# gbordelon/fast_ray_tracer

Measured on AMD Instinct MI355X. Metric: Mrays/s (primary+shadow+secondary) + wall-clock/frame, 1/2/4/8 GPU, higher is better.
Workload: dtype f64

## Files before the change

### fast_ray_tracer_amd/csrc/frt_camera.hpp

```cpp
#pragma once

#include "frt_shadow.hpp"

namespace frt {

struct QueuedRay {
    double o[3];
    double d[3];
    uint64_t key;
    int32_t parent;
    int32_t slot;
};

struct HitRec {
    double t;
    int32_t node;
    int32_t pad;
};

__device__ __forceinline__ double rng_uniform(uint64_t seed, uint64_t key, uint64_t d) {
    const uint64_t h = mix64(seed ^ mix64(key * 0x9e3779b97f4a7c15ULL + d * 0xd1b54a32d192ed03ULL + 0x632be59bd9b4e019ULL));
    return (double)(h >> 11) * 0x1.0p-53;
}

__device__ inline void cmj_point(uint64_t seed, uint64_t pixel, int U, int V, int u, int v, double* out) {
    const uint64_t base = 2ull * (uint64_t)U * (uint64_t)V;
    int p = v;
    for (int j = V - 1; j >= 0; --j) {
        const int k = (int)(j + rng_uniform(seed, pixel, base + j) * (double)(V - j));
        if (p == j) p = k;
        else if (p == k) p = j;
    }
    {
        const int f = p * U + u;
        const int jj = f / V, ii = f % V;
        const double r = rng_uniform(seed, pixel, 2ull * (uint64_t)f);
        out[0] = (ii + (jj + r) / (double)U) / (double)V;
    }
    p = u;
    for (int i = U - 1; i >= 0; --i) {
        const int k = (int)(i + rng_uniform(seed, pixel, base + (uint64_t)V + i) * (double)(U - i));
        if (p == i) p = k;
        else if (p == k) p = i;
    }
    {
        const int f = v * U + p;
        const int jj = f / V, ii = f % V;
        const double r = rng_uniform(seed, pixel, 2ull * (uint64_t)f + 1);
        out[1] = (jj + (ii + r) / (double)V) / (double)U;
    }
}

__device__ inline void aperture_point(const frt_camera& cam, uint64_t seed, uint64_t sample, double* xy,
                                      unsigned& err) {
    const double* a = cam.aperture_args;
    const int type = cam.aperture_type;
    if (type == 6 || type == 4 || type == 5 || type == 8 || type < 0 || type > 8) {
        xy[0] = 0.5;
        xy[1] = 0.5;
        return;
    }
    for (int attempt = 0; attempt < 4096; ++attempt) {
        const double x = rng_uniform(seed ^ 0xa5e7u, sample, 2ull * attempt);
        const double y = rng_uniform(seed ^ 0xa5e7u, sample, 2ull * attempt + 1);
        const double u = 2 * x - 1, v = 2 * y - 1;
        bool ok;
        switch (type) {
        case 0: ok = !(u * u + v * v > a[0]); break;
        case 1: ok = ((u > a[0]) && (u <= a[1])) || ((v > a[2]) && (v <= a[3])); break;
        case 2:
            ok = (u <= 0) ? (-u + a[0] <= v) && (v < u + a[1]) : (0 <= x) ? (u + a[2] <= v) && (v < -u + a[3]) : false;
            break;
        case 3: {
            const double mag = u * u + v * v;
            ok = !(mag > a[0] || mag < a[1]);
            break;
        }
        default: ok = true; break;
        }
        if (ok) {
            xy[0] = x;
            xy[1] = y;
            return;
        }
    }
    err |= kErrAperture;
    xy[0] = 0.5;
    xy[1] = 0.5;
}

__device__ __forceinline__ void ray_for_pixel(const frt_camera& cam, double px, double py, const double* jit,
                                              const double* ap, Ray& r) {
    double xoff = (px + jit[0]) * cam.pixel_size;
    double yoff = (py + jit[1]) * cam.pixel_size;
    double wx = cam.half_width - xoff, wy = cam.half_height - yoff;
    double p[3] = {wx, wy, -cam.canvas_distance}, pixel[3], origin[3];
    xf_point(cam.inv, p, pixel);
    double q[3] = {(ap[0] - 0.5) * cam.aperture_size, (ap[1] - 0.5) * cam.aperture_size, 0.0};
    xf_point(cam.inv, q, origin);
    double v[3] = {pixel[0] - origin[0], pixel[1] - origin[1], pixel[2] - origin[2]};
    r.o[0] = origin[0];
    r.o[1] = origin[1];
    r.o[2] = origin[2];
    normalize3(v, r.d);
}

__device__ __forceinline__ void camera_ray(const DevScene& S, const Batch& B, int64_t s, Ray& r, uint64_t& key,
                                           unsigned& err) {
    const int64_t pix = B.pixel_begin + s / B.spp;
    const int sub = (int)(s % B.spp);
    const int64_t hs = S.cam.hsize;
    const int64_t row = B.row_begin + (pix / hs) * B.row_stride;
    const int64_t col = pix % hs;
    const uint64_t global_pixel = (uint64_t)(row * hs + col);
    const uint64_t global_sample = global_pixel * (uint64_t)B.spp + (uint64_t)sub;
    double jit[2], ap[2] = {0.5, 0.5};
    if (S.cam.jitter) {
        const int U = (int)S.cam.usteps, V = (int)S.cam.vsteps;
        cmj_point(B.seed, global_pixel, U, V, sub % U, sub / U, jit);
    } else {
        jit[0] = S.sample_table[2 * sub];
        jit[1] = S.sample_table[2 * sub + 1];
    }
    if (S.cam.aperture_size != 0.0) aperture_point(S.cam, B.seed, global_sample, ap, err);
    ray_for_pixel(S.cam, (double)col, (double)row, jit, ap, r);
    key = (global_sample << 12) | 1ull;
}

}
```

### fast_ray_tracer_amd/csrc/frt_engine.hip

```cpp
#include <hip/hip_runtime.h>
#include <hipcub/hipcub.hpp>

#include <algorithm>
#include <array>
#include <atomic>
#include <condition_variable>
#include <memory>
#include <mutex>
#include <cmath>
#include <cstdio>
#include <cstdlib>
#include <cstring>
#include <string>
#include <chrono>
#include <functional>
#include <thread>
#include <vector>

#include "frt_device.h"
#include "frt_jit.h"
#include "frt_shade.hpp"
#include "frt_shade32.hpp"
#include "frt_shadow.hpp"
#include "frt_jit_rt.hpp"
#include "frt_camera.hpp"
#include "frt_cols.hpp"

namespace frt {

constexpr int kBlock = 256;
constexpr int kMaxPathLength = 11;

struct NodeRec {
    double over_point[3];
    uint64_t key;
    int32_t material;
    int32_t parent;
    int32_t slot;
    int32_t flags;
    double normalv[3];
    double eyev[3];
    double Ka[3], Kd[3], Ks[3];
    double refl[3];
    double Ns, over_d, rf;
};
static_assert(sizeof(NodeRec) == 216, "NodeRec layout");

struct NodeCore {
    int32_t material, flags, parent, slot;
    double normalv[3], eyev[3];
    double over_d, rf;
};
struct NodeColors {
    double Ka[3], Kd[3], Ks[3], refl[3];
    double Ns;
};
static_assert(sizeof(NodeCore) == 80 && sizeof(NodeColors) == 104, "NodeCols layout");
enum NodeFlags : int32_t { kReflApplies = 1, kRefrApplies = 2, kMix = 4, kDissolve = 8, kReflSpawned = 16, kRefrSpawned = 32 };
enum : int32_t { kOwnColors = 64, kOwnD = 128 };

struct NodeCols {
    Cols<NodeCore> core;
    Cols<NodeColors> col;
    const ShadowHead* head = nullptr;
    int32_t root = 0;
    int32_t eye_cam = 0;
    static size_t bytes(int64_t cap) { return Cols<NodeCore>::bytes(cap) + Cols<NodeColors>::bytes(cap); }
    void set(uint64_t* base, int64_t cap) {
        core.w = base;
        core.cap = cap;
        col.w = base + (size_t)Cols<NodeCore>::kWords * cap;
        col.cap = cap;
    }
    __device__ __forceinline__ void store(int64_t i, const NodeRec& v, bool own_colors, bool own_d) const {
        NodeCore c;
        for (int k = 0; k < 3; ++k) {
            c.normalv[k] = v.normalv[k];
            c.eyev[k] = v.eyev[k];
        }
        c.material = v.material;
        c.parent = v.parent;
        c.slot = v.slot;
        c.flags = v.flags | (own_colors ? kOwnColors : 0) | (own_d ? kOwnD : 0);
        c.over_d = v.over_d;
        c.rf = v.rf;
        uint64_t t[10];
        __builtin_memcpy(t, &c, sizeof(c));
        const int64_t cap = core.cap;
        core.w[i] = t[0];
        if (!root) core.w[cap + i] = t[1];
#pragma unroll
        for (int f = 2; f < 5; ++f) core.w[f * cap + i] = t[f];
        if (!eye_cam) {
#pragma unroll
            for (int f = 5; f < 8; ++f) core.w[f * cap + i] = t[f];
        }
        if (own_d) core.w[8 * cap + i] = t[8];
        if (c.flags & kMix) core.w[9 * cap + i] = t[9];
        if (own_colors) {
            NodeColors o;
            for (int k = 0; k < 3; ++k) {
                o.Ka[k] = v.Ka[k];
                o.Kd[k] = v.Kd[k];
                o.Ks[k] = v.Ks[k];
                o.refl[k] = v.refl[k];
            }
            o.Ns = v.Ns;
            col.store(i, o);
        }
    }
    __device__ __forceinline__ void store_miss(int64_t i, int32_t parent, int32_t slot) const {
        core.w[i] = (uint64_t)(uint32_t)-1;
        if (!root) core.w[core.cap + i] = (uint64_t)(uint32_t)parent | ((uint64_t)(uint32_t)slot << 32);
    }
    __device__ __forceinline__ NodeRec load(int64_t i, const frt_material* __restrict__ mats) const {
        uint64_t t[10];
        const int64_t cap = core.cap;
        t[0] = core.w[i];
        t[1] = root ? (uint64_t)(uint32_t)-1 : core.w[cap + i];
#pragma unroll
        for (int f = 2; f < 5; ++f) t[f] = core.w[f * cap + i];
#pragma unroll
        for (int f = 5; f < 8; ++f) t[f] = eye_cam ? 0ull : core.w[f * cap + i];
        const int32_t mat = (int32_t)(uint32_t)t[0], fl = (int32_t)(t[0] >> 32);
        const double od = (fl & kOwnD) ? __longlong_as_double((long long)core.w[8 * cap + i])
                          : mat >= 0 ? 1.0 - mats[mat].Tr : 0.0;
        const double rf = (fl & kMix) ? __longlong_as_double((long long)core.w[9 * cap + i]) : 0.0;
        t[8] = (uint64_t)__double_as_longlong(od);
        t[9] = (uint64_t)__double_as_longlong(rf);
        NodeCore c;
        __builtin_memcpy(&c, t, sizeof(c));
        NodeRec v;
        const ShadowHead& hd = head[i];
        for (int k = 0; k < 3; ++k) {
            v.over_point[k] = hd.over_point[k];
            v.normalv[k] = c.normalv[k];
            v.eyev[k] = c.eyev[k];
        }
        v.key = hd.key;
        v.material = c.material;
        v.parent = c.parent;
        v.slot = c.slot;
        v.flags = c.flags;
        v.over_d = c.over_d;
        v.rf = c.rf;
        if (c.material < 0) {
            for (int k = 0; k < 3; ++k) v.Ka[k] = v.Kd[k] = v.Ks[k] = v.refl[k] = 0.0;
            v.Ns = 0.0;
        } else if (c.flags & kOwnColors) {
            const NodeColors o = col.load(i);
            for (int k = 0; k < 3; ++k) {
                v.Ka[k] = o.Ka[k];
                v.Kd[k] = o.Kd[k];
                v.Ks[k] = o.Ks[k];
                v.refl[k] = o.refl[k];
            }
            v.Ns = o.Ns;
        } else {
            const frt_material& M = mats[c.material];
            for (int k = 0; k < 3; ++k) {
                v.Ka[k] = M.Ka[k];
                v.Kd[k] = M.Kd[k];
                v.Ks[k] = M.Ks[k];
                v.refl[k] = M.refl[k];
            }
            v.Ns = M.Ns;
        }
        return v;
    }
};










extern __shared__ __align__(16) char frt_walk_smem[];

#ifndef FRT_TRACE_WAVES
#define FRT_TRACE_WAVES 4
#endif
template <int kFeat>
__global__ void __launch_bounds__(kTraceBlock)
__attribute__((amdgpu_waves_per_eu((kFeat & kFeatTorus) ? 1 : FRT_TRACE_WAVES, 8))) k_trace(DevScene S, Batch B, const QueuedRay* __restrict__ q, int64_t n,
                                                       HitRec* __restrict__ hits, double* __restrict__ hn12, unsigned* err,
                                                       int filter_casts) {
    const int64_t i = (int64_t)blockIdx.x * blockDim.x + threadIdx.x;
    const bool live = i < n && (q == nullptr || q[queue_slot(B, i)].parent >= -1);
    Ray r{{0, 0, 0}, {0, 0, 1}};
    unsigned e = 0;
    if (live) {
        if (q == nullptr) {
            uint64_t key;
            camera_ray(S, B, i, r, key, e);
        } else {
            const QueuedRay& qr = q[queue_slot(B, i)];
            for (int k = 0; k < 3; ++k) {
                r.o[k] = qr.o[k];
                r.d[k] = qr.d[k];
            }
        }
    }
    double t;
    double n12[2];
    const int node = walk<false, kFeat>(S, r, 0.0, live, t, frt_walk_smem, e, n12, filter_casts != 0);
    if (i < n) {
        hits[i] = live ? HitRec{t, node, 0} : HitRec{0.0, -1, 0};
        if (hn12 != nullptr) {
            hn12[2 * i] = live ? n12[0] : 1.0;
            hn12[2 * i + 1] = live ? n12[1] : 1.0;
        }
    }
    if (e) atomicOr(err, e);
}

template <int kFeat>
__global__ void __launch_bounds__(kTraceBlock) k_trace_redo(DevScene S, Batch B, const QueuedRay* __restrict__ q, int64_t n,
                                                            HitRec* __restrict__ hits, unsigned* err,
                                                            const int32_t* __restrict__ redo,
                                                            const unsigned* __restrict__ redo_count, unsigned redo_cap) {
    const unsigned cnt = min(*redo_count, redo_cap);
    const int64_t wave = ((int64_t)blockIdx.x * blockDim.x + threadIdx.x) >> 6;
    const int64_t nwaves = ((int64_t)gridDim.x * blockDim.x) >> 6;
    unsigned e = 0;
    for (int64_t base = wave * 64; base < (int64_t)cnt; base += nwaves * 64) {
        const int64_t k = base + (threadIdx.x & 63);
        const int64_t i = k < (int64_t)cnt ? (int64_t)redo[k] : -1;
        const bool live = i >= 0 && i < n;
        Ray r{{0, 0, 0}, {0, 0, 1}};
        if (live) {
            if (q == nullptr) {
                uint64_t key;
                camera_ray(S, B, i, r, key, e);
            } else {
                const QueuedRay& qr = q[queue_slot(B, i)];
                for (int a = 0; a < 3; ++a) {
                    r.o[a] = qr.o[a];
                    r.d[a] = qr.d[a];
                }
            }
        }
        double t;
        double n12[2];
        const int node = walk<false, kFeat>(S, r, 0.0, live, t, frt_walk_smem, e, n12, false);
        if (live) hits[i] = HitRec{t, node, 0};
    }
    if (e) atomicOr(err, e);
}

#ifndef FRT_PREPARE_WAVES
#define FRT_PREPARE_WAVES 1
#endif
template <bool kPat>
__device__ __forceinline__ bool prepare_node(const DevScene& S, const Batch& B, const QueuedRay* __restrict__ q,
                                             int64_t n, const HitRec* __restrict__ hits, const double* __restrict__ hn12,
                                             NodeCols& rec,
                                             ShadowHead* __restrict__ heads, QueuedRay* __restrict__ next_q,
                                             unsigned long long* counters, unsigned* err, int64_t node, double* op,
                                             int* spawned, int uniform_ok) {
    unsigned long long* line = counters + kCounterLine * (blockIdx.x % kQueueSegs);
    const int64_t seg_base = (int64_t)(blockIdx.x % kQueueSegs) * B.next_segcap;
#ifdef FRT_WALK_PROF
    unsigned long long pt0 = prof_stamp();
    auto pstamp = [&](int k) {
        const unsigned long long t1 = prof_stamp();
        if ((threadIdx.x & 63) == 0) atomicAdd(S.dbg + kDbgProf + 8 + k, t1 - pt0);
        pt0 = t1;
    };
#define PSTAMP(k) pstamp(k)
#else
#define PSTAMP(k)
#endif
    Ray r;
    uint64_t key;
    int32_t parent = -1, slot = 0;
    if (q == nullptr) {
        unsigned ce = 0;
        camera_ray(S, B, node, r, key, ce);
    } else {
        const QueuedRay& qr = q[queue_slot(B, node)];
        for (int k = 0; k < 3; ++k) {
            r.o[k] = qr.o[k];
            r.d[k] = qr.d[k];
        }
        key = qr.key;
        parent = qr.parent;
        slot = qr.slot;
    }
    PSTAMP(0);
    const HitRec hr = hits[node];
    PSTAMP(1);
    if (hr.node < 0) {
        rec.store_miss(node, parent, slot);
        heads[node].material = -1;
        return false;
    }
    auto prepare_hit = [&](const DevScene& S, const int leaf) __attribute__((always_inline)) {
    Hit h{hr.t, -1, -1, leaf};
    Comps c;
    prepare<kPat>(S, r, h, c);
    c.n1 = hn12 != nullptr ? hn12[2 * node] : 1.0;
    c.n2 = hn12 != nullptr ? hn12[2 * node + 1] : 1.0;
    PSTAMP(2);
    if (B.stats) wave_count(line + 17, true);
    const frt_material& M = S.materials[c.material];
    NodeRec nr;
    for (int k = 0; k < 3; ++k) {
        nr.over_point[k] = c.over_point[k];
        nr.normalv[k] = c.normalv[k];
        nr.eyev[k] = c.eyev[k];
        nr.Ka[k] = c.Ka[k];
        nr.Kd[k] = c.Kd[k];
        nr.Ks[k] = c.Ks[k];
        nr.refl[k] = c.refl[k];
    }
    nr.Ns = c.Ns;
    nr.over_d = c.over_d;
    nr.rf = 0.0;
    nr.key = key;
    nr.material = c.material;
    nr.parent = parent;
    nr.slot = slot;
    int32_t flags = 0;
    if (S.cfg.include_specular) {
        const bool reflect_applies = B.remaining > 0 && M.reflective;
        bool refract_applies = false;
        double refr_dir[3] = {0, 0, 0};
        if (B.remaining > 0 && c.over_d > 0.0) {
            double n_ratio = c.n1 / c.n2;
            double cos_i = dot3(c.eyev, c.normalv);
            double sin2_t = n_ratio * n_ratio * (1.0 - cos_i * cos_i);
            if (!(sin2_t > 1.0)) {
                refract_applies = true;
                double cos_t = sqrt(1.0 - sin2_t);
                double s1 = n_ratio * cos_i - cos_t;
                for (int k = 0; k < 3; ++k) {
                    double t1 = c.normalv[k] * s1;
                    double t2 = c.eyev[k] * n_ratio;
                    refr_dir[k] = t1 - t2;
                }
            }
        }
        if (reflect_applies) flags |= kReflApplies;
        if (refract_applies) flags |= kRefrApplies;
        if (M.reflective && c.over_d < 1.0) {
            flags |= kMix;
            nr.rf = schlick(c.eyev, c.normalv, c.n1, c.n2);
        }
        if (M.Tr > 0.0 && c.over_d > 0.0) flags |= kDissolve;

        const uint64_t code = key & 0xFFFull;
        const uint64_t base = key & ~0xFFFull;
        const bool want_refl = reflect_applies && (c.refl[0] != 0.0 || c.refl[1] != 0.0 || c.refl[2] != 0.0);
        const bool tf_zero = M.Tf[0] == 0.0 && M.Tf[1] == 0.0 && M.Tf[2] == 0.0;
        const bool want_refr = refract_applies && !tf_zero;
        if (want_refl) flags |= kReflSpawned;
        if (want_refr) flags |= kRefrSpawned;
        const bool dense = spawned != nullptr;
        const unsigned long long at_refl = dense ? 0ull : wave_append(line + B.level + 1, want_refl);
        const unsigned long long at_refr = dense ? 0ull : wave_append(line + B.level + 1, want_refr);
        if (dense) *spawned = (want_refl ? 1 : 0) | (want_refr ? 2 : 0);
        if (B.stats) {
            wave_count(line + 16, reflect_applies && !want_refl);
            wave_count(line + 16, refract_applies && !want_refr);
        }
        if (want_refl) {
            if (dense || (int64_t)at_refl < B.next_segcap) {
                QueuedRay qo;
                for (int k = 0; k < 3; ++k) {
                    qo.o[k] = c.over_point[k];
                    qo.d[k] = c.reflectv[k];
                }
                qo.key = base | ((code * 2) & 0xFFFull);
                qo.parent = (int32_t)node;
                qo.slot = 0;
                next_q[dense ? node : seg_base + (int64_t)at_refl] = qo;
            } else {
                atomicOr(err, kErrQueueOverflow);
            }
        }
        if (want_refr) {
            if (dense || (int64_t)at_refr < B.next_segcap) {
                QueuedRay qo;
                for (int k = 0; k < 3; ++k) {
                    qo.o[k] = c.under_point[k];
                    qo.d[k] = refr_dir[k];
                }
                qo.key = base | ((code * 2 + 1) & 0xFFFull);
                qo.parent = (int32_t)node;
                qo.slot = 1;
                next_q[dense ? n + node : seg_base + (int64_t)at_refr] = qo;
            } else {
                atomicOr(err, kErrQueueOverflow);
            }
        }
    }
    nr.flags = flags;
    PSTAMP(3);
    const bool own = kPat && (M.map_Ka >= 0 || M.map_Kd >= 0 || M.map_Ks >= 0 || M.map_refl >= 0 || M.map_Ns >= 0);
    rec.store(node, nr, own, kPat && M.map_d >= 0);
    ShadowHead hd;
    for (int k = 0; k < 3; ++k) hd.over_point[k] = c.over_point[k];
    hd.key = key;
    hd.material = c.material;
    hd.pad = 0;
#ifdef FRT_EXPERIMENT_HEAD_COLS
    {
        uint64_t t[5];
        __builtin_memcpy(t, &hd, sizeof(hd));
        uint64_t* w = (uint64_t*)heads;
#pragma unroll
        for (int f = 0; f < 5; ++f) w[(int64_t)f * n + node] = t[f];
    }
#else
    heads[node] = hd;
#endif
    PSTAMP(4);
    for (int k = 0; k < 3; ++k) op[k] = c.over_point[k];
    };
    if (uniform_ok) {
        const int leaf_u = uniform(hr.node);
        if (__ballot(hr.node != leaf_u) == 0ull) {
            if (B.stats) wave_count(line + 18, (int)(threadIdx.x & 63) == __builtin_ctzll(__ballot(true)));
            prepare_hit(uniform_view(S), leaf_u);
            return true;
        }
    }
    prepare_hit(S, hr.node);
    return true;
}

__device__ __forceinline__ void tile_box(int64_t node, int64_t n, bool hit, const double* op, float* __restrict__ tbox,
                                         int tile_log2, float* __restrict__ stbox, int sub_log2) {
    float lo[3], hi[3];
#pragma unroll
    for (int a = 0; a < 3; ++a) {
        lo[a] = hit ? __double2float_rd(op[a]) : __builtin_huge_valf();
        hi[a] = hit ? __double2float_ru(op[a]) : -__builtin_huge_valf();
    }
    for (int off = 1; off < (1 << tile_log2); off <<= 1) {
        if (stbox != nullptr && off == (1 << sub_log2) && node < n && (node & (off - 1)) == 0) {
            float* b = stbox + 6 * (node >> sub_log2);
#pragma unroll
            for (int a = 0; a < 3; ++a) {
                b[a] = lo[a];
                b[a + 3] = hi[a];
            }
        }
#pragma unroll
        for (int a = 0; a < 3; ++a) {
            lo[a] = fminf(lo[a], __shfl_xor(lo[a], off, 64));
            hi[a] = fmaxf(hi[a], __shfl_xor(hi[a], off, 64));
        }
    }
    if (node < n && (node & ((1 << tile_log2) - 1)) == 0) {
        float* b = tbox + 6 * (node >> tile_log2);
#pragma unroll
        for (int a = 0; a < 3; ++a) {
            b[a] = lo[a];
            b[a + 3] = hi[a];
        }
    }
}

template <bool kPat>
__global__ void __launch_bounds__(kBlock) __attribute__((amdgpu_waves_per_eu(kPat ? 1 : FRT_PREPARE_WAVES, 8)))
k_prepare(DevScene S, Batch B, const QueuedRay* __restrict__ q, int64_t n, const HitRec* __restrict__ hits,
          const double* __restrict__ hn12,
          NodeCols rec, ShadowHead* __restrict__ heads, QueuedRay* __restrict__ next_q, unsigned long long* counters,
          unsigned* err, float* __restrict__ tbox, int tile_log2, float* __restrict__ stbox, int sub_log2,
          int32_t* __restrict__ counts, unsigned long long* __restrict__ spawn_masks, int uniform_ok) {
    const int64_t node = (int64_t)blockIdx.x * blockDim.x + threadIdx.x;
    double op[3] = {0.0, 0.0, 0.0};
    bool hit = false;
    if (node < n && counts != nullptr)
        for (int l = 0; l < S.num_lights; ++l) counts[node * S.num_lights + l] = 0;
    int spawned = 0;
    if (node < n)
        hit = prepare_node<kPat>(S, B, q, n, hits, hn12, rec, heads, next_q, counters, err, node, op,
                                 spawn_masks != nullptr ? &spawned : nullptr, uniform_ok);
    if (spawn_masks != nullptr) {
        const unsigned long long mr = __ballot(spawned & 1), mt = __ballot((spawned >> 1) & 1);
        const int64_t g = node >> 6, G = (n + 63) >> 6;
        if ((threadIdx.x & 63) == 0 && g < G) {
            spawn_masks[g] = mr;
            spawn_masks[G + g] = mt;
        }
    }
    if (tbox != nullptr) tile_box(node, n, hit, op, tbox, tile_log2, stbox, sub_log2);
}

#ifdef FRT_SHADOW_WAVES
#define FRT_SHADOW_ATTR __attribute__((amdgpu_waves_per_eu(FRT_SHADOW_WAVES, 8)))
#else
#define FRT_SHADOW_ATTR
#endif
template <int kFeat>
__global__ void __launch_bounds__(kTraceBlock) FRT_SHADOW_ATTR k_shadow(DevScene S, Batch B, const ShadowHead* __restrict__ shead, int64_t n,
                                                        const int32_t* __restrict__ j_light,
                                                        const int32_t* __restrict__ j_point, int32_t samples_per_node,
                                                        int32_t* __restrict__ counts, unsigned* err) {
    ShadowLane L;
    shadow_lane(S, B, shead, n, j_light, j_point, samples_per_node, (int64_t)blockIdx.x * blockDim.x + threadIdx.x, L);
    unsigned e = 0;
    double unused;
#ifdef FRT_EXPERIMENT_NOWALK
    const bool lit = L.live && L.distance > 0.5;
#else
    const bool lit = walk<true, kFeat>(S, L.r, L.distance, L.live, unused, frt_walk_smem, e) == 0 && L.live;
#endif
    if (e) atomicOr(err, e);
    shadow_count(S, L, lit, counts);
}

template <int kFeat>
__global__ void __launch_bounds__(kTraceBlock) k_shadow_redo(DevScene S, Batch B, const ShadowHead* __restrict__ shead, int64_t n,
                                                             const int32_t* __restrict__ j_light,
                                                             const int32_t* __restrict__ j_point, int32_t samples_per_node,
                                                             int32_t* __restrict__ counts, unsigned* err,
                                                             const int64_t* __restrict__ redo,
                                                             const unsigned* __restrict__ redo_count, unsigned redo_cap) {
    const unsigned cnt = min(*redo_count, redo_cap);
    const int64_t wave = ((int64_t)blockIdx.x * blockDim.x + threadIdx.x) >> 6;
    const int64_t nwaves = ((int64_t)gridDim.x * blockDim.x) >> 6;
    unsigned e = 0;
    for (int64_t base = wave * 64; base < (int64_t)cnt; base += nwaves * 64) {
        const int64_t k = base + (threadIdx.x & 63);
        ShadowLane L;
        shadow_lane(S, B, shead, n, j_light, j_point, samples_per_node, k < (int64_t)cnt ? redo[k] : -1, L);
        double unused;
        const bool lit = walk<true, kFeat>(S, L.r, L.distance, L.live, unused, frt_walk_smem, e) == 0 && L.live;
        if (lit) atomicAdd(counts + L.node * S.num_lights + L.light, 1);
    }
    if (e) atomicOr(err, e);
}

#ifndef FRT_SHADE_FACTOR
#define FRT_SHADE_FACTOR 1
#endif
#ifndef FRT_SHADE_ALG
#define FRT_SHADE_ALG 1
#endif
#ifndef FRT_SHADE_SKIP
#define FRT_SHADE_SKIP 1
#endif
#ifndef FRT_SHADE_FMA
#define FRT_SHADE_FMA 1
#endif
__device__ __forceinline__ double dot3_shade(const double* a, const double* b) {
    if (FRT_SHADE_FMA) return __builtin_fma(a[0], b[0], __builtin_fma(a[1], b[1], a[2] * b[2]));
    return dot3(a, b);
}
__device__ __forceinline__ void camera_eyev(const DevScene& S, const Batch& B, int64_t i, double* eyev) {
    Ray r;
    uint64_t key;
    unsigned ce = 0;
    camera_ray(S, B, i, r, key, ce);
    for (int k = 0; k < 3; ++k) eyev[k] = r.d[k] * -1.0;
}

__global__ void __launch_bounds__(kBlock) k_view_rays(DevScene S, Batch B, const frt_camera* __restrict__ cams,
                                                      int32_t nviews, int64_t view_pixels, int64_t n,
                                                      QueuedRay* __restrict__ q, unsigned* err) {
    const int64_t i = (int64_t)blockIdx.x * blockDim.x + threadIdx.x;
    if (i >= n) return;
    const int64_t pix = B.pixel_begin + i / B.spp;
    const int view = (int)min((int64_t)(nviews - 1), pix / view_pixels);
    Batch Bv = B;
    Bv.pixel_begin = pix - (int64_t)view * view_pixels - i / B.spp;
    unsigned e = 0;
    auto emit = [&](const frt_camera& cam) {
        DevScene Sv = S;
        Sv.cam = cam;
        QueuedRay qr;
        Ray r;
        camera_ray(Sv, Bv, i, r, qr.key, e);
        for (int k = 0; k < 3; ++k) {
            qr.o[k] = r.o[k];
            qr.d[k] = r.d[k];
        }
        qr.parent = -1;
        qr.slot = 0;
        q[i] = qr;
    };
    const int view_u = uniform(view);
    if (__ballot(view != view_u) == 0ull) emit(const_table(cams)[view_u]);
    else emit(cams[view]);
    if (e) atomicOr(err, e);
}

constexpr int kLdsPoints = 128;
__device__ __forceinline__ void shade_node(const DevScene& S, const Batch& B, const NodeRec& nr, int64_t i,
                                           const int32_t* __restrict__ counts, double* out, double* lds_row = nullptr,
                                           int32_t c0 = -1) {
    double sA[3] = {0, 0, 0}, sD[3] = {0, 0, 0}, sS[3] = {0, 0, 0};
    if (S.cfg.include_direct) {
        for (int li = 0; li < S.num_lights; ++li) {
            const frt_light& L = S.lights[li];
            const int32_t cnt = c0 >= 0 ? c0 : counts[i * S.num_lights + li];
// ... 308 lines not shown
                const int row = L.rows <= 1 ? 0 : light_row(L, B.seed, nr.key, li, 1);
                const int ra = __builtin_amdgcn_readfirstlane(row);
                if (L.rows <= 1) {
                    uniform_points(row0);
                } else if (__ballot(row != ra) == 0ull) {
                    uniform_points(row0 + 3 * (int64_t)ra * ns);
                } else {
                    const float* pts = row0 + 3 * (int64_t)row * ns;
                    float a[3] = {pts[0], pts[1], pts[2]};
                    const float* q1 = pts + 3 * min(1, ns - 1);
                    float b[3] = {q1[0], q1[1], q1[2]};
                    for (int p = 0; p < ns; ++p) {
                        const float lp[3] = {a[0], a[1], a[2]};
                        a[0] = b[0];
                        a[1] = b[1];
                        a[2] = b[2];
                        const float* q = pts + 3 * min(p + 2, ns - 1);
                        b[0] = q[0];
                        b[1] = q[1];
                        b[2] = q[2];
                        point_term32(P, Q, lp, sums);
                    }
                }
                const double scaling = inten / (double)L.num_samples;
                for (int k = 0; k < 3; ++k) {
                    const double dacc = nr.Kd[k] * L.intensity[k] * sums.ldn;
                    const double sacc =
                        nr.Ks[k] * L.intensity[k] * sums.b + (1.0 - nr.Ks[k]) * L.intensity[k] * sums.fb;
                    cD[k] = (0.0 + dacc) * scaling;
                    cS[k] = (0.0 + sacc) * scaling;
                }
            }
            if (S.cfg.include_ambient)
                for (int k = 0; k < 3; ++k) cA[k] = 0.0 + amb[k];
            for (int k = 0; k < 3; ++k) {
                sA[k] += cA[k];
                sD[k] += cD[k];
                sS[k] += cS[k];
            }
        }
    }
    for (int k = 0; k < 3; ++k) {
        out[k] = sA[k];
        out[4 + k] = sD[k];
        out[8 + k] = sS[k];
    }
    out[3] = out[7] = out[11] = 0.0;
}

__device__ __forceinline__ bool shade_heavy(const DevScene& S, const int32_t* __restrict__ counts, int64_t i) {
    if (!S.cfg.include_direct || !(S.cfg.include_diffuse || S.cfg.include_spec_highlight)) return false;
    for (int li = 0; li < S.num_lights; ++li)
        if (counts[i * S.num_lights + li] != 0) return true;
    return false;
}

__device__ __forceinline__ void ambient_node(const DevScene& S, const NodeRec& nr, double* out) {
    double sA[3] = {0, 0, 0};
    if (S.cfg.include_direct && S.cfg.include_ambient)
        for (int li = 0; li < S.num_lights; ++li) {
            const frt_light& L = S.lights[li];
            for (int k = 0; k < 3; ++k) sA[k] += 0.0 + nr.Ka[k] * L.intensity[k];
        }
    for (int k = 0; k < 3; ++k) {
        out[k] = sA[k];
        out[4 + k] = 0.0;
        out[8 + k] = 0.0;
    }
    out[3] = out[7] = out[11] = 0.0;
}

constexpr int kShadeSegs = 64;
static_assert(kShadeSegs == jit::kMixSegs, "k_shade_lit reads its slots with jit::mix_slot");
template <bool kLazy>
__global__ void __launch_bounds__(kBlock) k_shade(DevScene S, Batch B, NodeCols rec, int64_t n,
                                                  const int32_t* __restrict__ counts, Cols<Tri9> surface,
                                                  uint32_t* __restrict__ lit, unsigned* __restrict__ lcount,
                                                  uint32_t segcap) {
    const int64_t i = (int64_t)blockIdx.x * blockDim.x + threadIdx.x;
    bool heavy = false, mine = false;
    NodeRec nr{};
    if (i < n) {
        nr = rec.load(i, S.materials);
        mine = nr.material >= 0;
        heavy = mine && lit != nullptr && shade_heavy(S, counts, i);
    }
    if (!kLazy && mine && !heavy) {
        double out[12];
        if (rec.eye_cam) camera_eyev(S, B, i, nr.eyev);
        shade_node(S, B, nr, i, counts, out);
        tri_store(surface, i, out);
    }
    if (lit != nullptr) {
        const unsigned long long m = __ballot(heavy);
        if (m) {
            const int lane = threadIdx.x & 63;
            const int seg = (int)(blockIdx.x % kShadeSegs);
            unsigned base = 0;
            if (lane == 0) base = atomicAdd(lcount + seg * jit::kMixLine, (unsigned)__popcll(m));
            base = __shfl(base, 0, 64);
            const unsigned at = base + (unsigned)__popcll(m & ((1ull << lane) - 1));
            if (heavy) lit[(size_t)seg * segcap + at] = (uint32_t)i;
        }
    }
}

struct MaskPopc {
    const unsigned long long* m;
    int64_t count;
    __host__ __device__ uint32_t operator()(int64_t i) const { return i < count ? (uint32_t)__popcll(m[i]) : 0u; }
};
__global__ void __launch_bounds__(kBlock) k_spawn_expand(const unsigned long long* __restrict__ masks,
                                                         const uint32_t* __restrict__ offs, int64_t n, int64_t G,
                                                         uint32_t* __restrict__ qperm,
                                                         unsigned long long* __restrict__ counters) {
    const int64_t g = (int64_t)blockIdx.x * blockDim.x + threadIdx.x;
    if (g == 0) counters[20] = offs[2 * G];
    if (g >= 2 * G) return;
    unsigned long long m = masks[g];
    uint32_t at = offs[g];
    const uint32_t slot0 = (uint32_t)((g < G ? 0 : n) + ((g < G ? g : g - G) << 6));
    while (m != 0ull) {
        qperm[at++] = slot0 + (uint32_t)__builtin_ctzll(m);
        m &= m - 1ull;
    }
}

__global__ void __launch_bounds__(kBlock) k_queue_keys(Batch B, const QueuedRay* __restrict__ q, int64_t n, int pbits,
                                                       int shift, uint32_t* __restrict__ keys,
                                                       uint32_t* __restrict__ slots) {
    const int64_t i = (int64_t)blockIdx.x * blockDim.x + threadIdx.x;
    if (i >= n) return;
    const int64_t s = queue_slot(B, i);
    const QueuedRay& qr = q[s];
    keys[i] = ((uint32_t)(qr.slot & 1) << (pbits - shift)) | ((uint32_t)qr.parent >> shift);
    slots[i] = (uint32_t)s;
}

__device__ __forceinline__ unsigned lit_total(const unsigned* __restrict__ lcount) {
    const int lane = threadIdx.x & 63;
    unsigned incl = lcount[lane * jit::kMixLine];
#pragma unroll
    for (int o = 1; o < 64; o <<= 1) {
        const unsigned t = __shfl_up(incl, o, 64);
        if (lane >= o) incl += t;
    }
    return __shfl(incl, 63, 64);
}

__global__ void __launch_bounds__(kBlock) k_lit_rows(DevScene S, Batch B, const ShadowHead* __restrict__ head,
                                                     const uint32_t* __restrict__ lit, const unsigned* __restrict__ lcount,
                                                     uint32_t segcap, int sort_light, uint32_t* __restrict__ rows,
                                                     uint32_t* __restrict__ nodes) {
    const uint32_t m = blockIdx.x * blockDim.x + threadIdx.x;
    const unsigned total = lit_total(lcount);
    if (blockIdx.x * blockDim.x + (threadIdx.x & ~63u) >= total) return;
    const size_t slot = jit::mix_slot(m < total ? m : 0u, lcount, segcap);
    if (m >= total) return;
    const uint32_t i = lit[slot];
    rows[m] = (uint32_t)light_row(S.lights[sort_light], B.seed, head[i].key, sort_light, 1);
    nodes[m] = i;
}

struct LitStage {
    double over_point[3], normalv[3], eyev[3];
    uint64_t key;
    int32_t material, flags;
    uint32_t node;
    int32_t c0;
};
static_assert(sizeof(LitStage) == 96, "LitStage layout");

__global__ void __launch_bounds__(kBlock) k_lit_stage(DevScene S, Batch B, NodeCols rec, const int32_t* __restrict__ counts,
                                                      const uint32_t* __restrict__ lit, const unsigned* __restrict__ lcount,
                                                      uint32_t segcap, int sort_light, uint32_t* __restrict__ rows,
                                                      uint32_t* __restrict__ vals, LitStage* __restrict__ stage) {
    const uint32_t m = blockIdx.x * blockDim.x + threadIdx.x;
    const unsigned total = lit_total(lcount);
    if (blockIdx.x * blockDim.x + (threadIdx.x & ~63u) >= total) return;
    const size_t slot = jit::mix_slot(m < total ? m : 0u, lcount, segcap);
    if (m >= total) return;
    const uint32_t i = lit[slot];
    NodeRec nr = rec.load(i, S.materials);
    if (rec.eye_cam) camera_eyev(S, B, i, nr.eyev);
    LitStage r;
    for (int k = 0; k < 3; ++k) {
        r.over_point[k] = nr.over_point[k];
        r.normalv[k] = nr.normalv[k];
        r.eyev[k] = nr.eyev[k];
    }
    r.key = nr.key;
    r.material = nr.material;
    r.flags = nr.flags;
    r.node = i;
    r.c0 = S.num_lights == 1 ? counts[i] : -1;
    uint64_t w[12];
    __builtin_memcpy(w, &r, sizeof(r));
    uint64_t* dst = (uint64_t*)(stage + m);
#pragma unroll
    for (int k = 0; k < 12; ++k) dst[k] = w[k];
    rows[m] = (uint32_t)light_row(S.lights[sort_light], B.seed, nr.key, sort_light, 1);
    vals[m] = m;
}

#ifndef FRT_SHADE_WAVES
#define FRT_SHADE_WAVES 4
#endif
template <bool kRows, bool kFast32>
__device__ __forceinline__ void shade_lit_body(const DevScene& S, const Batch& B, const NodeCols& rec,
                                               const int32_t* __restrict__ counts, Cols<Tri9> surface,
                                               const uint32_t* __restrict__ lit,
                                               const unsigned* __restrict__ lcount, uint32_t segcap,
                                               const uint32_t* __restrict__ flat,
                                               const LitStage* __restrict__ stage, uint32_t* __restrict__ spos,
                                               const Light32& F) {
    const uint32_t m = blockIdx.x * blockDim.x + threadIdx.x;
    const int lane = threadIdx.x & 63;
    const unsigned c = lcount[lane * jit::kMixLine];
    unsigned incl = c;
#pragma unroll
    for (int o = 1; o < 64; o <<= 1) {
        const unsigned t = __shfl_up(incl, o, 64);
        if (lane >= o) incl += t;
    }
    const unsigned total = __shfl(incl, 63, 64);
    if (blockIdx.x * blockDim.x + (threadIdx.x & ~63u) >= total) return;
    int64_t i = 0;
    NodeRec nr{};
    int32_t c0 = -1;
    const bool staged = kRows && stage != nullptr;
    const bool sorted_out = kRows && spos != nullptr;
    if (staged) {
        if (m >= total) return;
        const uint64_t* src = (const uint64_t*)(stage + flat[m]);
        uint64_t w[12];
#pragma unroll
        for (int k = 0; k < 12; ++k) w[k] = src[k];
        LitStage r;
        __builtin_memcpy(&r, w, sizeof(r));
        for (int k = 0; k < 3; ++k) {
            nr.over_point[k] = r.over_point[k];
            nr.normalv[k] = r.normalv[k];
            nr.eyev[k] = r.eyev[k];
        }
        nr.key = r.key;
        nr.material = r.material;
        nr.flags = r.flags;
        c0 = r.c0;
        i = (int64_t)r.node;
    } else {
        if (flat != nullptr) {
            if (m >= total) return;
            i = (int64_t)flat[m];
        } else {
            const size_t slot = jit::mix_slot(m < total ? m : 0u, lcount, segcap);
            if (m >= total) return;
            i = (int64_t)lit[slot];
        }
        nr = rec.load(i, S.materials);
        if (rec.eye_cam) camera_eyev(S, B, i, nr.eyev);
    }
    if (staged) {
        if (nr.flags & kOwnColors) {
            const NodeColors o = rec.col.load(i);
            for (int k = 0; k < 3; ++k) {
                nr.Ka[k] = o.Ka[k];
                nr.Kd[k] = o.Kd[k];
                nr.Ks[k] = o.Ks[k];
            }
            nr.Ns = o.Ns;
        } else {
            const frt_material& M = S.materials[nr.material];
            for (int k = 0; k < 3; ++k) {
                nr.Ka[k] = M.Ka[k];
                nr.Kd[k] = M.Kd[k];
                nr.Ks[k] = M.Ks[k];
            }
            nr.Ns = M.Ns;
        }
    }
    double out[12];
#ifndef FRT_SHADE_LDS_ROWS
#define FRT_SHADE_LDS_ROWS 0
#endif
    if constexpr (kFast32) {
        shade_node32(S, B, F, nr, i, counts, out, c0);
    } else if (kRows && FRT_SHADE_LDS_ROWS) {
        __shared__ double lds_rows[kBlock / 64][3 * kLdsPoints];
        shade_node(S, B, nr, i, counts, out, lds_rows[threadIdx.x >> 6], c0);
    } else {
        shade_node(S, B, nr, i, counts, out, nullptr, c0);
    }
    if (sorted_out) {
        uint64_t* dst = surface.w + (size_t)9 * m;
#pragma unroll
        for (int k = 0; k < 3; ++k) {
            dst[k] = (uint64_t)__double_as_longlong(out[k]);
            dst[3 + k] = (uint64_t)__double_as_longlong(out[4 + k]);
            dst[6 + k] = (uint64_t)__double_as_longlong(out[8 + k]);
        }
        spos[i] = m;
        return;
    }
    tri_store(surface, i, out);
}

template <bool kRows>
__global__ void __launch_bounds__(kBlock) __attribute__((amdgpu_waves_per_eu(FRT_SHADE_WAVES, 8))) k_shade_lit(DevScene S, Batch B, NodeCols rec,
                                                      const int32_t* __restrict__ counts, Cols<Tri9> surface,
                                                      const uint32_t* __restrict__ lit,
                                                      const unsigned* __restrict__ lcount, uint32_t segcap,
                                                      const uint32_t* __restrict__ flat,
                                                      const LitStage* __restrict__ stage, uint32_t* __restrict__ spos) {
    shade_lit_body<kRows, false>(S, B, rec, counts, surface, lit, lcount, segcap, flat, stage, spos, Light32{});
}

template <bool kRows>
__global__ void __launch_bounds__(kBlock) k_shade_lit32(DevScene S, Batch B, NodeCols rec,
                                                        const int32_t* __restrict__ counts, Cols<Tri9> surface,
                                                        const uint32_t* __restrict__ lit,
                                                        const unsigned* __restrict__ lcount, uint32_t segcap,
                                                        const uint32_t* __restrict__ flat,
                                                        const LitStage* __restrict__ stage, uint32_t* __restrict__ spos,
                                                        Light32 F) {
    shade_lit_body<kRows, true>(S, B, rec, counts, surface, lit, lcount, segcap, flat, stage, spos, F);
}

__device__ __forceinline__ void combine_node(const DevScene& S, const int32_t* __restrict__ counts,
                                             const NodeRec& nr, int64_t i, Cols<Tri9> surface, Cols<Tri9> child,
                                             const frt_material* __restrict__ mats, int32_t include_specular,
                                             double* col, const uint32_t* __restrict__ spos = nullptr) {
    if (nr.material < 0) {
        for (int k = 0; k < 12; ++k) col[k] = 0.0;
        return;
    }
    if (counts != nullptr && !shade_heavy(S, counts, i)) {
        ambient_node(S, nr, col);
    } else if (spos != nullptr) {
        const uint64_t* src = surface.w + (size_t)9 * spos[i];
#pragma unroll
        for (int k = 0; k < 3; ++k) {
            col[k] = __longlong_as_double((long long)src[k]);
// ... 720 lines not shown
    std::vector<void*> owned;
    std::vector<double> host_table;
    hipStream_t stream = nullptr;
    int32_t* j_light = nullptr;
    int32_t* j_point = nullptr;
    int32_t samples_per_node = 0;
    size_t lds_bytes = 0;
    void* jit_shadow = nullptr;
    void* jit_beam = nullptr;
    void* jit_tile = nullptr;
    void* jit_list = nullptr;
    int tile = 0;
    uint64_t scene_key = 0;
    void* jit_sub = nullptr;
    int sub = 0;
    int sub_ps = 0;
    const int32_t* light_psamp2 = nullptr;
    const float* light_sbox = nullptr;
    uint32_t* slist = nullptr;
    int64_t slist_cap = 0;
    uint64_t sub_pairs = 0, sub_mixed = 0;
    void* jit_subtile = nullptr;
    void* jit_trace = nullptr;
    int32_t* tredo = nullptr;
    int64_t tredo_cap = 0;
    int subtile = 0;
    bool node_beam = false;
    float* stbox = nullptr;
    int64_t stbox_cap = 0;
    uint32_t* s2list = nullptr;
    int64_t s2list_cap = 0;
    uint64_t subtile_pairs = 0, subtile_mixed = 0;
    float* tbox = nullptr;
    int64_t tbox_cap = 0;
    uint32_t* tlist = nullptr;
    int64_t tlist_cap = 0;
    uint64_t tile_pairs = 0, tile_mixed = 0, node_pairs = 0, node_mixed = 0;
    bool jit_beam_on = true;
    const int32_t* light_psamp = nullptr;
    const float* light_aabb = nullptr;
    uint32_t* mixed = nullptr;
    int64_t mixed_cap = 0;
    unsigned* mcount = nullptr;
    uint64_t sync_epoch = 0;
    PinnedBuf<unsigned> host_mcount;
    PinnedBuf<unsigned long long> host_counters;
    PinnedBuf<unsigned> host_lcount;
    int64_t* redo = nullptr;
    unsigned* redo_count = nullptr;
    unsigned redo_cap = 0;
    frt_frame_stats* cur_st = nullptr;
    uint64_t rays_walked = 0;
    uint64_t pairs_walked = 0;
    uint64_t heads_walked = 0;
    unsigned long long uniform_stats[3] = {0, 0, 0};
    uint32_t* shade_lit = nullptr;
    int64_t shade_lit_cap = 0;
    int sort_light = -1;
    int shade_stage = 0;
    uint32_t* lit_row = nullptr;
    int64_t lit_row_cap = 0;
    uint32_t* lit_flat = nullptr;
    int64_t lit_flat_cap = 0;
    frt::LitStage* lit_stage = nullptr;
    int64_t lit_stage_cap = 0;
    bool fast32 = false;
    frt::Light32 light32{nullptr, nullptr};
    int queue_sort = 2;
    int queue_sort_shift = 0;
    int prepare_uniform = 1;
    uint32_t* qsort = nullptr;
    int64_t qsort_cap = 0;
    unsigned long long* spawn_masks = nullptr;
    int64_t spawn_masks_cap = 0;
    uint32_t* spawn_offs = nullptr;
    int64_t spawn_offs_cap = 0;
    unsigned char* scan_tmp = nullptr;
    int64_t scan_tmp_cap = 0;
    unsigned* shade_lcount = nullptr;
    int64_t shade_lcount_cap = 0;
    unsigned long long* jit_stats = nullptr;
    struct Level {
        frt::NodeCols rec;
        frt::ShadowHead* head = nullptr;
        frt::QueuedRay* q = nullptr;
        frt::Cols<frt::Tri9> surface;
        frt::Cols<frt::Tri9> child;
        int64_t* qprefix = nullptr;
        std::vector<int64_t> hprefix = std::vector<int64_t>(frt::kQueueSegs + 1, 0);
        int32_t* counts = nullptr;
        uint32_t* spos = nullptr;
        bool staged = false;
        uint32_t* qperm = nullptr;
        int64_t qperm_cap = 0;
        bool sorted = false;
        int64_t cap = 0;
    };
    std::vector<Level> levels;
    frt::HitRec* hits = nullptr;
    int64_t hits_cap = 0;
    double* hn12 = nullptr;
    int64_t hn12_cap = 0;
    frt::Cols<frt::Tri9> sample_col;
    int64_t sample_cap = 0;
    double* out_dev = nullptr;
    int64_t out_cap = 0;
    frt_camera* view_cams = nullptr;
    int64_t view_cams_cap = 0;
    int32_t strip_views = 0;
    frt::QueuedRay* view_q = nullptr;
    int64_t view_q_cap = 0;
    unsigned long long* counters = nullptr;
    unsigned* err = nullptr;
    hipEvent_t ev[2] = {nullptr, nullptr};
    struct Mark {
        int slot;
        size_t a, b;
    };
    std::vector<hipEvent_t> ev_pool;
    std::vector<Mark> ev_marks;
    size_t ev_used = 0;
    std::vector<frt_light> host_lights;
    struct Gi {
        bool built = false;
        uint64_t seed = 0;
        void* map_mem[2] = {nullptr, nullptr};
        uint64_t photons[2] = {0, 0};
        frt::QueuedRay* pq[2] = {nullptr, nullptr};
        double* ppow[2] = {nullptr, nullptr};
        int64_t pq_cap[2] = {0, 0}, ppow_cap[2] = {0, 0};
        frt::HitRec* phits = nullptr;
        int64_t phits_cap = 0;
        double* pn12 = nullptr;
        int64_t pn12_cap = 0;
        frt::StoredPhoton* store = nullptr;
        int64_t store_cap = 0;
        frt::QueuedRay* gq = nullptr;
        frt::HitRec* ghits = nullptr;
        double* gcol = nullptr;
        frt::GatherReq* greq = nullptr;
        int64_t gq_cap = 0, ghits_cap = 0, gcol_cap = 0, greq_cap = 0;
        unsigned* gwork = nullptr;
        uint32_t* gkeys = nullptr;
        int64_t gkeys_cap = 0;
        double* extra = nullptr;
        double* fgather = nullptr;
        int64_t extra_cap = 0, fgather_cap = 0;
    } gi;
};

static thread_local std::string g_last_error;

static inline void hip_ignore(hipError_t) {}

static int fail(const std::string& msg) {
    g_last_error = msg;
    return -1;
}

#define FRT_HIP(call)                                                                                   \
    do {                                                                                                \
        hipError_t e_ = (call);                                                                         \
        if (e_ != hipSuccess) return fail(std::string(#call) + ": " + hipGetErrorString(e_));          \
    } while (0)

template <typename T>
static const T* upload(frt_scene_handle* h, const T* src, size_t count, int& rc) {
// ... 1137 lines not shown
        hipMemset(h->S.dbg, 0, frt::kDbgSlots * sizeof(unsigned long long)) != hipSuccess) {
        frt_scene_release(h);
        return fail("frt_scene_upload: debug counters");
    }
#endif
    static const bool wtrace = std::getenv("FRT_WARMUP_TRACE") != nullptr;
    const auto ts0 = std::chrono::steady_clock::now();
    {
        std::lock_guard<std::mutex> lk(g_warm_mu);
        if (device >= 0 && device < 64 && g_warm_stream[device] != nullptr) {
            h->stream = g_warm_stream[device];
            g_warm_stream[device] = nullptr;
        }
    }
    const bool stream_ok = h->stream != nullptr || hipStreamCreate(&h->stream) == hipSuccess;
    if (wtrace)
        std::fprintf(stderr, "frt upload: hipStreamCreate %.2f ms\n",
                     std::chrono::duration<double, std::milli>(std::chrono::steady_clock::now() - ts0).count());
    if (!stream_ok || hipMalloc((void**)&h->counters, frt::kQueueSegs * frt::kCounterLine * sizeof(unsigned long long)) != hipSuccess ||
        hipMalloc((void**)&h->err, sizeof(unsigned)) != hipSuccess || hipEventCreate(&h->ev[0]) != hipSuccess ||
        hipEventCreate(&h->ev[1]) != hipSuccess) {
        frt_scene_release(h);
        return fail("frt_scene_upload: stream / counter allocation failed");
    }
    h->levels.resize((size_t)std::max(1, sc->config.path_length + 2));
    *out = h;
    phase(6);
    t_upload_phases[7] = std::chrono::duration<double, std::milli>(std::chrono::steady_clock::now() - up0).count();
    return 0;
}

void frt_scene_release(frt_scene_handle* h) {
    if (!h) return;
    hip_ignore(hipSetDevice(h->device));
    if (h->jit_stats) {
        std::vector<unsigned long long> c(kJitStatWords);
        if (hipMemcpy(c.data(), h->jit_stats, c.size() * sizeof(unsigned long long), hipMemcpyDeviceToHost) == hipSuccess) {
            unsigned long long live = 0, amb = 0, pairs = 0, mixed = 0, tpairs = 0, tmixed = 0, spairs = 0, smixed = 0,
                               upairs = 0, umixed = 0;
            for (int j = 0; j < 64; ++j) {
                live += c[32 * j];
                amb += c[32 * j + 1];
                pairs += c[32 * j + 2];
                mixed += c[32 * j + 3];
                tpairs += c[32 * j + 4];
                tmixed += c[32 * j + 5];
                spairs += c[32 * j + 6];
                smixed += c[32 * j + 7];
                upairs += c[32 * j + 8];
                umixed += c[32 * j + 9];
            }
            if (tpairs)
                std::fprintf(stderr, "frt jit stats: tile pair kernel (%d nodes per tile): live tile pairs %llu, mixed %llu (%.2f%%)\n",
                             h->tile, tpairs, tmixed, 100.0 * (double)tmixed / (double)tpairs);
            std::fprintf(stderr, "frt jit stats: pair kernel: live pairs %llu, mixed %llu (%.2f%%)\n", pairs, mixed,
                         pairs ? 100.0 * (double)mixed / (double)pairs : 0.0);
            if (spairs)
                std::fprintf(stderr, "frt jit stats: sub-part pair kernel (%d sub-parts): live sub-pairs %llu, mixed %llu (%.2f%%)\n",
                             h->sub, spairs, smixed, 100.0 * (double)smixed / (double)spairs);
            if (upairs)
                std::fprintf(stderr, "frt jit stats: sub-tile pair kernel (%d nodes per sub-tile): live sub-tile pairs %llu, mixed %llu (%.2f%%)\n",
                             h->subtile, upairs, umixed, 100.0 * (double)umixed / (double)upairs);
            std::fprintf(stderr, "frt jit stats: live shadow lanes %llu, re-walked in binary64 %llu (%.4f%%)\n", live, amb,
                         live ? 100.0 * (double)amb / (double)live : 0.0);
            std::fprintf(stderr, "frt jit stats: (node, light) pairs: all lit %llu, all shadowed %llu, mixed %llu\n",
                         h->uniform_stats[0], h->uniform_stats[1], h->uniform_stats[2]);
            for (int k = 0; k < std::min(h->S.num_nodes, 512); ++k)
                if (c[2048 + 2 * k])
                    std::fprintf(stderr, "frt jit stats: node %d: %llu waves, %llu lanes tested; composites: %llu waves, %llu lanes entered\n",
                                 k, c[2048 + 2 * k], c[2048 + 2 * k + 1], c[3072 + 2 * k], c[3072 + 2 * k + 1]);
            for (int k = std::max(h->S.num_nodes, 100); k < 2048; ++k)
                if (c[3072 + 2 * k + 1])
                    std::fprintf(stderr, "frt jit stats: beam site %d: %llu waves, %llu lanes\n", k, c[3072 + 2 * k],
                                 c[3072 + 2 * k + 1]);
            for (int k = 0; k < 2048; ++k)
                if (c[9216 + 2 * k + 1])
                    std::fprintf(stderr, "frt jit stats: tile beam site %d: %llu waves, %llu lanes\n", k, c[9216 + 2 * k],
                                 c[9216 + 2 * k + 1]);
        }
    }
    for (void* p : h->owned) hip_ignore(hipFree(p));
    for (auto& L : h->levels) {
        hip_ignore(hipFree(L.rec.core.w));
        hip_ignore(hipFree(L.head));
        hip_ignore(hipFree(L.q));
        hip_ignore(hipFree(L.surface.w));
        hip_ignore(hipFree(L.child.w));
        hip_ignore(hipFree(L.counts));
        hip_ignore(hipFree(L.spos));
        hip_ignore(hipFree(L.qprefix));
        hip_ignore(hipFree(L.qperm));
    }
    hip_ignore(hipFree(h->hits));
    hip_ignore(hipFree(h->hn12));
    {
        auto& G = h->gi;
        for (int m = 0; m < 2; ++m) {
            hip_ignore(hipFree(G.map_mem[m]));
            hip_ignore(hipFree(G.pq[m]));
            hip_ignore(hipFree(G.ppow[m]));
        }
        hip_ignore(hipFree(G.phits));
        hip_ignore(hipFree(G.pn12));
        hip_ignore(hipFree(G.store));
        hip_ignore(hipFree(G.gq));
        hip_ignore(hipFree(G.ghits));
        hip_ignore(hipFree(G.gcol));
        hip_ignore(hipFree(G.greq));
        hip_ignore(hipFree(G.gwork));
        hip_ignore(hipFree(G.gkeys));
        hip_ignore(hipFree(G.extra));
        hip_ignore(hipFree(G.fgather));
    }
    hip_ignore(hipFree(h->sample_col.w));
    hip_ignore(hipFree(h->out_dev));
    hip_ignore(hipFree(h->view_cams));
    hip_ignore(hipFree(h->view_q));
    hip_ignore(hipFree(h->counters));
    hip_ignore(hipFree(h->shade_lit));
    hip_ignore(hipFree(h->shade_lcount));
    hip_ignore(hipFree(h->lit_row));
    hip_ignore(hipFree(h->lit_flat));
    hip_ignore(hipFree(h->qsort));
    hip_ignore(hipFree(h->spawn_masks));
    hip_ignore(hipFree(h->spawn_offs));
    hip_ignore(hipFree(h->lit_stage));
    hip_ignore(hipFree(h->scan_tmp));
    hip_ignore(hipFree(h->mixed));
    hip_ignore(hipFree(h->tlist));
    hip_ignore(hipFree(h->slist));
    hip_ignore(hipFree(h->stbox));
    hip_ignore(hipFree(h->s2list));
    hip_ignore(hipFree(h->tredo));
    hip_ignore(hipFree(h->tbox));
    hip_ignore(hipFree(h->err));
    for (hipEvent_t e : h->ev_pool) hip_ignore(hipEventDestroy(e));
    if (h->ev[0]) hip_ignore(hipEventDestroy(h->ev[0]));
    if (h->ev[1]) hip_ignore(hipEventDestroy(h->ev[1]));
    if (h->stream) hip_ignore(hipStreamDestroy(h->stream));
    delete h;
}

static int32_t level_eye_cam(const frt_scene_handle* h, size_t d) {
    static const bool eye_cam_env = !(std::getenv("FRT_EYE_CAM") && std::atoi(std::getenv("FRT_EYE_CAM")) == 0);
    return d == 0 && !h->S.cfg.use_gi && eye_cam_env && h->strip_views == 0 ? 1 : 0;
}

static int ensure_level(frt_scene_handle* h, size_t d, int64_t need) {
    auto& L = h->levels[d];
    if (need <= L.cap) return 0;
    int64_t nc = std::max<int64_t>(need, L.cap * 2);
    hip_ignore(hipFree(L.rec.core.w));
    hip_ignore(hipFree(L.head));
    L.head = nullptr;
    hip_ignore(hipFree(L.q));
    hip_ignore(hipFree(L.surface.w));
    hip_ignore(hipFree(L.child.w));
    hip_ignore(hipFree(L.counts));
    hip_ignore(hipFree(L.spos));
    L.spos = nullptr;
    L.rec = {};
    L.q = nullptr;
    L.surface = {};
    L.child = {};
    L.counts = nullptr;
    {
        void* p = nullptr;
        FRT_HIP(hipMalloc(&p, frt::NodeCols::bytes(nc)));
        L.rec.set((uint64_t*)p, nc);
        L.rec.root = d == 0 ? 1 : 0;
        L.rec.eye_cam = level_eye_cam(h, d);
    }
    FRT_HIP(hipMalloc((void**)&L.head, nc * sizeof(frt::ShadowHead)));
    L.rec.head = L.head;
    FRT_HIP(hipMalloc((void**)&L.q, nc * sizeof(frt::QueuedRay)));
    FRT_HIP(hipMalloc((void**)&L.surface.w, frt::Cols<frt::Tri9>::bytes(nc)));
    L.surface.cap = nc;
    FRT_HIP(hipMalloc((void**)&L.child.w, frt::Cols<frt::Tri9>::bytes(2 * nc)));
    L.child.cap = 2 * nc;
    if (!L.qprefix) FRT_HIP(hipMalloc((void**)&L.qprefix, (frt::kQueueSegs + 1) * sizeof(int64_t)));
    FRT_HIP(hipMalloc((void**)&L.counts, nc * std::max(1, h->S.num_lights) * sizeof(int32_t)));
    if (h->shade_stage) FRT_HIP(hipMalloc((void**)&L.spos, nc * sizeof(uint32_t)));
    L.cap = nc;
    return 0;
}

static inline unsigned grid_for(int64_t n, int block = frt::kBlock) { return (unsigned)((n + block - 1) / block); }

static hipError_t stream_sync(frt_scene_handle* h) {
    const hipError_t e = hipStreamSynchronize(h->stream);
    if (e == hipSuccess) h->sync_epoch++;
    return e;
}

static bool shade_split() {
    const char* e = std::getenv("FRT_SHADE_SPLIT");
    return !(e && std::strcmp(e, "0") == 0);
}
static bool shade_lazy(const frt_scene_handle* h) {
    const char* e = std::getenv("FRT_SHADE_LAZY");
    return shade_split() && !h->S.cfg.use_gi && !(e && std::strcmp(e, "0") == 0);
}

struct KTimer {
    frt_scene_handle* h;
    frt_frame_stats* st;
    int slot;
    size_t a = 0;
    static hipEvent_t event(frt_scene_handle* h, size_t i) {
        while (h->ev_pool.size() <= i) {
            hipEvent_t e;
            hip_ignore(hipEventCreate(&e));
            h->ev_pool.push_back(e);
        }
        return h->ev_pool[i];
    }
    KTimer(frt_scene_handle* h_, frt_frame_stats* st_, int slot_) : h(h_), st(st_), slot(slot_) {
        if (st) {
            a = h->ev_used++;
            hip_ignore(hipEventRecord(event(h, a), h->stream));
        }
    }
    ~KTimer() {
        if (st) {
            size_t b = h->ev_used++;
            hip_ignore(hipEventRecord(event(h, b), h->stream));
            h->ev_marks.push_back({slot, a, b});
        }
    }
};

static void collect_timings(frt_scene_handle* h, frt_frame_stats* st) {
    for (const auto& m : h->ev_marks) {
        float ms = 0.f;
        hip_ignore(hipEventElapsedTime(&ms, h->ev_pool[m.a], h->ev_pool[m.b]));
        if (m.slot < 8) {
            st->kernel_ms[m.slot] += ms;
            st->kernel_launches[m.slot] += 1;
        } else if (m.slot < 24) {
            st->sub_ms[m.slot - 8] += ms;
            st->sub_launches[m.slot - 8] += 1;
        }
    }
    h->ev_marks.clear();
    h->ev_used = 0;
}

}

template <int F>
static void launch_trace_f(frt_scene_handle* h, const frt::Batch& B, const frt::QueuedRay* q, int64_t n,
                           frt::HitRec* hits, int filter_casts, double* hn12) {
    hipLaunchKernelGGL(frt::k_trace<F>, dim3(grid_for(n, frt::kTraceBlock)), dim3(frt::kTraceBlock), h->lds_bytes,
                       h->stream, h->S, B, q, n, hits, hn12, h->err, filter_casts);
}

template <int F>
static void launch_trace_redo_f(frt_scene_handle* h, const frt::Batch& B, const frt::QueuedRay* q, int64_t n,
                                frt::HitRec* hits) {
    const unsigned cap = (unsigned)(h->tredo_cap - 2);
    hipLaunchKernelGGL(frt::k_trace_redo<F>, dim3(1024), dim3(frt::kTraceBlock), h->lds_bytes, h->stream, h->S, B, q, n,
                       hits, h->err, h->tredo, (const unsigned*)(h->tredo + cap), cap);
}

static void launch_trace(frt_scene_handle* h, const frt::Batch& B, const frt::QueuedRay* q, int64_t n,
                         frt::HitRec* hits = nullptr, int filter_casts = 0, double* hn12 = nullptr, bool jit = false) {
    if (hits == nullptr) hits = h->hits;
    static const bool jit_trace_env = !(std::getenv("FRT_JIT_TRACE") && std::atoi(std::getenv("FRT_JIT_TRACE")) == 0);
    if (jit && h->jit_trace && jit_trace_env && !filter_casts && hn12 == nullptr && n > 0 && n < ((int64_t)1 << 31)) {
        if (!grow(&h->tredo, h->tredo_cap, n + 2)) {
            unsigned cap = (unsigned)(h->tredo_cap - 2);
            unsigned* cnt = (unsigned*)(h->tredo + cap);
            hip_ignore(hipMemsetAsync(cnt, 0, sizeof(unsigned), h->stream));
            void* args[] = {&h->S, (void*)&B, (void*)&q, &n, &hits, &h->err, &h->tredo, &cnt, &cap};
            if (hipModuleLaunchKernel((hipFunction_t)h->jit_trace, (unsigned)grid_for(n, frt::kTraceBlock), 1, 1,
                                      frt::kTraceBlock, 1, 1, 0, h->stream, args, nullptr) == hipSuccess) {
                switch (h->S.features & 3) {
                case 0: launch_trace_redo_f<0>(h, B, q, n, hits); break;
                case 1: launch_trace_redo_f<1>(h, B, q, n, hits); break;
                case 2: launch_trace_redo_f<2>(h, B, q, n, hits); break;
                default: launch_trace_redo_f<3>(h, B, q, n, hits); break;
                }
                static const bool trace_stats = std::getenv("FRT_JIT_TRACE_STATS") != nullptr;
                if (trace_stats) {
                    unsigned c = 0;
                    hip_ignore(hipMemcpyAsync(&c, cnt, sizeof(c), hipMemcpyDeviceToHost, h->stream));
                    hip_ignore(hipStreamSynchronize(h->stream));
                    std::fprintf(stderr, "frt: frt_jit_trace level %d: %lld rays, %u to the generic walk\n", B.level,
                                 (long long)n, c);
                    const char* dump = std::getenv("FRT_JIT_TRACE_DUMP");
                    if (dump && B.level == 0 && c > 0) {
                        std::vector<int32_t> v(std::min<size_t>(c, cap));
                        hip_ignore(hipMemcpy(v.data(), h->tredo, v.size() * sizeof(int32_t), hipMemcpyDeviceToHost));
                        if (FILE* f = std::fopen(dump, "wb")) {
                            std::fwrite(v.data(), sizeof(int32_t), v.size(), f);
                            std::fclose(f);
                        }
                    }
                }
                return;
            }
            std::fprintf(stderr, "frt: scene-specialised closest-hit kernel launch failed; k_trace\n");
            (void)hipGetLastError();
            h->jit_trace = nullptr;
        } else {
            (void)hipGetLastError();
        }
    }
    switch (h->S.features & 3) {
    case 0: launch_trace_f<0>(h, B, q, n, hits, filter_casts, hn12); break;
    case 1: launch_trace_f<1>(h, B, q, n, hits, filter_casts, hn12); break;
    case 2: launch_trace_f<2>(h, B, q, n, hits, filter_casts, hn12); break;
    default: launch_trace_f<3>(h, B, q, n, hits, filter_casts, hn12); break;
    }
}

template <int F>
static void launch_shadow_f(frt_scene_handle* h, const frt::Batch& B, const frt::ShadowHead* rec, int64_t n, int32_t* counts) {
    const int64_t work = n * h->samples_per_node;
    hipLaunchKernelGGL(frt::k_shadow<F>, dim3(grid_for(work, frt::kTraceBlock)), dim3(frt::kTraceBlock), h->lds_bytes,
                       h->stream, h->S, B, rec, n, h->j_light, h->j_point, h->samples_per_node, counts, h->err);
}

template <int F>
static void launch_shadow_redo_f(frt_scene_handle* h, const frt::Batch& B, const frt::ShadowHead* rec, int64_t n,
                                 int32_t* counts) {
    hipLaunchKernelGGL(frt::k_shadow_redo<F>, dim3(64), dim3(frt::kTraceBlock), h->lds_bytes, h->stream, h->S, B, rec, n,
                       h->j_light, h->j_point, h->samples_per_node, counts, h->err, h->redo, h->redo_count, h->redo_cap);
}

static uint64_t seg_table(const PinnedBuf<unsigned>& host_mcount, uint32_t segcap, uint64_t lpe,
                          frt::jit::SegTable& seg, uint64_t& total) {
    uint64_t nblk = 0;
    total = 0;
    for (int j = 0; j < frt::jit::kMixSegs; ++j) {
        const uint64_t c = std::min<uint64_t>(host_mcount[(size_t)j * frt::jit::kMixLine], segcap);
        seg.bstart[j] = (uint32_t)nblk;
        seg.count[j] = (uint32_t)c;
        total += c;
        nblk += (c * lpe + frt::kTraceBlock - 1) / frt::kTraceBlock;
    }
    seg.bstart[frt::jit::kMixSegs] = (uint32_t)nblk;
    return nblk;
}

static void launch_shadow(frt_scene_handle* h, const frt::Batch& B, const frt::ShadowHead* rec, int64_t n, int32_t* counts,
                          int64_t node0 = 0) {
    if (h->jit_shadow) {
        using frt::jit::kMixLine;
        using frt::jit::kMixSegs;
        int64_t NP = 0;
        for (const auto& L : h->host_lights) NP += std::max(1, (L.num_samples + frt_jit_part_size() - 1) / frt_jit_part_size());
        const char* mp_env = std::getenv("FRT_JIT_MAX_PAIRS");
        const long long mp = mp_env ? std::atoll(mp_env) : 0;
        int64_t kMaxPairs = mp >= 1 && mp < (1ll << 31) ? (int64_t)mp : (int64_t)((1ll << 31) - 1);
        static const int64_t min_pairs = [] {
            const char* e = std::getenv("FRT_JIT_MIN_PAIRS");
            return e ? (int64_t)std::atoll(e) : (int64_t)1 << 18;
        }();
        const bool beam_on = h->jit_beam_on && n * NP >= min_pairs;
        const bool tiled = beam_on && h->tile > 0 && h->jit_tile && h->jit_list && h->tbox;
        const bool subbed = tiled && h->jit_sub && h->sub > 0 && h->light_psamp2 && h->light_sbox;
        if (subbed && h->node_beam) {
            kMaxPairs = std::min<int64_t>(kMaxPairs, (int64_t)(0xFFFFFFFFull / (uint64_t)h->sub));
        } else if (subbed) {
            int stl = 0;
            while (h->subtile > 0 && (1 << stl) < h->tile / h->subtile) ++stl;
            const uint64_t per_tile = ((uint64_t)NP * (uint64_t)h->sub) << stl;
            const int64_t tiled_max = (int64_t)(0xFFFFFFFFull / per_tile) * h->tile * NP;
            kMaxPairs = std::min<int64_t>(std::min<int64_t>(tiled_max, (int64_t)0xFFFFFFFFll),
                                          mp >= 1 && mp < (1ll << 31) ? (int64_t)mp : INT64_MAX);
        }
        if (n * NP > kMaxPairs) {
            int64_t per = std::max<int64_t>(1, kMaxPairs / NP);
            if (h->tile > 0) per = std::max<int64_t>(h->tile, per / h->tile * h->tile);
            for (int64_t off = 0; off < n; off += per)
                launch_shadow(h, B, rec + off, std::min(per, n - off), counts + off * h->S.num_lights, node0 + off);
            return;
        }
        const int64_t npairs = n * NP;
        uint32_t nn = (uint32_t)n;
        uint32_t segcap = 0;
        unsigned* mc_tile = h->mcount;
        unsigned* mc_sub = h->mcount + kMixSegs * kMixLine;
        unsigned* mc_subtile = h->mcount + 2 * kMixSegs * kMixLine;
        unsigned* mc_node = h->mcount + 3 * kMixSegs * kMixLine;
        if (beam_on) hip_ignore(hipMemsetAsync(h->mcount, 0, 4 * kMixSegs * kMixLine * sizeof(unsigned), h->stream));
        uint64_t total_mixed = 0;
        const uint32_t* direct_in = nullptr;
        uint32_t direct_subq = 0, direct_nodes = 0;
        if (beam_on) {
            frt::jit::SegTable tseg{};
            uint32_t tsegcap = 0;
            uint64_t list_blocks = 0, listed = 0;
            const uint32_t* list_in = h->tlist;
            uint32_t list_segcap = 0;
            const float* list_boxes = h->light_aabb;
            int tl = 0;
            while ((1 << tl) < h->tile) ++tl;
            if (tiled) {
                const int64_t ntiles = (n + h->tile - 1) >> tl;
                uint32_t ntp = (uint32_t)(ntiles * NP);
                const int64_t tblocks = (ntiles * NP + frt::kTraceBlock - 1) / frt::kTraceBlock;
                tsegcap = (uint32_t)std::max<int64_t>(frt::kTraceBlock, ((tblocks + kMixSegs - 1) / kMixSegs) * frt::kTraceBlock);
                if (grow(&h->tlist, h->tlist_cap, 2 * (int64_t)tsegcap * kMixSegs)) {
                    (void)hipGetLastError();
                    h->jit_shadow = nullptr;
                    launch_shadow(h, B, rec, n, counts, node0);
                    return;
                }
                const float* tb = h->tbox + 6 * (node0 >> tl);
                const uint32_t* no_list = nullptr;
                uint32_t zero = 0;
                void* targs[] = {&h->S, (void*)&B, (void*)&rec, &ntp, &nn, (void*)&tb, (void*)&no_list, &tseg, &zero, &zero,
                                 &h->light_aabb, &counts, &h->tlist, &mc_tile, &tsegcap, &h->err, &h->jit_stats,
                                 &h->light_psamp2};
                hipError_t le;
                {
                    KTimer tt(h, h->cur_st, 12);
                    le = hipModuleLaunchKernel((hipFunction_t)h->jit_tile, grid_for(ntiles * NP, frt::kTraceBlock), 1, 1,
                                               frt::kTraceBlock, 1, 1, 0, h->stream, targs, nullptr);
                }
                if (le != hipSuccess) {
                    std::fprintf(stderr, "frt: scene-specialised tile kernel launch failed (%s); pairs per node\n",
                                 hipGetErrorString(le));
                    (void)hipGetLastError();
                    h->tile = 0;
                    launch_shadow(h, B, rec, n, counts, node0);
                    return;
                }
                if (hipMemcpyAsync(h->host_mcount.data(), mc_tile, h->host_mcount.size() * sizeof(unsigned),
                                   hipMemcpyDeviceToHost, h->stream) != hipSuccess ||
                    stream_sync(h) != hipSuccess)
                    return;
                list_blocks = seg_table(h->host_mcount, tsegcap, subbed ? (uint64_t)h->sub : (uint64_t)h->tile, tseg, listed);
                h->tile_pairs += ntp;
                h->tile_mixed += listed;
                list_in = h->tlist;
                list_segcap = tsegcap;
                if (subbed && listed > 0) {
                    const uint64_t sblocks = list_blocks;
                    const frt::jit::SegTable sseg = tseg;
                    const uint32_t ssegcap = (uint32_t)std::max<uint64_t>(frt::kTraceBlock,
                                                                          ((sblocks + kMixSegs - 1) / kMixSegs) * frt::kTraceBlock);
                    if (grow(&h->slist, h->slist_cap, 2 * (int64_t)ssegcap * kMixSegs)) {
                        (void)hipGetLastError();
                        h->jit_shadow = nullptr;
                        hip_ignore(hipMemsetAsync(counts, 0, (size_t)n * h->S.num_lights * sizeof(int32_t), h->stream));
                        launch_shadow(h, B, rec, n, counts, node0);
                        return;
                    }
                    hipError_t se = hipSuccess;
                    {
                        KTimer ts(h, h->cur_st, 13);
                        const uint64_t max_blocks = ((1ull << 31) - 1) / frt::kTraceBlock;
                        uint32_t zero = 0;
                        for (uint64_t b0 = 0; b0 < sblocks && se == hipSuccess; b0 += max_blocks) {
                            uint32_t b0u = (uint32_t)b0;
                            void* sargs[] = {&h->S, (void*)&B, (void*)&rec, &zero, &nn, (void*)&tb, &h->tlist, (void*)&sseg, &b0u,
                                             &tsegcap, &h->light_sbox, &counts, &h->slist, &mc_sub, (void*)&ssegcap, &h->err,
// ... 852 lines not shown
        else if (std::strcmp(e, "fast32") == 0)
            p = FRT_PRECISION_FAST32;
        else
            return fail(std::string("FRT_PRECISION=") + e + " is not supported (parity or fast32)");
    }
    if (p != FRT_PRECISION_PARITY && p != FRT_PRECISION_FAST32)
        return fail("precision " + std::to_string(P->precision) + " is not supported");
    if (p == FRT_PRECISION_FAST32 && !shade_split())
        return fail("precision fast32 is not supported with FRT_SHADE_SPLIT=0 (the unsplit k_shade is binary64 only)");
    h->fast32 = p == FRT_PRECISION_FAST32;
    return 0;
}

static int ensure_light32(frt_scene_handle* h) {
    if (h->light32.off != nullptr || h->S.num_lights == 0) return 0;
    int64_t len = 0;
    for (const frt_light& L : h->host_lights)
        len = std::max<int64_t>(len, L.points + 3 * (int64_t)L.num_samples * std::max(1, L.rows));
    if (len == 0 || h->S.light_points == nullptr) return 0;
    std::vector<double> pts((size_t)len);
    FRT_HIP(hipMemcpy(pts.data(), h->S.light_points, (size_t)len * sizeof(double), hipMemcpyDeviceToHost));
    std::vector<float> off((size_t)len + 4, 0.0f);
    std::vector<double> cent((size_t)h->S.num_lights * 3, 0.0);
    for (size_t l = 0; l < h->host_lights.size(); ++l) {
        const frt_light& L = h->host_lights[l];
        const int64_t np = (int64_t)L.num_samples * std::max(1, L.rows);
        if (np <= 0) continue;
        const double* p = pts.data() + L.points;
        double c[3] = {0.0, 0.0, 0.0};
        for (int64_t q = 0; q < np; ++q)
            for (int k = 0; k < 3; ++k) c[k] += p[3 * q + k];
        for (int k = 0; k < 3; ++k) cent[3 * l + (size_t)k] = c[k] /= (double)np;
        for (int64_t q = 0; q < np; ++q)
            for (int k = 0; k < 3; ++k) off[(size_t)(L.points + 3 * q + k)] = (float)(p[3 * q + k] - c[k]);
    }
    int rc = 0;
    const float* doff = upload(h, off.data(), off.size(), rc);
    const double* dcent = upload(h, cent.data(), cent.size(), rc);
    if (rc) return rc;
    h->light32.cent = dcent;
    h->light32.off = doff;
    return 0;
}

static int render_impl(frt_scene_handle* h, const frt_frame_params* P, double* dev_out, frt_frame_stats* st) {
    h->cur_st = st;
    h->rays_walked = 0;
    h->pairs_walked = 0;
    h->heads_walked = 0;
    h->tile_pairs = h->tile_mixed = h->node_pairs = h->node_mixed = h->sub_pairs = h->sub_mixed = 0;
    h->subtile_pairs = h->subtile_mixed = 0;
    const int rc = render_frame(h, P, dev_out, st);
    if (rc) h->gi.built = false;
    return rc;
}

static int render_strip(frt_scene_handle* h, const frt_camera* cams, int32_t nviews, const frt_frame_params* P,
                        double* dev_out, frt_frame_stats* st) {
    FRT_HIP(hipSetDevice(h->device));
    if (grow(&h->view_cams, h->view_cams_cap, nviews)) return -1;
    FRT_HIP(hipMemcpy(h->view_cams, cams, (size_t)nviews * sizeof(frt_camera), hipMemcpyHostToDevice));
    const frt_camera own = h->S.cam;
    h->S.cam = cams[0];
    h->strip_views = nviews;
    const int rc = render_impl(h, P, dev_out, st);
    h->strip_views = 0;
    h->S.cam = own;
    if (!h->levels.empty()) h->levels[0].rec.eye_cam = level_eye_cam(h, 0);
    return rc;
}

static int render_frame(frt_scene_handle* h, const frt_frame_params* P, double* dev_out, frt_frame_stats* st) {
    using namespace frt;
    FRT_HIP(hipSetDevice(h->device));
    if (frame_precision(h, P)) return -1;
    if (h->fast32 && ensure_light32(h)) return -1;
    const int64_t hs = h->S.cam.hsize;
    const int64_t stride = P->row_stride > 0 ? P->row_stride : 1;
    int64_t nrows = 0;
    for (int64_t r = P->row_begin; r < P->row_end; r += stride) nrows++;
    const int32_t nviews = h->strip_views;
    const int64_t npix = nrows * hs * std::max(1, nviews);
    if (!h->levels.empty()) h->levels[0].rec.eye_cam = level_eye_cam(h, 0);
    const int32_t spp = (int32_t)(h->S.cam.usteps * h->S.cam.vsteps);
    if (spp <= 0) return fail("render: usteps*vsteps must be positive");
    const char* benv = std::getenv("FRT_BATCH_SAMPLES");
    const int64_t bdef = benv && std::atoll(benv) > 0 ? (int64_t)std::atoll(benv) : (int64_t)1 << 23;
    int64_t batch = P->batch_samples > 0 ? P->batch_samples : bdef;
    int64_t pix_per_batch = std::max<int64_t>(1, batch / spp);
    const int path = h->S.cfg.path_length;
    if (st) {
        std::memset(st, 0, sizeof(*st));
        (void)hipEventRecord(h->ev[0], h->stream);
    }
    FRT_HIP(hipMemsetAsync(h->err, 0, sizeof(unsigned), h->stream));
    FRT_HIP(hipMemsetAsync(h->counters, 0, frt::kQueueSegs * frt::kCounterLine * sizeof(unsigned long long), h->stream));
    if (h->S.cfg.use_gi && (!h->gi.built || h->gi.seed != P->seed)) {
        hipEvent_t p0 = nullptr, p1 = nullptr;
        if (st) {
            hip_ignore(hipEventCreate(&p0));
            hip_ignore(hipEventCreate(&p1));
            hip_ignore(hipEventRecord(p0, h->stream));
        }
        const int rc = build_photon_maps(h, P->seed);
        if (st) {
            hip_ignore(hipEventRecord(p1, h->stream));
            hip_ignore(hipEventSynchronize(p1));
            float ms = 0.f;
            hip_ignore(hipEventElapsedTime(&ms, p0, p1));
            st->photon_ms = ms;
            st->photon_pass = 1;
            hip_ignore(hipEventDestroy(p0));
            hip_ignore(hipEventDestroy(p1));
        }
        if (rc) return rc;
    }
    if (st) {
        st->photons[0] = h->gi.photons[0];
        st->photons[1] = h->gi.photons[1];
    }
    if (!h->host_counters.resize((size_t)kQueueSegs * kCounterLine) ||
        !h->host_lcount.resize((size_t)kShadeSegs * jit::kMixLine))
        return fail("render: pinned host buffer allocation failed");
    auto& host_counters = h->host_counters;
    for (int64_t p0 = 0; p0 < npix; p0 += pix_per_batch) {
        const int64_t bp = std::min<int64_t>(pix_per_batch, npix - p0);
        const int64_t ns = bp * spp;
        if (ns > h->sample_cap) {
            hip_ignore(hipFree(h->sample_col.w));
            h->sample_col = {};
            h->sample_cap = 0;
            FRT_HIP(hipMalloc((void**)&h->sample_col.w, frt::Cols<frt::Tri9>::bytes(ns)));
            h->sample_col.cap = h->sample_cap = ns;
        }
        if (ensure_level(h, 0, ns)) return -1;
        if (nviews > 0 && grow(&h->view_q, h->view_q_cap, ns)) return -1;
        Batch B{};
        B.sample_begin = 0;
        const int64_t first_row = P->row_begin + ((p0 / hs) % std::max<int64_t>(1, nrows)) * stride;
        B.sample_begin = (first_row * hs + p0 % hs) * spp;
        B.pixel_begin = p0;
        B.num_samples = ns;
        B.row_begin = P->row_begin;
        B.row_stride = stride;
        B.seed = P->seed;
        B.spp = spp;
        B.stats = st != nullptr ? 1 : 0;
        std::vector<int64_t> count(path + 2, 0);
        count[0] = ns;
        FRT_HIP(hipMemset2DAsync(h->counters, kCounterLine * sizeof(unsigned long long), 0, 16 * sizeof(unsigned long long),
                                 kQueueSegs, h->stream));
        for (int d = 0; d <= path; ++d) {
            const int64_t n = count[d];
            if (n == 0) break;
            B.level = d;
            B.remaining = path - d;
            auto& L = h->levels[d];
            if (ensure_level(h, d + 1, 2 * n + (int64_t)kQueueSegs * 2 * kBlock)) return -1;
            auto& N = h->levels[d + 1];
            B.qprefix = d > 0 ? L.qprefix : nullptr;
            B.qperm = d > 0 && L.sorted ? L.qperm : nullptr;
            B.qsegcap = L.cap / kQueueSegs;
            B.next_segcap = N.cap / kQueueSegs;
            if (h->S.num_lights < 1)
                FRT_HIP(hipMemsetAsync(L.counts, 0, (size_t)n * sizeof(int32_t), h->stream));
            if (grow(&h->hits, h->hits_cap, n)) return -1;
            if (!h->S.cfg.all_ni_one && grow(&h->hn12, h->hn12_cap, 2 * n)) return -1;
            double* hn12 = h->S.cfg.all_ni_one ? nullptr : h->hn12;
            const QueuedRay* q = d == 0 ? (nviews > 0 ? h->view_q : nullptr) : L.q;
            bool dense = false;
            {
                KTimer t(h, st, d == 0 ? 5 : 0);
                if (d == 0 && nviews > 0) {
                    hipLaunchKernelGGL(k_view_rays, dim3(grid_for(n)), dim3(kBlock), 0, h->stream, h->S, B,
                                       (const frt_camera*)h->view_cams, nviews, nrows * hs, n, h->view_q, h->err);
                    FRT_HIP(hipGetLastError());
                }
                launch_trace(h, B, q, n, h->hits, 0, hn12, true);
                FRT_HIP(hipGetLastError());
            }
            {
                KTimer t(h, st, 6);
                const bool tiles = h->tile > 0 && h->jit_shadow && h->jit_beam_on && h->S.cfg.include_direct &&
                                   h->samples_per_node > 0;
                int tl = 0;
                while (tiles && (1 << tl) < h->tile) ++tl;
                if (tiles && grow(&h->tbox, h->tbox_cap, 6 * ((n >> tl) + 1))) return -1;
                const bool subtiles = tiles && h->subtile > 0 && h->subtile < h->tile;
                int stl = 0;
                while (subtiles && (1 << stl) < h->subtile) ++stl;
                if (subtiles && grow(&h->stbox, h->stbox_cap, 6 * ((n >> stl) + 1))) return -1;
                dense = h->queue_sort == 2 && d < path && 2 * n <= (int64_t)UINT32_MAX && N.cap >= 2 * n;
                const int64_t G = (n + 63) >> 6;
                if (dense && (grow(&h->spawn_masks, h->spawn_masks_cap, 2 * G) ||
                              grow(&h->spawn_offs, h->spawn_offs_cap, 2 * G + 1) || grow(&N.qperm, N.qperm_cap, 2 * n)))
                    return -1;
                hipLaunchKernelGGL(h->S.num_patterns > 0 ? k_prepare<true> : k_prepare<false>, dim3(grid_for(n)),
                                   dim3(kBlock), 0, h->stream, h->S, B, q, n, h->hits, hn12,
                                   L.rec, L.head, N.q, h->counters, h->err, tiles ? h->tbox : nullptr, tl,
                                   subtiles ? h->stbox : nullptr, stl, L.counts, dense ? h->spawn_masks : nullptr,
                                   h->prepare_uniform);
                FRT_HIP(hipGetLastError());
                if (dense) {
                    hipcub::CountingInputIterator<int64_t> idx(0);
                    hipcub::TransformInputIterator<uint32_t, MaskPopc, hipcub::CountingInputIterator<int64_t>> popc(
                        idx, MaskPopc{h->spawn_masks, 2 * G});
                    size_t tmp_bytes = 0;
                    FRT_HIP(hipcub::DeviceScan::ExclusiveSum(nullptr, tmp_bytes, popc, h->spawn_offs, (int)(2 * G + 1),
                                                             h->stream));
                    if (grow(&h->scan_tmp, h->scan_tmp_cap, (int64_t)tmp_bytes + 16)) return -1;
                    FRT_HIP(hipcub::DeviceScan::ExclusiveSum((void*)h->scan_tmp, tmp_bytes, popc, h->spawn_offs,
                                                             (int)(2 * G + 1), h->stream));
                    hipLaunchKernelGGL(k_spawn_expand, dim3(grid_for(2 * G)), dim3(kBlock), 0, h->stream, h->spawn_masks,
                                       h->spawn_offs, n, G, N.qperm, h->counters);
                    FRT_HIP(hipGetLastError());
                }
            }
            FRT_HIP(hipMemcpyAsync(host_counters.data(), h->counters, host_counters.size() * sizeof(unsigned long long),
                                   hipMemcpyDeviceToHost, h->stream));
            const uint64_t counters_epoch = h->sync_epoch;
            if (h->S.cfg.include_direct && h->samples_per_node > 0) {
                KTimer t(h, st, 1);
                launch_shadow(h, B, L.head, n, L.counts);
                FRT_HIP(hipGetLastError());
            }
            if (h->jit_stats && h->S.num_lights > 0) {
                std::vector<int32_t> hc((size_t)n * h->S.num_lights);
                std::vector<frt::ShadowHead> hh((size_t)n);
                FRT_HIP(hipMemcpyAsync(hc.data(), L.counts, hc.size() * sizeof(int32_t), hipMemcpyDeviceToHost, h->stream));
                FRT_HIP(hipMemcpyAsync(hh.data(), L.head, hh.size() * sizeof(frt::ShadowHead), hipMemcpyDeviceToHost, h->stream));
                FRT_HIP(hipStreamSynchronize(h->stream));
                for (int64_t i = 0; i < n; ++i) {
                    if (hh[(size_t)i].material < 0) continue;
                    for (int l = 0; l < h->S.num_lights; ++l) {
                        const int32_t c = hc[(size_t)(i * h->S.num_lights + l)];
                        h->uniform_stats[c == 0 ? 1 : (c == h->host_lights[(size_t)l].num_samples ? 0 : 2)]++;
                    }
                }
            }
            {
                KTimer t(h, st, 2);
                const bool split = shade_split();
                const int64_t nblocks = grid_for(n);
                const uint32_t segcap = (uint32_t)(((nblocks + kShadeSegs - 1) / kShadeSegs) * kBlock);
                if (split && (grow(&h->shade_lit, h->shade_lit_cap, (int64_t)segcap * kShadeSegs) ||
                              grow(&h->shade_lcount, h->shade_lcount_cap, (int64_t)kShadeSegs * jit::kMixLine)))
                    return -1;
                if (split)
                    FRT_HIP(hipMemsetAsync(h->shade_lcount, 0, (size_t)kShadeSegs * jit::kMixLine * sizeof(unsigned),
                                           h->stream));
                const bool sorted = split && h->sort_light >= 0;
                const int nrows = sorted ? std::max(1, h->host_lights[(size_t)h->sort_light].rows) : 0;
                int row_bits = 1;
                while (row_bits < 32 && (1ll << row_bits) < nrows) ++row_bits;
                const bool sorted_out = sorted && shade_lazy(h) && L.spos != nullptr && h->shade_stage > 0;
                const bool staged = sorted_out && h->shade_stage == 1;
                L.staged = sorted_out;
                if (sorted) {
                    const int64_t lcap = (int64_t)segcap * kShadeSegs;
                    if (grow(&h->lit_row, h->lit_row_cap, 2 * lcap) || grow(&h->lit_flat, h->lit_flat_cap, 2 * lcap))
                        return -1;
                    if (staged && grow(&h->lit_stage, h->lit_stage_cap, lcap)) return -1;
                }
                if (shade_lazy(h))
                    hipLaunchKernelGGL(k_shade<true>, dim3(grid_for(n)), dim3(kBlock), 0, h->stream, h->S, B, L.rec, n,
                                       L.counts, L.surface, h->shade_lit, h->shade_lcount, segcap);
                else
                    hipLaunchKernelGGL(k_shade<false>, dim3(grid_for(n)), dim3(kBlock), 0, h->stream, h->S, B, L.rec, n,
                                       L.counts, L.surface, split ? h->shade_lit : nullptr, h->shade_lcount, segcap);
                if (sorted) {
                    KTimer ts(h, st, 16);
                    const int64_t lcap = (int64_t)segcap * kShadeSegs;
                    uint32_t *keys = h->lit_row, *keys2 = h->lit_row + lcap, *vals = h->lit_flat + lcap;
                    if (staged)
                        hipLaunchKernelGGL(k_lit_stage, dim3(grid_for(n)), dim3(kBlock), 0, h->stream, h->S, B, L.rec,
                                           L.counts, h->shade_lit, h->shade_lcount, segcap, h->sort_light, keys, vals,
                                           h->lit_stage);
                    else
                        hipLaunchKernelGGL(k_lit_rows, dim3(grid_for(n)), dim3(kBlock), 0, h->stream, h->S, B, L.head,
                                           h->shade_lit, h->shade_lcount, segcap, h->sort_light, keys, vals);
                    auto& lc = h->host_lcount;
                    FRT_HIP(hipMemcpyAsync(lc.data(), h->shade_lcount, lc.size() * sizeof(unsigned), hipMemcpyDeviceToHost,
                                           h->stream));
                    FRT_HIP(stream_sync(h));
                    int64_t listed = 0;
                    for (int sgi = 0; sgi < kShadeSegs; ++sgi) listed += lc[(size_t)sgi * jit::kMixLine];
                    if (st != nullptr) st->lit_nodes += (uint64_t)listed;
                    if (listed > 0) {
                        size_t tmp_bytes = 0;
                        FRT_HIP(hipcub::DeviceRadixSort::SortPairs(nullptr, tmp_bytes, keys, keys2, vals, h->lit_flat,
                                                                   (int)listed, 0, row_bits, h->stream));
                        if (grow(&h->scan_tmp, h->scan_tmp_cap, (int64_t)tmp_bytes + 16)) return -1;
                        FRT_HIP(hipcub::DeviceRadixSort::SortPairs((void*)h->scan_tmp, tmp_bytes, keys, keys2, vals,
                                                                   h->lit_flat, (int)listed, 0, row_bits, h->stream));
                    }
                }
                if (split && st != nullptr && !sorted) {
                    auto& lc = h->host_lcount;
                    FRT_HIP(hipMemcpyAsync(lc.data(), h->shade_lcount, lc.size() * sizeof(unsigned), hipMemcpyDeviceToHost,
                                           h->stream));
                    FRT_HIP(hipStreamSynchronize(h->stream));
                    for (int sgi = 0; sgi < kShadeSegs; ++sgi) st->lit_nodes += lc[(size_t)sgi * jit::kMixLine];
                }
#ifndef FRT_SHADE_LIT_BLOCK
#define FRT_SHADE_LIT_BLOCK 64
#endif
                if (split && h->fast32) {
                    KTimer tl(h, st, 17);
                    hipLaunchKernelGGL(sorted ? k_shade_lit32<true> : k_shade_lit32<false>,
                                       dim3(grid_for(n, FRT_SHADE_LIT_BLOCK)), dim3(FRT_SHADE_LIT_BLOCK), 0, h->stream,
                                       h->S, B, L.rec, L.counts, L.surface, h->shade_lit, h->shade_lcount, segcap,
                                       sorted ? (const uint32_t*)h->lit_flat : nullptr,
                                       staged ? (const frt::LitStage*)h->lit_stage : nullptr,
                                       sorted_out ? L.spos : nullptr, h->light32);
                } else if (split) {
                    KTimer tl(h, st, 15);
                    hipLaunchKernelGGL(sorted ? k_shade_lit<true> : k_shade_lit<false>, dim3(grid_for(n, FRT_SHADE_LIT_BLOCK)),
                                       dim3(FRT_SHADE_LIT_BLOCK), 0,
                                       h->stream, h->S, B, L.rec, L.counts, L.surface, h->shade_lit, h->shade_lcount, segcap,
                                       sorted ? (const uint32_t*)h->lit_flat : nullptr,
                                       staged ? (const frt::LitStage*)h->lit_stage : nullptr,
                                       sorted_out ? L.spos : nullptr);
                }
                FRT_HIP(hipGetLastError());
            }
            if (h->S.cfg.use_gi) {
                KTimer t(h, st, 7);
                if (shade_gi(h, B, L, n, st)) return -1;
            }
            if (h->sync_epoch == counters_epoch) FRT_HIP(stream_sync(h));
            int64_t next = 0;
            bool overflow = false;
            for (int j = 0; j < kQueueSegs && !dense; ++j) {
                N.hprefix[j] = next;
                int64_t c = (int64_t)host_counters[(size_t)j * kCounterLine + d + 1];
                if (c > B.next_segcap) {
                    overflow = true;
                    c = B.next_segcap;
                }
                next += c;
            }
            if (dense) next = (int64_t)host_counters[20];
            N.hprefix[kQueueSegs] = next;
            if (overflow) {
                unsigned e = kErrQueueOverflow;
                FRT_HIP(hipMemcpyAsync(h->err, &e, sizeof(unsigned), hipMemcpyHostToDevice, h->stream));
            }
            if (next > 0 && d < path && !dense)
                FRT_HIP(hipMemcpyAsync(N.qprefix, N.hprefix.data(), (kQueueSegs + 1) * sizeof(int64_t), hipMemcpyHostToDevice,
                                       h->stream));
            count[d + 1] = d < path ? next : 0;
            int pbits = 1;
            while (pbits < 32 && (1ll << pbits) < n) ++pbits;
            N.sorted = dense || (h->queue_sort == 1 && d < path && next >= 4096 && !overflow && pbits < 32 &&
                                 N.cap <= (int64_t)UINT32_MAX);
            if (N.sorted && !dense) {
                KTimer t(h, st, 6);
                if (grow(&h->qsort, h->qsort_cap, 3 * next) || grow(&N.qperm, N.qperm_cap, next)) return -1;
                uint32_t *keys = h->qsort, *keys2 = h->qsort + next, *slots = h->qsort + 2 * next;
                Batch Bn = B;
                Bn.qprefix = N.qprefix;
                Bn.qsegcap = N.cap / kQueueSegs;
                Bn.qperm = nullptr;
                const int shift = std::min(h->queue_sort_shift, pbits - 1);
                hipLaunchKernelGGL(k_queue_keys, dim3(grid_for(next)), dim3(kBlock), 0, h->stream, Bn, N.q, next, pbits,
                                   shift, keys, slots);
                FRT_HIP(hipGetLastError());
                size_t tmp_bytes = 0;
                FRT_HIP(hipcub::DeviceRadixSort::SortPairs(nullptr, tmp_bytes, keys, keys2, slots, N.qperm, (int)next, 0,
                                                           pbits - shift + 1, h->stream));
                if (grow(&h->scan_tmp, h->scan_tmp_cap, (int64_t)tmp_bytes + 16)) return -1;
                FRT_HIP(hipcub::DeviceRadixSort::SortPairs((void*)h->scan_tmp, tmp_bytes, keys, keys2, slots, N.qperm,
                                                           (int)next, 0, pbits - shift + 1, h->stream));
            }
            if (st) {
                if (d > 0) st->secondary_rays += (uint64_t)n;
                else st->primary_rays += (uint64_t)n;
            }
        }
        const char* fuse_env = std::getenv("FRT_FUSE_RESOLVE");
        const bool fuse = spp <= kFuseBlock && !(fuse_env && std::strcmp(fuse_env, "0") == 0);
        const bool lazy = shade_lazy(h);
        for (int d = path; d >= 0; --d) {
            const int64_t n = count[d];
            if (n == 0) continue;
            if (d == 0 && fuse) {
                KTimer t(h, st, 4);
                const int32_t ppb = kFuseBlock / spp;
                hipLaunchKernelGGL(k_combine_resolve, dim3((unsigned)((bp + ppb - 1) / ppb)), dim3(kFuseBlock), 0, h->stream,
                                   h->S, lazy ? h->levels[0].counts : nullptr, h->levels[0].rec, n, h->levels[0].surface, h->levels[0].child, spp, ppb, bp,
                                   h->S.materials, h->S.cfg.include_specular, dev_out + 4 * p0,
                                   h->levels[0].staged ? (const uint32_t*)h->levels[0].spos : nullptr);
                FRT_HIP(hipGetLastError());
                continue;
            }
            KTimer t(h, st, 3);
            const Cols<Tri9> parent_child = d > 0 ? h->levels[d - 1].child : Cols<Tri9>{};
            hipLaunchKernelGGL(k_combine, dim3(grid_for(n)), dim3(kBlock), 0, h->stream, h->S,
                               lazy ? h->levels[d].counts : nullptr, h->levels[d].rec, n,
                               h->levels[d].surface, h->levels[d].child, parent_child, h->sample_col, spp,
                               h->S.materials, h->S.cfg.include_specular,
                               h->levels[d].staged ? (const uint32_t*)h->levels[d].spos : nullptr);
            FRT_HIP(hipGetLastError());
        }
        if (!fuse) {
            KTimer t(h, st, 4);
            hipLaunchKernelGGL(k_resolve, dim3((unsigned)((bp + 63) / 64)), dim3(kResolveBlock), 0, h->stream, h->sample_col, bp, spp,
                               dev_out + 4 * p0);
            FRT_HIP(hipGetLastError());
        }
    }
    FRT_HIP(hipMemcpyAsync(host_counters.data(), h->counters, host_counters.size() * sizeof(unsigned long long),
                           hipMemcpyDeviceToHost, h->stream));
    unsigned err = 0;
    FRT_HIP(hipMemcpyAsync(&err, h->err, sizeof(unsigned), hipMemcpyDeviceToHost, h->stream));
    if (st) (void)hipEventRecord(h->ev[1], h->stream);
    FRT_HIP(hipStreamSynchronize(h->stream));
    if (st) {
        float ms = 0.f;
        (void)hipEventElapsedTime(&ms, h->ev[0], h->ev[1]);
        st->render_ms = ms;
        uint64_t pruned = 0, hits = 0, uniform_waves = 0;
        for (int j = 0; j < kQueueSegs; ++j) {
            pruned += host_counters[(size_t)j * kCounterLine + 16];
            hits += host_counters[(size_t)j * kCounterLine + 17];
            uniform_waves += host_counters[(size_t)j * kCounterLine + 18];
        }
        st->prepare_uniform_waves = uniform_waves;
        st->pruned_secondary = pruned;
        st->hits = hits;
        st->shadow_rays = h->S.cfg.include_direct ? hits * (uint64_t)h->samples_per_node : 0;
        constexpr double kHead = (double)sizeof(frt::ShadowHead);
        bool multi = false;
        for (const auto& L : h->host_lights) multi = multi || L.rows > 1;
        st->shadow_kernel_bytes = !(h->S.cfg.include_direct && h->samples_per_node > 0) ? 0.0
                                  : h->jit_shadow != nullptr ? (double)h->pairs_walked * 8.0 + (double)h->heads_walked * (kHead + 4.0) +
                                                                   (multi ? 24.0 * (double)h->rays_walked : 0.0)
                                                             : (double)hits * (kHead + 4.0 * h->S.num_lights);
        st->errors = err;
        st->shadow_jit = h->jit_shadow != nullptr ? 1 : 0;
        st->shadow_rays_walked = h->jit_shadow != nullptr ? h->rays_walked : st->shadow_rays;
        st->shadow_tile_pairs = h->tile_pairs;
        st->shadow_tile_mixed = h->tile_mixed;
        st->shadow_pairs = h->node_pairs;
        st->shadow_pairs_mixed = h->node_mixed;
        st->shadow_sub_pairs = h->sub_pairs;
        st->shadow_sub_mixed = h->sub_mixed;
        st->shadow_subtile_pairs = h->subtile_pairs;
        st->shadow_subtile_mixed = h->subtile_mixed;
        collect_timings(h, st);
    }
#if defined(FRT_WALK_STATS) || defined(FRT_WALK_PROF)
    dump_walk_stats(h);
#endif
    if (err) {
        char buf[128];
        std::snprintf(buf, sizeof(buf), "render: device error bits 0x%x", err);
        return fail(buf);
    }
    return 0;
}

static int check_camera(const char* who, const frt_camera* cam) {
    const std::string w(who);
    if (cam->hsize <= 0 || cam->vsize <= 0)
        return fail(w + ": hsize and vsize must be positive (got " + std::to_string(cam->hsize) + " x " +
                    std::to_string(cam->vsize) + ")");
    if (cam->usteps <= 0 || cam->vsteps <= 0)
        return fail(w + ": usteps and vsteps must be positive (got " + std::to_string(cam->usteps) + " x " +
                    std::to_string(cam->vsteps) + ")");
    const int64_t kMaxSamples = (int64_t)1 << 52;
    if (cam->usteps > INT32_MAX / cam->vsteps)
        return fail(w + ": usteps * vsteps = " + std::to_string(cam->usteps) + " * " + std::to_string(cam->vsteps) +
                    " samples per pixel are more than the engine indexes (2^31 - 1)");
    const int64_t spp = cam->usteps * cam->vsteps;
    if (cam->hsize > kMaxSamples / spp || cam->vsize > kMaxSamples / spp / cam->hsize)
        return fail(w + ": " + std::to_string(cam->hsize) + " x " + std::to_string(cam->vsize) + " pixels of " +
                    std::to_string(spp) + " samples are more samples per frame than the engine indexes (2^52)");
    return 0;
}

int frt_scene_set_camera(frt_scene_handle* h, const frt_camera* cam, const double* sample_table) {
    if (!h || !cam) return fail("frt_scene_set_camera: null argument");
    if (check_camera("frt_scene_set_camera", cam)) return -1;
    if (!sample_table) return fail("frt_scene_set_camera: null sample table");
    const size_t nt = (size_t)(2 * cam->usteps * cam->vsteps);
    if (h->host_table.size() != nt || std::memcmp(h->host_table.data(), sample_table, nt * sizeof(double)) != 0) {
        FRT_HIP(hipSetDevice(h->device));
        void* p = nullptr;
        FRT_HIP(hipMalloc(&p, nt * sizeof(double)));
        const hipError_t e = hipMemcpy(p, sample_table, nt * sizeof(double), hipMemcpyHostToDevice);
        if (e != hipSuccess) {
            hip_ignore(hipFree(p));
            return fail(std::string("frt_scene_set_camera: hipMemcpy: ") + hipGetErrorString(e));
        }
        void* old = (void*)h->S.sample_table;
        auto at = old != nullptr ? std::find(h->owned.begin(), h->owned.end(), old) : h->owned.end();
        if (at != h->owned.end()) {
            *at = p;
            hip_ignore(hipFree(old));
        } else {
            h->owned.push_back(p);
        }
        h->S.sample_table = (const double*)p;
        h->host_table.assign(sample_table, sample_table + nt);
    }
    h->S.cam = *cam;
    return 0;
}

static int check_views(const char* who, const frt_scene_handle* h, const frt_camera* cams, int32_t nviews) {
    const std::string w(who);
    if (nviews <= 0) return fail(w + ": the number of views must be positive (got " + std::to_string(nviews) + ")");
    for (int32_t k = 0; k < nviews; ++k) {
        if (check_camera(who, cams + k)) return -1;
        const frt_camera &a = cams[0], &b = cams[k];
        if (a.hsize != b.hsize || a.vsize != b.vsize)
// ... 105 lines not shown
```

### fast_ray_tracer_amd/csrc/frt_jit.hip

```cpp
#include <hip/hip_runtime.h>
#include <hip/hiprtc.h>

#include <unistd.h>
#include <sys/stat.h>

#include <atomic>
#include <chrono>
#include <cmath>
#include <condition_variable>
#include <cstdio>
#include <cstdlib>
#include <cstring>
#include <functional>
#include <map>
#include <memory>
#include <mutex>
#include <set>
#include <thread>
#include <sstream>
#include <string>
#include <vector>

#include "frt_device.h"
#include "frt_jit.h"
// ... 1149 lines not shown
            o << "            if (ms && result != 1) {\n                amb = true;\n                alive = false;\n            }\n";
        o << "            if (alive && any_entry) alive = false;  // the first world shape with entries ends the walk\n";
        o << "        }\n";
    }
}

std::string frt_jit_shadow_source(const frt::WalkNode* wn, int num_nodes, const int32_t* roots, int num_roots,
                                  const frt_light* lights, int num_lights, std::string& why) {
    if (num_nodes > kMaxNodes) {
        why = "scene has more than " + std::to_string(kMaxNodes) + " nodes";
        return "";
    }
    if (num_lights < 1 || num_lights > kMaxLights) {
        why = "scene has " + std::to_string(num_lights) + " lights (the scene-specialised kernel takes 1.." +
              std::to_string(kMaxLights) + ")";
        return "";
    }
    Gen g;
    g.wn = wn;
    g.nn = num_nodes;
    g.stats = std::getenv("FRT_JIT_STATS") != nullptr;
    for (int ri = 0; ri < num_roots; ++ri)
        if (!g.check(roots[ri])) {
            why = g.why;
            return "";
        }
    LightTabs T;
    T.lights = lights;
    T.n = num_lights;
    T.start.assign((size_t)num_lights + 1, 0);
    T.rowbase.assign((size_t)num_lights + 1, 0);
    for (int l = 0; l < num_lights; ++l) {
        T.start[(size_t)l + 1] = T.start[(size_t)l] + lights[l].num_samples;
        T.rowbase[(size_t)l + 1] = T.rowbase[(size_t)l] + std::max(1, lights[l].rows);
        T.multi_row = T.multi_row || lights[l].rows > 1;
    }
    T.parts.assign((size_t)num_lights, 0);
    T.partbase.assign((size_t)num_lights + 1, 0);
    T.boxbase.assign((size_t)num_lights + 1, 0);
    for (int l = 0; l < num_lights; ++l) {
        T.parts[(size_t)l] = std::max<int64_t>(1, (lights[l].num_samples + frt_jit_part_size() - 1) / frt_jit_part_size());
        T.partbase[(size_t)l + 1] = T.partbase[(size_t)l] + T.parts[(size_t)l];
        T.boxbase[(size_t)l + 1] = T.boxbase[(size_t)l] + T.parts[(size_t)l] * std::max(1, lights[l].rows);
    }
    T.np = T.partbase[(size_t)num_lights];
    const std::string NP = std::to_string(T.np) + "u";
    const std::string NL = std::to_string(num_lights) + "u";
    std::ostringstream& o = g.o;
    header(o);

    const int TS = frt_jit_tile_size();
    int TSL = 0;
    while ((1 << TSL) < TS) ++TSL;
    const bool resume = std::getenv("FRT_JIT_RESUME") == nullptr || std::atoi(std::getenv("FRT_JIT_RESUME")) != 0;
    if (resume && !(std::getenv("FRT_JIT_FLAGS") && std::atoi(std::getenv("FRT_JIT_FLAGS")) == 0)) g.assign_flags();
    const bool stats_on = g.stats;
    const int u32_mode = std::getenv("FRT_JIT_U32") ? std::atoi(std::getenv("FRT_JIT_U32")) : 1;
    const int order_mode = std::getenv("FRT_JIT_ORDER") ? std::atoi(std::getenv("FRT_JIT_ORDER")) : 1;
    const int SQ = TS > 0 ? frt_jit_sub_count() : 0;
    int SQL = 0;
    while ((1 << SQL) < SQ) ++SQL;
    const bool st_on = !T.multi_row || std::getenv("FRT_JIT_SUBTILE") != nullptr;
    const int ST = SQ > 0 && st_on && frt_jit_subtile_size() < TS ? frt_jit_subtile_size() : 0;
    const int NST = ST ? TS / ST : 0;
    int STL = 0, NSTL = 0;
    while (ST && (1 << STL) < ST) ++STL;
    while (NST && (1 << NSTL) < NST) ++NSTL;
    const int PS = frt_jit_part_size();
    const int PS2 = SQ ? frt_jit_sub_ps(PS, SQ) : 0;
    int NM = T.multi_row ? 4 : 1;
    if (const char* e = std::getenv("FRT_JIT_NODE_MAJOR")) NM = std::atoi(e);
    if (NM < 1 || NM > 64 || (NM & (NM - 1)) != 0) NM = 1;
    std::string subn;
    for (int l = 0; SQ && l < num_lights; ++l)
        for (int64_t p = 0; p < T.parts[(size_t)l]; ++p) {
            const int c = p + 1 < T.parts[(size_t)l] ? PS : lights[l].num_samples - (int)p * PS;
            for (int x : frt_jit_sub_sizes(std::max(c, 0), SQ)) subn += (subn.empty() ? "" : ", ") + std::to_string(x);
        }
    auto pair_kernel = [&](int mode) {
        const char* name = mode == 0 ? "frt_jit_beam" : mode == 1 ? "frt_jit_tile" : mode == 2 ? "frt_jit_beam_list"
                         : mode == 3 ? "frt_jit_sub" : "frt_jit_subtile";
        const bool boxed = mode == 1 || mode == 3 || mode == 4;
        o << "extern \"C\" __global__ void __launch_bounds__(kTraceBlock)" << waves_attr("FRT_JIT_BEAM_WAVES") << "\n"
          << name << "(DevScene S, Batch B, const ShadowHead* __restrict__ shead, uint32_t nlanes, uint32_t nnodes,\n"
             "             const float* __restrict__ tbox, const uint32_t* __restrict__ tlist, jit::SegTable seg,\n"
             "             uint32_t b0, uint32_t tsegcap,\n"
             "             const float* __restrict__ laabb, int32_t* __restrict__ counts, uint32_t* __restrict__ mixed,\n"
             "             unsigned* __restrict__ mcount, uint32_t segcap, unsigned* __restrict__ err,\n"
             "             unsigned long long* __restrict__ jstats, const int32_t* __restrict__ psamp2) {\n"
             "    const uint32_t tid = blockIdx.x * blockDim.x + threadIdx.x;\n";
        for (int k = 0; k < num_nodes; ++k) g.node32(k, "    ");
        o << "    uint32_t node = 0, gp = 0, pp = 0, tile = 0;\n"
             "    bool live = false;\n"
             "    uint32_t START = 0, FLAGS = 0;  // (frt_jit_beam_list: the tile's resume point and flags)\n"
             "    bool START_ANY = false;\n"
          << (boxed ? "    jit::BeamBox32 W;\n" : "    jit::Beam32 W;\n");
        if (mode == 0) {
            o << "    bool in = tid < nlanes;\n"
                 "    if (in) {\n"
                 "        node = tid / " << NP << ";\n"
                 "        gp = tid - node * " << NP << ";\n"
                 "    }\n";
        } else if (mode == 1) {
            o << "    bool in = tid < nlanes;\n"
                 "    if (in) {\n"
                 "        tile = tid / " << NP << ";\n"
                 "        gp = tid - tile * " << NP << ";\n"
                 "    }\n";
        } else if (mode == 3) {
            o << "    constexpr int32_t SUBN[] = {" << subn << "};\n"
                 "    bool in = false;\n"
                 "    uint32_t q = 0;\n"
                 "    {\n"
                 "        const uint32_t gb = b0 + blockIdx.x;\n"
                 "        const int sg = jit::seg_of_block(seg, gb);\n"
                 "        const uint32_t u = (gb - seg.bstart[sg]) * blockDim.x + threadIdx.x;\n"
                 "        const uint32_t mi = u >> " << SQL << ";\n"
                 "        q = u & " << (SQ - 1) << "u;\n"
                 "        if (mi < seg.count[sg]) {\n"
                 "            const size_t slot = (size_t)sg * tsegcap + mi;\n"
                 "            const uint32_t entry = tlist[slot];\n"
                 "            const uint32_t rsv = tlist[(size_t)jit::kMixSegs * tsegcap + slot];\n"
                 "            START = rsv & " << ((1u << kStartBits) - 1) << "u;\n"
                 "            FLAGS = rsv & " << (0x7fffffffu & ~((1u << kStartBits) - 1)) << "u;\n"
                 "            START_ANY = (rsv >> 31) != 0;\n"
                 "            tile = entry / " << NP << ";\n"
                 "            gp = entry - tile * " << NP << ";\n"
                 "            in = (tile << " << TSL << ") < nnodes && SUBN[gp * " << SQ << "u + q] > 0;\n"
                 "        }\n"
                 "    }\n";
        } else {
            const int LL = mode == 4 ? NSTL : ST ? STL : TSL;
            if (SQ) o << "    constexpr int32_t SUBN[] = {" << subn << "};\n";
            o << "    bool in = false;\n"
                 "    uint32_t q = 0, st = 0;\n"
                 "    {\n"
                 "        const uint32_t gb = b0 + blockIdx.x;\n"
                 "        const int sg = jit::seg_of_block(seg, gb);\n"
                 "        const uint32_t u = (gb - seg.bstart[sg]) * blockDim.x + threadIdx.x;\n"
                 "        const uint32_t mi = u >> " << LL << ";\n"
                 "        if (mi < seg.count[sg]) {\n"
                 "            const size_t slot = (size_t)sg * tsegcap + mi;\n"
                 "            const uint32_t entry = tlist[slot];\n"
                 "            const uint32_t rsv = tlist[(size_t)jit::kMixSegs * tsegcap + slot];\n"
                 "            START = rsv & " << ((1u << kStartBits) - 1) << "u;\n"
                 "            FLAGS = rsv & " << (0x7fffffffu & ~((1u << kStartBits) - 1)) << "u;\n"
                 "            START_ANY = (rsv >> 31) != 0;\n"
                 "            // (SQ: tile sub-pairs (tile pair) * SQ + q; mode 2 after the sub-tile kernel: times NST plus\n"
                 "            // the sub-tile; mode 4: its lanes' sub-tiles)\n"
                 "            const uint32_t e2 = entry >> " << (mode == 2 ? NSTL : 0) << ";\n"
                 "            st = " << (mode == 4 ? "u & " + std::to_string(std::max(NST - 1, 0)) + "u"
                                       : "entry & " + std::to_string(mode == 2 ? std::max(NST - 1, 0) : 0) + "u") << ";\n"
                 "            const uint32_t tp = e2 >> " << SQL << ";\n"
                 "            q = e2 & " << std::max(SQ - 1, 0) << "u;\n"
                 "            tile = tp / " << NP << ";\n"
                 "            gp = tp - tile * " << NP << ";\n";
            if (mode == 4)
                o << "            node = (tile << " << TSL << ") + (st << " << STL << ");  // (the sub-tile's first)\n";
            else if (ST)
                o << "            node = (tile << " << TSL << ") + (st << " << STL << ") + (u & " << (ST - 1) << "u);\n";
            else
                o << "            node = (tile << " << TSL << ") + (u & " << (TS - 1) << "u);\n";
            o << "            in = node < nnodes;\n"
                 "        }\n"
                 "    }\n";
        }
        T.light_of_part(o, "gp", "    ");
        o << "    pp = gp - " << T.partbase_of() << ";\n"
             "    if (in) {\n";
        if (boxed) {
            if (mode != 1)
                o << "        const float* bx = laabb + 6 * ((size_t)gp * " << SQ << "u + q);\n";
            else
                o << "        const float* bx = laabb + 6 * (" << (T.multi_row ? T.boxbase[(size_t)num_lights] : 0)
                  << "LL + (int64_t)gp);\n";
            if (mode == 4)
                o << "        live = jit::beam_box32(tbox + 6 * ((size_t)tile * " << NST << "u + st), bx, bx + 3, W);  // (false: no live node)\n";
            else
                o << "        live = jit::beam_box32(tbox + 6 * (size_t)tile, bx, bx + 3, W);  // (false: no live node in the tile)\n";
        } else {
            o << "        const ShadowHead* nr = shead + node;\n"
                 "        live = nr->material >= 0;\n"
                 "        if (live) {\n";
            if (T.multi_row)
                o << "            const int row = light_row_n(" << T.rows() << ", B.seed, nr->key, lt, 0);\n";
            else
                o << "            const int row = 0;\n";
            if (mode == 2 && SQ && T.multi_row) {
                o << "            float bl[3] = {__builtin_huge_valf(), __builtin_huge_valf(), __builtin_huge_valf()};\n"
                     "            float bh[3] = {-__builtin_huge_valf(), -__builtin_huge_valf(), -__builtin_huge_valf()};\n"
                     "            const double* rp = S.light_points + " << T.points() << " + 3 * ((int64_t)row * " << T.ns()
                  << ");\n"
                     "            for (uint32_t k = 0; k < " << PS2 << "u; ++k) {\n"
                     "                const int32_t js = psamp2[((size_t)gp * " << SQ << "u + q) * " << PS2 << "u + k];\n"
                     "                if (js < 0) break;\n"
                     "                for (int a = 0; a < 3; ++a) {\n"
                     "                    bl[a] = fminf(bl[a], __double2float_rd(rp[3 * js + a]));\n"
                     "                    bh[a] = fmaxf(bh[a], __double2float_ru(rp[3 * js + a]));\n"
                     "                }\n"
                     "            }\n"
                     "            jit::beam32(nr->over_point, bl, bh, W);\n";
            } else {
                if (mode == 2 && SQ)
                    o << "            const float* bx = laabb + 6 * ((size_t)gp * " << SQ << "u + q);\n";
                else
                    o << "            const float* bx = laabb + 6 * (" << T.boxbase_of() << " + (int64_t)row * " << T.nparts()
                      << " + pp);\n";
                o << "            jit::beam32(nr->over_point, bx, bx + 3, W);\n";
            }
            o << "        }\n";
        }
        o << "    }\n"
             "    bool alive = live;\n"
             "    bool amb = false;  // a pair the beam cannot decide: mixed\n"
             "    bool ms = false;  // a sphere that may block some of the rays was passed (sphere_beam32 == 2)\n"
             "    int result = 0;\n"
             "    uint32_t RS = START;  // the next kernel's resume point for this pair (Gen::track_start)\n"
             "    bool RS_ANY = START_ANY;\n"
             "    {  // the interval walk on the beam (s = t / |D|: DIST = 1)\n"
             "        const jit::Iv DIST{1.0f - 1e-7f, 1.0f + 1e-7f};\n";
        g.beam = true;
        g.order_opt = order_mode == 2 || (order_mode == 1 && boxed);
        g.u32 = u32_mode >= 1;
        g.beam_stats = stats_on;
        g.stats = false;
        g.track_start = resume;
        g.gate_start = (mode == 2 || mode == 3 || mode == 4) && resume;
        g.JS = boxed ? "jstats + 1024 + 6144" : "jstats + 1024";
        walk32(g, roots, num_roots);
        g.JS = "jstats + 1024";
        g.beam = false;
        g.order_opt = false;
        g.track_start = false;
        g.gate_start = false;
        g.stats = stats_on;
        o << "    }\n";
        const std::string cnt = "(int32_t)min(" + std::to_string(frt_jit_part_size()) + "u, " + T.ns() + " - pp * " +
                                std::to_string(frt_jit_part_size()) + "u)";
        const std::string rsv = "RS | FLAGS | (RS_ANY ? 0x80000000u : 0u)";
        const bool run_counts = !(std::getenv("FRT_JIT_RUN_COUNTS") && std::atoi(std::getenv("FRT_JIT_RUN_COUNTS")) == 0);
        if (mode == 1 && run_counts) {
            o << "    // the part's samples are unshadowed from every node of the tile (summed over the wave's lanes of the tile)\n"
                 "    jit::add_run_counts(shead, counts, " << NL << ", live && !amb && result == 0, tile << " << TSL << ", "
              << TS << "u, (uint32_t)lt, " << cnt << ", nnodes);\n"
                 "    jit::mix_append(live && amb, tile * " << NP << " + gp, " << rsv << ", mixed, mcount, segcap, err);\n"
                 "    if (jstats != nullptr) {  // diagnostics (FRT_JIT_STATS): tile pairs / mixed tile pairs\n"
                 "        unsigned long long* line = jstats + 32 * (blockIdx.x % 64);\n"
                 "        wave_count(line + 4, live);\n"
                 "        wave_count(line + 5, live && amb);\n"
                 "    }\n"
                 "}\n\n";
        } else if (mode == 3 && run_counts) {
            o << "    // the sub-part's samples are unshadowed from every node of the tile (summed over the tile's lanes)\n"
                 "    jit::add_run_counts(shead, counts, " << NL << ", live && !amb && result == 0, tile << " << TSL << ", "
              << TS << "u, (uint32_t)lt, in ? SUBN[gp * " << SQ << "u + q] : 0, nnodes);\n"
                 "    jit::mix_append(live && amb, (tile * " << NP << " + gp) * " << SQ << "u + q, " << rsv
              << ", mixed, mcount, segcap, err);\n"
                 "    if (jstats != nullptr) {  // diagnostics (FRT_JIT_STATS): sub-part pairs / mixed ones\n"
                 "        unsigned long long* line = jstats + 32 * (blockIdx.x % 64);\n"
                 "        wave_count(line + 6, live);\n"
                 "        wave_count(line + 7, live && amb);\n"
                 "    }\n"
                 "}\n\n";
        } else if (mode == 4 && run_counts) {
            o << "    // the sub-part's samples are unshadowed from every node of the sub-tile (summed over its lanes)\n"
                 "    jit::add_run_counts(shead, counts, " << NL << ", live && !amb && result == 0, node, " << ST
              << "u, (uint32_t)lt, in ? SUBN[gp * " << SQ << "u + q] : 0, nnodes);\n"
                 "    jit::mix_append(live && amb, (((tile * " << NP << " + gp) * " << SQ << "u + q) << " << NSTL << ") + st, "
              << rsv << ", mixed, mcount, segcap, err);\n"
                 "    if (jstats != nullptr) {  // diagnostics (FRT_JIT_STATS): sub-tile pairs / mixed ones\n"
                 "        unsigned long long* line = jstats + 32 * (blockIdx.x % 64);\n"
                 "        wave_count(line + 8, live);\n"
                 "        wave_count(line + 9, live && amb);\n"
                 "    }\n"
                 "}\n\n";
        } else if (mode == 1) {
            o << "    if (live && !amb && result == 0) {  // the part's samples are unshadowed from every node of the tile\n"
                 "        for (uint32_t n = 0; n < " << TS << "u; ++n) {\n"
                 "            const uint32_t nd = (tile << " << TSL << ") + n;\n"
                 "            if (nd < nnodes && shead[nd].material >= 0) atomicAdd(counts + nd * " << NL << " + (uint32_t)lt, " << cnt << ");\n"
                 "        }\n"
                 "    }\n"
                 "    jit::mix_append(live && amb, tile * " << NP << " + gp, " << rsv << ", mixed, mcount, segcap, err);\n"
                 "    if (jstats != nullptr) {  // diagnostics (FRT_JIT_STATS): tile pairs / mixed tile pairs\n"
                 "        unsigned long long* line = jstats + 32 * (blockIdx.x % 64);\n"
                 "        wave_count(line + 4, live);\n"
                 "        wave_count(line + 5, live && amb);\n"
                 "    }\n"
                 "}\n\n";
        } else if (mode == 3) {
            o << "    if (live && !amb && result == 0) {  // the sub-part's samples are unshadowed from every node of the tile\n"
                 "        for (uint32_t n = 0; n < " << TS << "u; ++n) {\n"
                 "            const uint32_t nd = (tile << " << TSL << ") + n;\n"
                 "            if (nd < nnodes && shead[nd].material >= 0) atomicAdd(counts + nd * " << NL
              << " + (uint32_t)lt, SUBN[gp * " << SQ << "u + q]);\n"
                 "        }\n"
                 "    }\n"
                 "    jit::mix_append(live && amb, (tile * " << NP << " + gp) * " << SQ << "u + q, " << rsv
              << ", mixed, mcount, segcap, err);\n"
                 "    if (jstats != nullptr) {  // diagnostics (FRT_JIT_STATS): sub-part pairs / mixed ones\n"
                 "        unsigned long long* line = jstats + 32 * (blockIdx.x % 64);\n"
                 "        wave_count(line + 6, live);\n"
                 "        wave_count(line + 7, live && amb);\n"
                 "    }\n"
                 "}\n\n";
        } else if (mode == 4) {
            o << "    if (live && !amb && result == 0) {  // the sub-part's samples are unshadowed from every node of the sub-tile\n"
                 "        for (uint32_t n = 0; n < " << ST << "u; ++n) {\n"
                 "            const uint32_t nd = node + n;\n"
                 "            if (nd < nnodes && shead[nd].material >= 0) atomicAdd(counts + nd * " << NL
              << " + (uint32_t)lt, SUBN[gp * " << SQ << "u + q]);\n"
                 "        }\n"
                 "    }\n"
                 "    jit::mix_append(live && amb, (((tile * " << NP << " + gp) * " << SQ << "u + q) << " << NSTL << ") + st, "
              << rsv << ", mixed, mcount, segcap, err);\n"
                 "    if (jstats != nullptr) {  // diagnostics (FRT_JIT_STATS): sub-tile pairs / mixed ones\n"
                 "        unsigned long long* line = jstats + 32 * (blockIdx.x % 64);\n"
                 "        wave_count(line + 8, live);\n"
                 "        wave_count(line + 9, live && amb);\n"
                 "    }\n"
                 "}\n\n";
        } else if (mode == 2 && SQ) {
            o << "    if (live && !amb && result == 0)  // the sub-part's samples are all unshadowed\n"
                 "        atomicAdd(counts + node * " << NL << " + (uint32_t)lt, SUBN[gp * " << SQ << "u + q]);\n"
                 "    jit::mix_append(live && amb, (node * " << NP << " + gp) * " << SQ << "u + q, " << rsv
              << ", mixed, mcount, segcap, err);\n"
                 "    if (jstats != nullptr) {  // diagnostics (FRT_JIT_STATS): pairs / mixed pairs\n"
                 "        unsigned long long* line = jstats + 32 * (blockIdx.x % 64);\n"
                 "        wave_count(line + 2, live);\n"
                 "        wave_count(line + 3, live && amb);\n"
                 "    }\n"
                 "}\n\n";
        } else {
            o << "    if (live && !amb && result == 0)  // the part's samples are all unshadowed\n"
                 "        atomicAdd(counts + node * " << NL << " + (uint32_t)lt, " << cnt << ");\n"
                 "    jit::mix_append(live && amb, node * " << NP << " + gp, " << rsv << ", mixed, mcount, segcap, err);\n"
                 "    if (jstats != nullptr) {  // diagnostics (FRT_JIT_STATS): pairs / mixed pairs\n"
                 "        unsigned long long* line = jstats + 32 * (blockIdx.x % 64);\n"
                 "        wave_count(line + 2, live);\n"
                 "        wave_count(line + 3, live && amb);\n"
                 "    }\n"
                 "}\n\n";
        }
    };
    pair_kernel(0);
    if (TS > 0) {
        pair_kernel(1);
        pair_kernel(2);
    }
    if (SQ > 0) pair_kernel(3);
    if (ST > 0) pair_kernel(4);
    g.u32 = u32_mode >= 2;

    o << "extern \"C\" __global__ void __launch_bounds__(kTraceBlock)" << waves_attr("FRT_JIT_WAVES") << "\n"
         "frt_jit_shadow(DevScene S, Batch B, const ShadowHead* __restrict__ shead, uint32_t total, uint32_t m0,\n"
         "               const uint32_t* __restrict__ mixed, jit::SegTable seg, uint32_t b0, uint32_t segcap,\n"
         "               uint32_t all_pairs, const int32_t* __restrict__ psamp, uint32_t subq,\n"
         "               const int32_t* __restrict__ psamp2,\n"
         "               uint32_t lpp, uint64_t magic, uint32_t shift, uint32_t spn,\n"
         "               int32_t* __restrict__ counts, int64_t* __restrict__ redo, unsigned* __restrict__ redo_count,\n"
         "               unsigned redo_cap, unsigned* __restrict__ err, unsigned long long* __restrict__ jstats,\n"
         "               uint32_t nnodes) {\n"
         "    const uint32_t tid = blockIdx.x * blockDim.x + threadIdx.x;\n";
    for (int k = 0; k < num_nodes; ++k) g.node32(k, "    ");
    o << "    jit::Lane32 L;\n"
         "    uint32_t START = 0;  // first node whose subtree this lane walks (the pair kernel's resume point)\n"
         "    bool START_ANY = false;\n"
         "    uint32_t FLAGS = 0;  // boxes every ray of the lane's pair enters (Gen::fbit)\n"
         "    L.valid = L.live = false;\n"
         "    L.node = 0;\n"
         "    L.light = 0;\n"
         "    L.lp = L.op = nullptr;\n"
         "    double LP[3] = {0.0, 0.0, 0.0}, OP[3] = {0.0, 0.0, 0.0};\n"
         "    uint32_t jall = 0;  // the sample's index among the node's spn samples (k_shadow_redo's lane)\n"
         "    uint32_t j = 0;  // the lane's sample within its part\n"
         "    {\n"
         "        // every pair in order (all_pairs: no pair kernel ran; lanes tid of pairs m0 + tid / lpp) or the\n"
         "        // mixed ones (the block's segment of the list, jit::SegTable)\n"
         "        uint32_t u = tid;\n"
         "        int sg = 0;\n"
         "        if (!all_pairs) {\n"
         "            const uint32_t gb = b0 + blockIdx.x;\n"
         "            sg = jit::seg_of_block(seg, gb);\n"
         "            u = (gb - seg.bstart[sg]) * blockDim.x + threadIdx.x;\n"
         "        }\n"
         "        uint32_t mi = (uint32_t)(((uint64_t)u * magic) >> shift);  // u / lpp\n"
         "        j = u - mi * lpp;\n";
    if (NM > 1)
        o << "        if (subq >= 2 && !all_pairs) {\n"
             "            // node-major lanes (a multi-row light): groups of " << NM << " consecutive list entries, lane w of a\n"
             "            // group = (entry w % kg, node lane w / kg), so a node's samples of the group's entries sit side by\n"
             "            // side and read its own light row together (kg: the group's entries, fewer in the last group)\n"
             "            const uint32_t cnt = seg.count[sg], grp = " << NM << "u * lpp, gi = u / grp, w = u - gi * grp;\n"
             "            const uint32_t base = gi * " << NM << "u;\n"
             "            const uint32_t kg = cnt > base ? min(" << NM << "u, cnt - base) : " << NM << "u;\n"
             "            const uint32_t jn = w / kg;\n"
             "            mi = u < cnt * lpp ? base + (w - jn * kg) : cnt;\n"
             "            j = jn;\n"
             "        }\n";
    o << "        const size_t slot = (size_t)sg * segcap + mi;\n"
         "        if (all_pairs ? tid < total : mi < seg.count[sg]) {\n"
         "            const uint32_t pair = all_pairs ? m0 + mi : mixed[slot];\n"
         "            const uint32_t rsv = all_pairs ? 0u : mixed[(size_t)jit::kMixSegs * segcap + slot];  // resume point\n"
         "            START = rsv & " << ((1u << kStartBits) - 1) << "u;\n"
         "            FLAGS = rsv & " << (0x7fffffffu & ~((1u << kStartBits) - 1)) << "u;\n"
         "            START_ANY = (rsv >> 31) != 0;\n"
         "            // subq 0: (node, part) pairs; 1: sub-part pairs (node pair) * SQ + q (frt_jit_beam_list after\n"
         "            // frt_jit_sub); 2 / 3: the entries frt_jit_sub / frt_jit_subtile leave, walked here without the node\n"
         "            // pair kernel: a tile's (sub-tile's) nodes times the sub-part's samples, the node's samples consecutive\n"
         "            uint32_t gp = 0, q = 0;\n"
         "            if (subq >= 2) {\n"
         "                const uint32_t nn = j / " << std::max(PS2, 1) << "u;\n"
         "                j -= nn * " << std::max(PS2, 1) << "u;\n"
         "                const uint32_t e2 = subq == 3 ? pair >> " << NSTL << " : pair;\n"
         "                const uint32_t tp = e2 >> " << SQL << ";\n"
         "                q = e2 & " << std::max(SQ - 1, 0) << "u;\n"
         "                const uint32_t tile = tp / " << NP << ";\n"
         "                gp = tp - tile * " << NP << ";\n"
         "                L.node = (tile << " << TSL << ") + (subq == 3 ? (pair & " << std::max(NST - 1, 0) << "u) << " << STL
      << " : 0u) + nn;\n"
         "            } else {\n"
         "                const uint32_t npair = subq ? pair >> " << SQL << " : pair;\n"
         "                L.node = npair / " << NP << ";\n"
         "                gp = npair - L.node * " << NP << ";\n"
         "                q = pair & " << std::max(SQ - 1, 0) << "u;\n"
         "            }\n";
    T.light_of_part(o, "gp", "            ");
    o << "            const int32_t jp = subq ? psamp2[(gp * " << std::max(SQ, 1) << "u + q) * " << std::max(PS2, 1)
      << "u + j] : psamp[gp * " << frt_jit_part_size() << "u + j];  // the light's sample (-1: none)\n"
         "            const uint32_t js = (uint32_t)max(jp, 0);\n"
         "            const bool in_range = L.node < nnodes;  // (a tile's nodes past the batch's last)\n"
         "            L.light = lt;\n"
         "            L.valid = jp >= 0 && in_range;\n"
         "            jall = " << T.first() << " + js;\n"
         "            const ShadowHead* nr = shead + (in_range ? L.node : 0u);\n"
         "            if (L.valid && nr->material >= 0) {\n"
         "                L.live = true;\n";
    if (T.multi_row)
        o << "                const int row = light_row_n(" << T.rows() << ", B.seed, nr->key, lt, 0);\n";
    else
        o << "                const int row = 0;\n";
    o << "                L.lp = S.light_points + " << T.points() << " + 3 * ((int64_t)row * " << T.ns() << " + js);\n"
         "                L.op = nr->over_point;\n"
         "                for (int a = 0; a < 3; ++a) {\n"
         "                    LP[a] = L.lp[a];\n"
         "                    OP[a] = L.op[a];\n"
         "                }\n"
         "            }\n"
         "        }\n"
         "    }\n"
         "    bool alive = L.live;\n"
         "    bool handed = false;\n"
         "    int shadowed = 0;\n"
         "    bool amb = false;  // a lane whose binary32 walk met an undecidable comparison\n"
         "    {  // binary32 interval walk\n"
         "        int result = 0;\n"
         "        jit::World32 W;\n"
         "        jit::Iv DIST{0.0f, 0.0f};\n"
         "        Ray R64 = Ray{{0, 0, 0}, {0, 0, 1}};  // the binary64 ray, once a leaf needs it\n"
         "        double D64 = 0.0;\n"
         "        bool have64 = false;\n";
    const int nowalk = std::getenv("FRT_JIT_DBG_NOWALK") ? std::atoi(std::getenv("FRT_JIT_DBG_NOWALK")) : 0;
    if (nowalk == 1) o << "        alive = false;\n";
    o << "        if (alive && !jit::ray32v(LP, OP, W, DIST)) {  // no binary32 bounds for this ray: binary64 walk\n"
         "            amb = true;\n"
         "            alive = false;\n"
         "        }\n";
    if (nowalk == 2) o << "        if (__builtin_amdgcn_readfirstlane(__float_as_int(W.P[0] + W.Q[2] + DIST.hi)) == 1) atomicOr(err, 0u);\n"
                          "        alive = false;\n";
    g.gate_start = resume;
    walk32(g, roots, num_roots);
    g.gate_start = false;
    o << "        shadowed = result;\n    }\n";
    o << "    if (__ballot(amb)) {  // the reference's binary64 arithmetic for those lanes\n"
         "        Ray R0 = Ray{{0, 0, 0}, {0, 0, 1}};\n"
         "        double dist = 0.0;\n"
         "        if (amb) jit::ray64(L, R0, dist);\n"
         "        if (amb && !jit::finite_ray(R0, dist)) {  // to the generic walk (k_shadow_redo)\n"
         "            amb = false;\n"
         "            handed = true;\n"
         "            const unsigned at = atomicAdd(redo_count, 1u);\n"
         "            if (at < redo_cap) redo[at] = (int64_t)L.node * spn + jall;\n"
         "            else atomicOr(err, kErrQueueOverflow);\n"
         "        }\n"
         "        bool alive = amb;\n"
         "        int result = 0;\n";
    for (int ri = 0; ri < num_roots; ++ri) {
        o << "        // ---- world shape " << ri << " (node " << roots[ri] << ")\n";
        o << "        if (__ballot(alive)) {\n";
        o << "            bool any_entry = false;\n";
        g.top(roots[ri], "true", "R0", ri == num_roots - 1, "            ");
        o << "            if (alive && any_entry) alive = false;\n";
        o << "        }\n";
    }
    o << "        if (amb) shadowed = result;\n    }\n";
    o << "    if (jstats != nullptr) {  // diagnostics (FRT_JIT_STATS): live lanes / lanes re-walked in binary64\n"
         "        unsigned long long* line = jstats + 32 * (blockIdx.x % 64);\n"
         "        wave_count(line, L.live);\n"
         "        wave_count(line + 1, amb);\n"
         "    }\n";
    if (NM > 1)
        o << "    if (subq >= 2 && !all_pairs) jit::count_runs(S, L, L.live && !handed && shadowed == 0, counts);\n    else\n";
    o << "    jit::count_part(S, L, L.live && !handed && shadowed == 0, j, subq >= 2 ? " << std::max(PS2, 1)
      << "u : lpp, counts);\n}\n";

    bool closest = std::getenv("FRT_JIT_TRACE") == nullptr || std::atoi(std::getenv("FRT_JIT_TRACE")) != 0;
    for (int ri = 0; closest && ri < num_roots; ++ri) closest = g.closest_ok(roots[ri]);
    if (closest) {
        g.u32 = false;
        g.stats = false;
        g.beam = false;
        g.track_start = g.gate_start = false;
        o << "extern \"C\" __global__ void __launch_bounds__(kTraceBlock)" << waves_attr("FRT_JIT_TRACE_WAVES") << "\n"
             "frt_jit_trace(DevScene S, Batch B, const QueuedRay* __restrict__ q, int64_t n, HitRec* __restrict__ hits,\n"
             "              unsigned* __restrict__ err, int32_t* __restrict__ redo, unsigned* __restrict__ redo_count,\n"
             "              unsigned redo_cap) {\n"
             "    const int64_t i = (int64_t)blockIdx.x * blockDim.x + threadIdx.x;\n";
        for (int k = 0; k < num_nodes; ++k) g.node32(k, "    ");
        o << "    const bool live = i < n && (q == nullptr || q[queue_slot(B, i)].parent >= -1);\n"
             "    Ray ray{{0, 0, 0}, {0, 0, 1}};\n"
             "    unsigned e = 0;\n"
             "    if (live) {\n"
             "        if (q == nullptr) {\n"
             "            uint64_t key;\n"
             "            camera_ray(S, B, i, ray, key, e);\n"
             "        } else {\n"
             "            const QueuedRay& qr = q[queue_slot(B, i)];\n"
             "            for (int a = 0; a < 3; ++a) {\n"
             "                ray.o[a] = qr.o[a];\n"
             "                ray.d[a] = qr.d[a];\n"
             "            }\n"
             "        }\n"
             "    }\n"
             "    bool alive = live, amb = false;\n"
             "    jit::World32 W;\n"
             "    if (alive && !jit::ray32d(ray, W)) {  // no binary32 bounds for this ray: the generic walk\n"
             "        amb = true;\n"
             "        alive = false;\n"
             "    }\n";
        g.trace_dbg = std::getenv("FRT_JIT_TRACE_DBG") != nullptr;
        if (g.trace_dbg)
            o << "    const bool dbgl = live && (i == 0 || i == " << std::atoll(std::getenv("FRT_JIT_TRACE_DBG")) << "ll);\n"
                 "    if (dbgl) printf(\"frt_jit_trace i %lld o %a %a %a d %a %a %a amb %d\\n\", (long long)i, ray.o[0], ray.o[1],"
                 " ray.o[2], ray.d[0], ray.d[1], ray.d[2], (int)amb);\n";
        o <<
             "    // (the binary64 ray for the leaves evaluated exactly; the shadow walk's lane state, unused)\n"
             "    const Ray R0 = ray;\n"
             "    jit::Lane32 L;\n"
             "    L.live = L.valid = false;\n"
             "    L.lp = L.op = nullptr;\n"
             "    bool have64 = true;\n"
             "    Ray R64 = ray;\n"
             "    double D64 = 0.0;\n"
             "    jit::Iv BT{0.0f, 0.0f};  // the best entry so far (bk < 0: none)\n"
             "    int bk = -1, bj = 0;\n";
        for (int ri = 0; ri < num_roots; ++ri) {
            o << "    // ---- world shape " << ri << " (node " << roots[ri] << ")\n";
            o << "    if (__ballot(alive)) {\n";
            g.slots.clear();
            g.topc(roots[ri], "true", "", "        ");
            o << "    }\n";
        }
        o << "    // the winner's binary64 t: its own leaf's entries (the same arithmetic as the generic walk's)\n"
             "    double t = 0.0;\n"
             "    if (!amb && bk >= 0) {\n"
             "        switch (bk) {\n";
        for (int k = 0; k < num_nodes; ++k) {
            if (composite(wn[k].type)) continue;
            o << "        case " << k << ": {\n";
            g.chain(k, false, "rl", "            ");
            o << "            t = jit::leaf_entry<" << type_name(wn[k].type) << ", " << (wn[k].has_xf ? "true" : "false")
              << ">(S, S.wn[" << k << "], rl, bj);\n            break;\n        }\n";
        }
        o << "        default: break;\n"
             "        }\n"
             "    }\n"
             "    // the undecided rays to the list, one atomic per wave\n"
             "    const bool rd = i < n && amb;\n"
             "    const unsigned long long m = __ballot(rd);\n"
             "    if (m) {\n"
             "        const int lane = (int)(threadIdx.x & 63), leader = __builtin_ctzll(m);\n"
             "        unsigned base = 0;\n"
             "        if (lane == leader) base = atomicAdd(redo_count, (unsigned)__popcll(m));\n"
             "        const unsigned at = __builtin_amdgcn_readlane(base, leader) + (unsigned)__popcll(m & ((1ull << lane) - 1));\n"
             "        if (rd) {\n"
             "            if (at < redo_cap) redo[at] = (int32_t)i;\n"
             "            else atomicOr(err, kErrQueueOverflow);\n"
             "        }\n"
             "    }\n"
             "    if (i < n && !amb) hits[i] = live && bk >= 0 ? HitRec{t, bk, 0} : HitRec{0.0, -1, 0};\n"
             "    if (e) atomicOr(err, e);\n"
             "}\n";
    }
    return o.str();
}

static int compile_code(const std::string& src, const std::string& arch, std::vector<char>& code, std::string& log) {
    hiprtcProgram prog;
    const int nh = (int)(sizeof(kJitHeaderNames) / sizeof(kJitHeaderNames[0]));
    if (hiprtcCreateProgram(&prog, src.c_str(), "frt_jit_shadow.hip", nh, kJitHeaderSrc, kJitHeaderNames) !=
        HIPRTC_SUCCESS) {
        log = "hiprtcCreateProgram failed";
        return -1;
    }
    const std::string off = "--offload-arch=" + arch;
    const char* opts[] = {off.c_str(), kJitOpts[0], kJitOpts[1], kJitOpts[2]};
    g_stat[0]++;
    const hiprtcResult rc = hiprtcCompileProgram(prog, 4, opts);
    size_t ls = 0;
    hiprtcGetProgramLogSize(prog, &ls);
    if (ls > 1) {
        log.assign(ls, '\0');
        hiprtcGetProgramLog(prog, &log[0]);
    }
    if (rc != HIPRTC_SUCCESS) {
        hiprtcDestroyProgram(&prog);
        return -1;
    }
    size_t cs = 0;
    hiprtcGetCodeSize(prog, &cs);
    code.resize(cs);
    hiprtcGetCode(prog, code.data());
    hiprtcDestroyProgram(&prog);
    if (const char* co = std::getenv("FRT_JIT_CO")) {
        if (FILE* f = std::fopen(co, "wb")) {
            std::fwrite(code.data(), 1, code.size(), f);
            std::fclose(f);
        }
    }
    return 0;
}

int frt_jit_compile_only(const std::string& src, const std::string& arch, std::string& log) {
// ... 150 lines not shown
```

### fast_ray_tracer_amd/csrc/frt_jit_rt.hpp

```cpp
#pragma once

#include "frt_shadow.hpp"

namespace frt {
namespace jit {

__device__ __forceinline__ bool box_enter(const WalkNode& nd, const Ray& lr, bool skip_behind) {
    Frame32 lf;
    frame32(lr, lf);
    float tmin32 = -1.0f, tmax32 = 1.0f, err32 = 0.0f;
    const int dec = lf.exact ? -1 : box32(nd.bb32, nd.bmag, lf, tmin32, tmax32, err32);
    double tmin = -1.0, tmax = 1.0;
    bool enter;
    if (dec >= 0) {
        enter = dec != 0;
        tmax = (double)tmax32 + (double)err32;
    } else if (origin_inside(nd.bbox, lr)) {
        enter = true;
    } else {
        double lrc[3];
#pragma unroll
        for (int a = 0; a < 3; ++a) lrc[a] = recip<1>(lr.d[a]);
        enter = box_decide(nd.bbox, lr, lrc, tmin, tmax);
    }
    if (skip_behind && behind(tmax)) enter = false;
    return enter;
}

template <int kType, bool kXf>
__device__ __forceinline__ void leaf_top(const DevScene& S, const WalkNode& nd, const Ray& R, double dist, bool act,
                                         bool& alive, int& result, bool& any_entry) {
    const Ray lr = kXf ? xf_ray_walk(nd.m, R) : R;
    LeafHits H;
    if (kType == FRT_CUBE) cube_hits_for_decisions(lr, dist, H);
    else leaf_hits<true>(kType, S.prim + nd.prim, lr, H);
    if (act && H.t.n > 0) {
        any_entry = true;
        bool stop_here = false, blocked = false;
#pragma unroll
        for (int j = 0; j < 4; ++j) {
            const double t = H.t.at(j);
            if (j < H.t.n) {
                stop_here = stop_here || !(t <= 0);
                blocked = blocked || (t > 0 && t < dist);
            }
        }
        if (stop_here) {
            result = blocked && nd.casts ? 1 : 0;
            alive = false;
        }
    }
}

template <int kType, bool kXf>
__device__ __forceinline__ void leaf_slots(const DevScene& S, const WalkNode& nd, const Ray& R, bool act, double& t0,
                                           double& t1, bool& v0, bool& v1) {
    const Ray lr = kXf ? xf_ray_walk(nd.m, R) : R;
    LeafHits H;
    leaf_hits<true>(kType, S.prim + nd.prim, lr, H);
    t0 = H.t.v0;
    t1 = H.t.v1;
    v0 = act && H.t.n > 0;
    v1 = act && H.t.n > 1;
}

template <int kOp>
__device__ __forceinline__ bool allowed(bool lhit, bool inl, bool inr) {
    if (kOp == 0) return lhit ? !inr : !inl;
    if (kOp == 1) return lhit ? inr : inl;
    return lhit ? !inr : inl;
}

__device__ __forceinline__ bool finite_ray(const Ray& r, double dist) {
    bool f = __builtin_isfinite(dist);
#pragma unroll
    for (int a = 0; a < 3; ++a) f = f && __builtin_isfinite(r.o[a]) && __builtin_isfinite(r.d[a]);
    return f;
}

constexpr float kU = 0x1p-24f;
constexpr float kXfErr = 6.0f * kU;
constexpr float kXfErrD = 12.0f * kU;
constexpr float kSlabRel = 7.0f * kU;
constexpr float kSlack = 1.01f;
constexpr float kAaK1 = 2.5f * kU;
constexpr float kAaK0 = 12.0f * kU;

struct Iv {
    float lo, hi;
};

__device__ __forceinline__ int iv_le(const Iv& a, const Iv& b) { return a.hi <= b.lo ? 1 : (a.lo > b.hi ? 0 : -1); }
__device__ __forceinline__ int iv_le0(const Iv& a) { return a.hi <= 0.0f ? 1 : (a.lo > 0.0f ? 0 : -1); }
__device__ __forceinline__ int iv_lt(const Iv& a, const Iv& b) { return a.hi < b.lo ? 1 : (a.lo >= b.hi ? 0 : -1); }

__device__ __forceinline__ Iv iv_of(double x) { return Iv{__double2float_rd(x), __double2float_ru(x)}; }

struct World32 {
    float o[3], d[3], omax;
    float r[3], ro[3], P[3], Q[3];
};

struct Node32 {
    float cm[12];
    float cN, cT;
    float bb32[6], bmag[3];
    float aab[6], aathr[3], aabmax, aasig;
    float sph[4], sphc;
    int casts;
};

__device__ __forceinline__ float o_lo(const World32& w, int a) { return w.o[a]; }
__device__ __forceinline__ float o_hi(const World32& w, int a) { return w.o[a]; }

__device__ __forceinline__ void world32_finish(World32& w) {
    w.omax = fmaxf(fmaxf(fabsf(w.o[0]), fabsf(w.o[1])), fabsf(w.o[2]));
#pragma unroll
    for (int a = 0; a < 3; ++a) {
        w.r[a] = __builtin_amdgcn_rcpf(w.d[a]);
        w.ro[a] = w.o[a] * w.r[a];
        w.P[a] = kAaK0 * fabsf(w.r[a]);
        w.Q[a] = w.P[a] * w.omax;
    }
}

struct Lane32 {
    uint32_t node;
    int light;
    bool valid, live;
    const double* lp;
    const double* op;
};

__device__ __forceinline__ void lane32(const DevScene& S, const Batch& B, const ShadowHead* __restrict__ shead,
                                       uint32_t total, const int32_t* __restrict__ j_light,
                                       const int32_t* __restrict__ j_point, uint32_t spn, uint64_t magic,
                                       uint32_t shift, uint32_t tid, Lane32& L) {
    L.valid = tid < total;
    L.live = false;
    L.node = 0;
    L.light = 0;
    L.lp = L.op = nullptr;
    if (L.valid) {
        L.node = (uint32_t)(((uint64_t)tid * magic) >> shift);
        const uint32_t j = tid - L.node * spn;
        L.light = j_light[j];
        const int pt = j_point[j];
        const ShadowHead* nr = shead + L.node;
        if (nr->material >= 0) {
            L.live = true;
            const frt_light& lt = S.lights[L.light];
            const int row = light_row(lt, B.seed, nr->key, L.light, 0);
            L.lp = S.light_points + lt.points + 3 * ((int64_t)row * lt.num_samples + pt);
            L.op = nr->over_point;
        }
    }
}

__device__ __forceinline__ bool ray32v(const double* lp, const double* op, World32& w, Iv& dist) {
    float vf[3];
#pragma unroll
    for (int a = 0; a < 3; ++a) {
        vf[a] = (float)(lp[a] - op[a]);
        w.o[a] = (float)op[a];
    }
    const float n2 = vf[0] * vf[0] + vf[1] * vf[1] + vf[2] * vf[2];
    const float rs = __builtin_amdgcn_rsqf(n2);
#pragma unroll
    for (int a = 0; a < 3; ++a) w.d[a] = vf[a] * rs;
    const float dl = n2 * rs;
    dist = Iv{dl * (1.0f - 8.0f * kU), dl * (1.0f + 8.0f * kU)};
    world32_finish(w);
    return n2 >= 0x1p-60f && n2 <= 0x1p100f && w.omax <= 0x1p100f;
}

__device__ __forceinline__ bool ray32(const Lane32& L, World32& w, Iv& dist) { return ray32v(L.lp, L.op, w, dist); }

__device__ __forceinline__ bool ray32d(const Ray& r, World32& w) {
#pragma unroll
    for (int a = 0; a < 3; ++a) {
        w.o[a] = (float)r.o[a];
        w.d[a] = (float)r.d[a];
    }
    world32_finish(w);
    const double n2 = r.d[0] * r.d[0] + r.d[1] * r.d[1] + r.d[2] * r.d[2];
    return n2 > 1.0 - 1e-6 && n2 < 1.0 + 1e-6 && w.omax <= 0x1p100f;
}

__device__ __forceinline__ void ray64(const Lane32& L, Ray& r, double& dist) {
    if (!L.live) {
        r = Ray{{0, 0, 0}, {0, 0, 1}};
        dist = 0.0;
        return;
    }
    double v[3];
#pragma unroll
    for (int a = 0; a < 3; ++a) {
        v[a] = L.lp[a] - L.op[a];
        r.o[a] = L.op[a];
    }
    dist = sqrt(v[0] * v[0] + v[1] * v[1] + v[2] * v[2]);
    normalize3(v, r.d);
}

__device__ __forceinline__ void ray64_once(const Lane32& L, bool& have, Ray& r, double& dist) {
    if (!have) {
        ray64(L, r, dist);
        have = true;
    }
}

constexpr int kMixSegs = 64;
constexpr int kMixLine = 64;

__device__ __forceinline__ void mix_append(bool mix, uint32_t pair, uint32_t value, uint32_t* __restrict__ mixed,
                                           unsigned* __restrict__ mcount, uint32_t segcap, unsigned* __restrict__ err) {
    const unsigned long long mm = __ballot(mix);
    if (mm == 0) return;
    const int lane = threadIdx.x & 63;
    const int seg = (int)(blockIdx.x % kMixSegs);
    unsigned base = 0;
    if (lane == 0) base = atomicAdd(mcount + seg * kMixLine, (unsigned)__popcll(mm));
    base = __shfl(base, 0, 64);
    if (mix) {
        const unsigned at = base + (unsigned)__popcll(mm & ((1ull << lane) - 1));
        if (at < segcap) {
            mixed[(size_t)seg * segcap + at] = pair;
            mixed[(size_t)kMixSegs * segcap + (size_t)seg * segcap + at] = value;
        } else {
            atomicOr(err, kErrQueueOverflow);
        }
    }
}

struct SegTable {
    uint32_t bstart[kMixSegs + 1];
    uint32_t count[kMixSegs];
};

__device__ __forceinline__ int seg_of_block(const SegTable& t, uint32_t gb) {
    int s = 0;
#pragma unroll
    for (int step = 32; step > 0; step >>= 1)
        if (t.bstart[s + step] <= gb) s += step;
    return s;
}

__device__ __forceinline__ void count_part(const DevScene& S, const Lane32& L, bool lit, uint32_t j, uint32_t lpp,
                                           int32_t* counts) {
    const int lane = threadIdx.x & 63;
    const unsigned long long lits = __ballot(lit);
    if (L.valid && (j == 0 || lane == 0)) {
        const uint32_t len = min(lpp - j, 64u - (uint32_t)lane);
        const unsigned long long seg = (len >= 64u ? ~0ull : ((1ull << len) - 1ull)) << lane;
        const int c = __popcll(lits & seg);
        if (c) atomicAdd(counts + L.node * (uint32_t)S.num_lights + (uint32_t)L.light, c);
    }
}

__device__ __forceinline__ void add_run_counts(const ShadowHead* __restrict__ shead, int32_t* counts, uint32_t nl,
                                               bool add, uint32_t base, uint32_t len, uint32_t lt, int32_t amount,
                                               uint32_t nnodes) {
    const int lane = threadIdx.x & 63;
    unsigned long long pending = __ballot(add);
    while (pending) {
        const int ld = __builtin_ctzll(pending);
        const uint32_t b0 = (uint32_t)__builtin_amdgcn_readlane((int)base, ld);
        const uint32_t l0 = (uint32_t)__builtin_amdgcn_readlane((int)lt, ld);
        const bool same = add && base == b0 && lt == l0;
        pending &= ~__ballot(same);
        int32_t v = same ? amount : 0;
#pragma unroll
        for (int o = 32; o > 0; o >>= 1) v += __shfl_xor(v, o, 64);
        for (uint32_t n = (uint32_t)lane; n < len; n += 64u) {
            const uint32_t nd = b0 + n;
            if (nd < nnodes && shead[nd].material >= 0) atomicAdd(counts + nd * nl + l0, v);
        }
    }
}

__device__ __forceinline__ void count_runs(const DevScene& S, const Lane32& L, bool lit, int32_t* counts) {
    const int lane = threadIdx.x & 63;
    const unsigned long long lits = __ballot(lit), valid = __ballot(L.valid);
    const uint32_t key = L.node * (uint32_t)S.num_lights + (uint32_t)L.light;
    const uint32_t prev = __shfl_up(key, 1, 64);
    const bool prev_valid = lane > 0 && ((valid >> (lane - 1)) & 1ull);
    const bool head = L.valid && (!prev_valid || prev != key);
    const unsigned long long heads = __ballot(head);
    if (head) {
        const unsigned long long after = lane == 63 ? 0ull : (~0ull << (lane + 1));
        const unsigned long long stops = (heads | ~valid) & after;
        const int next = stops ? __ffsll((long long)stops) - 1 : 64;
        const unsigned long long run = (next >= 64 ? ~0ull : ((1ull << next) - 1ull)) & (~0ull << lane);
        const int c = __popcll(lits & run);
        if (c) atomicAdd(counts + key, c);
    }
}

__device__ __forceinline__ size_t mix_slot(uint32_t m, const unsigned* __restrict__ mcount, uint32_t segcap) {
    const int lane = threadIdx.x & 63;
    const unsigned c = min(mcount[lane * kMixLine], segcap);
    unsigned incl = c;
#pragma unroll
    for (int o = 1; o < 64; o <<= 1) {
        const unsigned t = __shfl_up(incl, o, 64);
        if (lane >= o) incl += t;
    }
    const unsigned excl = incl - c;
    int lo = 0;
#pragma unroll
    for (int step = 32; step > 0; step >>= 1) {
        const int probe = lo + step;
        const unsigned e = __shfl(excl, probe & 63, 64);
        if (probe < 64 && e <= m) lo = probe;
    }
    return (size_t)lo * segcap + (m - __shfl(excl, lo, 64));
}

__device__ __forceinline__ void node_stat(unsigned long long* js, int k, bool act) {
    const unsigned long long m = __ballot(act);
    if ((threadIdx.x & 63) == 0) {
        atomicAdd(js + 2048 + 2 * k, 1ull);
        atomicAdd(js + 2048 + 2 * k + 1, (unsigned long long)__popcll(m));
    }
}

struct F32 {
    float o[3], d[3], eo, ed;
};

__device__ __forceinline__ void frame32i(const Node32& nd, const World32& w, F32& f) {
#pragma unroll
    for (int r = 0; r < 3; ++r) {
        const float* c = nd.cm + 4 * r;
        f.o[r] = fmaf(c[0], w.o[0], fmaf(c[1], w.o[1], fmaf(c[2], w.o[2], c[3])));
        f.d[r] = fmaf(c[0], w.d[0], fmaf(c[1], w.d[1], c[2] * w.d[2]));
    }
    f.eo = kXfErr * fmaf(nd.cN, w.omax, nd.cT);
    f.ed = kXfErrD * nd.cN;
}

typedef float f2 __attribute__((ext_vector_type(2)));
template <bool kSig>
__device__ __forceinline__ bool aa_slab(const Node32& nd, const World32& w, Iv& tmin, Iv& tmax) {
    bool ok = true;
    f2 lo = {0.0f, 0.0f}, hi = {0.0f, 0.0f};
#pragma unroll
    for (int a = 0; a < 3; ++a) {
        ok = ok && fabsf(w.d[a]) >= nd.aathr[a];
        const f2 B = {nd.aab[a], nd.aab[a + 3]};
        const f2 t = __builtin_elementwise_fma(B, f2{w.r[a], w.r[a]}, f2{-w.ro[a], -w.ro[a]});
        const float k1 = kSig ? fmaf(nd.aasig, fabsf(w.r[a]), kAaK1) : kAaK1;
        const float bm = fmaxf(fabsf(nd.aab[a]), fabsf(nd.aab[a + 3])) * (1.0f + 4.0f * kU);
        const float e = fmaf(fmaxf(fabsf(t.x), fabsf(t.y)), k1, fmaf(bm, w.P[a], w.Q[a]));
        const f2 m = {fminf(t.x, t.y), fmaxf(t.x, t.y)};
        const f2 l = m - f2{e, e}, h = m + f2{e, e};
        if (a == 0) {
            lo = l;
            hi = h;
// ... 554 lines not shown
```

### fast_ray_tracer_amd/csrc/frt_shadow.hpp

```cpp
#pragma once

#include "frt_traverse.hpp"

namespace frt {

__device__ __forceinline__ uint64_t mix64(uint64_t x) {
    x ^= x >> 30;
    x *= 0xbf58476d1ce4e5b9ULL;
    x ^= x >> 27;
    x *= 0x94d049bb133111ebULL;
    x ^= x >> 31;
    return x;
}

__device__ __forceinline__ int light_row_n(int rows, uint64_t seed, uint64_t key, int light, int draw) {
    if (rows <= 1) return 0;
    uint64_t h = mix64(seed ^ mix64(key * 0x9e3779b97f4a7c15ULL + (uint64_t)(light * 2 + draw + 1)));
    return (int)(h % (uint64_t)rows);
}

__device__ __forceinline__ int light_row(const frt_light& L, uint64_t seed, uint64_t key, int light, int draw) {
    return light_row_n(L.rows, seed, key, light, draw);
}

constexpr int kQueueSegs = 64;
constexpr int kCounterLine = 32;

struct Batch {
    int64_t sample_begin;
    int64_t pixel_begin;
    int64_t num_samples;
    int64_t row_begin, row_stride;
    uint64_t seed;
    int32_t spp, level;
    int32_t remaining;
    int32_t stats;
    const int64_t* qprefix;
    int64_t qsegcap;
    int64_t next_segcap;
    const uint32_t* qperm;
};

__device__ __forceinline__ int64_t queue_slot(const Batch& B, int64_t i) {
    if (B.qperm != nullptr) return B.qperm[i];
    if (B.qprefix == nullptr) return i;
    int lo = 0, hi = kQueueSegs;
    while (hi - lo > 1) {
        const int mid = (lo + hi) >> 1;
        if (B.qprefix[mid] <= i) lo = mid;
        else hi = mid;
    }
    return (int64_t)lo * B.qsegcap + (i - B.qprefix[lo]);
}

struct alignas(8) ShadowHead {
    double over_point[3];
    uint64_t key;
    int32_t material;
    int32_t pad;
};
static_assert(sizeof(ShadowHead) == 40, "ShadowHead layout");

struct ShadowLane {
    Ray r;
    double distance;
    int64_t node;
    int light;
    bool valid;
    bool live;
};

__device__ __forceinline__ void shadow_lane(const DevScene& S, const Batch& B, const ShadowHead* __restrict__ shead,
                                            int64_t n, const int32_t* __restrict__ j_light,
                                            const int32_t* __restrict__ j_point, int32_t samples_per_node,
                                            int64_t tid, ShadowLane& L) {
    L.valid = tid >= 0 && tid < n * samples_per_node;
    L.node = 0;
    L.light = 0;
    L.live = false;
    L.r = Ray{{0, 0, 0}, {0, 0, 1}};
    L.distance = 0.0;
    if (L.valid) {
        L.node = tid / samples_per_node;
        const int j = (int)(tid % samples_per_node);
        L.light = j_light[j];
        const int pt = j_point[j];
        const ShadowHead* nr = shead + L.node;
        if (nr->material >= 0) {
            L.live = true;
            const frt_light& lt = S.lights[L.light];
            const int row = light_row(lt, B.seed, nr->key, L.light, 0);
            const double* lp = S.light_points + lt.points + 3 * ((int64_t)row * lt.num_samples + pt);
            double v[3] = {lp[0] - nr->over_point[0], lp[1] - nr->over_point[1], lp[2] - nr->over_point[2]};
            L.distance = sqrt(v[0] * v[0] + v[1] * v[1] + v[2] * v[2]);
            L.r.o[0] = nr->over_point[0];
            L.r.o[1] = nr->over_point[1];
            L.r.o[2] = nr->over_point[2];
            normalize3(v, L.r.d);
        }
    }
}

__device__ __forceinline__ void shadow_count(const DevScene& S, const ShadowLane& L, bool lit, int32_t* counts) {
    const int lane = threadIdx.x & 63;
    const int64_t key = L.valid ? L.node * S.num_lights + L.light : -1 - (int64_t)lane;
    const int64_t prev = __shfl_up(key, 1, 64);
    const bool head = lane == 0 || prev != key;
    const unsigned long long heads = __ballot(head);
    const unsigned long long lits = __ballot(lit);
    if (L.valid && head) {
        const unsigned long long above = lane == 63 ? 0ull : (heads >> (lane + 1)) << (lane + 1);
        const int next = above ? __ffsll((long long)above) - 1 : 64;
        const unsigned long long seg = (next >= 64 ? ~0ull : ((1ull << next) - 1)) & ~((1ull << lane) - 1);
        const int c = __popcll(lits & seg);
        if (c) atomicAdd(counts + key, c);
    }
}

}
```

Measured before the change: 507,600.

## Split shadow head records into columnar arrays and recompute camera keys

Replaces the 40-byte array-of-structs ShadowHead with a structure-of-arrays HeadCols. Over-points sit in three column arrays, the hit test reads the existing material word in the node core columns, and keys are stored only when needed. For level 0 without GI or multi-row lights, the key is rebuilt from the camera sample index instead of being stored. This cuts write and read traffic for shadow heads in prepare, shadow and lit kernels and makes those accesses coalesced, at the cost of extra index arithmetic and a few more separate loads per lane.

```diff
diff --git a/fast_ray_tracer_amd/csrc/frt_camera.hpp b/fast_ray_tracer_amd/csrc/frt_camera.hpp
--- a/fast_ray_tracer_amd/csrc/frt_camera.hpp
+++ b/fast_ray_tracer_amd/csrc/frt_camera.hpp
@@ -105,26 +105,42 @@
     normalize3(v, r.d);
 }
 
+struct CameraSample {
+    int64_t row, col;
+    uint64_t global_pixel, global_sample;
+    int sub;
+};
+__device__ __forceinline__ CameraSample camera_sample(const DevScene& S, const Batch& B, int64_t s) {
+    CameraSample c;
+    const int64_t pix = B.pixel_begin + s / B.spp;
+    c.sub = (int)(s % B.spp);
+    const int64_t hs = S.cam.hsize;
+    c.row = B.row_begin + (pix / hs) * B.row_stride;
+    c.col = pix % hs;
+    c.global_pixel = (uint64_t)(c.row * hs + c.col);
+    c.global_sample = c.global_pixel * (uint64_t)B.spp + (uint64_t)c.sub;
+    return c;
+}
+
+__device__ __forceinline__ uint64_t camera_key(const DevScene& S, const Batch& B, int64_t s) {
+    return (camera_sample(S, B, s).global_sample << 12) | 1ull;
+}
+
 __device__ __forceinline__ void camera_ray(const DevScene& S, const Batch& B, int64_t s, Ray& r, uint64_t& key,
                                            unsigned& err) {
-    const int64_t pix = B.pixel_begin + s / B.spp;
-    const int sub = (int)(s % B.spp);
-    const int64_t hs = S.cam.hsize;
-    const int64_t row = B.row_begin + (pix / hs) * B.row_stride;
-    const int64_t col = pix % hs;
-    const uint64_t global_pixel = (uint64_t)(row * hs + col);
-    const uint64_t global_sample = global_pixel * (uint64_t)B.spp + (uint64_t)sub;
+    const CameraSample c = camera_sample(S, B, s);
+    const int sub = c.sub;
     double jit[2], ap[2] = {0.5, 0.5};
     if (S.cam.jitter) {
         const int U = (int)S.cam.usteps, V = (int)S.cam.vsteps;
-        cmj_point(B.seed, global_pixel, U, V, sub % U, sub / U, jit);
+        cmj_point(B.seed, c.global_pixel, U, V, sub % U, sub / U, jit);
     } else {
         jit[0] = S.sample_table[2 * sub];
         jit[1] = S.sample_table[2 * sub + 1];
     }
-    if (S.cam.aperture_size != 0.0) aperture_point(S.cam, B.seed, global_sample, ap, err);
-    ray_for_pixel(S.cam, (double)col, (double)row, jit, ap, r);
-    key = (global_sample << 12) | 1ull;
+    if (S.cam.aperture_size != 0.0) aperture_point(S.cam, B.seed, c.global_sample, ap, err);
+    ray_for_pixel(S.cam, (double)c.col, (double)c.row, jit, ap, r);
+    key = (c.global_sample << 12) | 1ull;
 }
 
 }
diff --git a/fast_ray_tracer_amd/csrc/frt_engine.hip b/fast_ray_tracer_amd/csrc/frt_engine.hip
--- a/fast_ray_tracer_amd/csrc/frt_engine.hip
+++ b/fast_ray_tracer_amd/csrc/frt_engine.hip
@@ -62,7 +62,7 @@
 struct NodeCols {
     Cols<NodeCore> core;
     Cols<NodeColors> col;
-    const ShadowHead* head = nullptr;
+    HeadCols head;
     int32_t root = 0;
     int32_t eye_cam = 0;
     static size_t bytes(int64_t cap) { return Cols<NodeCore>::bytes(cap) + Cols<NodeColors>::bytes(cap); }
@@ -131,13 +131,12 @@
         NodeCore c;
         __builtin_memcpy(&c, t, sizeof(c));
         NodeRec v;
-        const ShadowHead& hd = head[i];
+        head.over_point(i, v.over_point);
         for (int k = 0; k < 3; ++k) {
-            v.over_point[k] = hd.over_point[k];
             v.normalv[k] = c.normalv[k];
             v.eyev[k] = c.eyev[k];
         }
-        v.key = hd.key;
+        v.key = head.key != nullptr ? head.key[i] : 0ull;
         v.material = c.material;
         v.parent = c.parent;
         v.slot = c.slot;
@@ -167,6 +166,9 @@
             v.Ns = M.Ns;
         }
         return v;
+    }
+    __device__ __forceinline__ uint64_t key(const DevScene& S, const Batch& B, int64_t i) const {
+        return head_key(S, B, head, i);
     }
 };
 
@@ -258,8 +260,7 @@
 template <bool kPat>
 __device__ __forceinline__ bool prepare_node(const DevScene& S, const Batch& B, const QueuedRay* __restrict__ q,
                                              int64_t n, const HitRec* __restrict__ hits, const double* __restrict__ hn12,
-                                             NodeCols& rec,
-                                             ShadowHead* __restrict__ heads, QueuedRay* __restrict__ next_q,
+                                             NodeCols& rec, QueuedRay* __restrict__ next_q,
                                              unsigned long long* counters, unsigned* err, int64_t node, double* op,
                                              int* spawned, int uniform_ok) {
     unsigned long long* line = counters + kCounterLine * (blockIdx.x % kQueueSegs);
@@ -296,7 +297,6 @@
     PSTAMP(1);
     if (hr.node < 0) {
         rec.store_miss(node, parent, slot);
-        heads[node].material = -1;
         return false;
     }
     auto prepare_hit = [&](const DevScene& S, const int leaf) __attribute__((always_inline)) {
@@ -403,22 +403,9 @@
     PSTAMP(3);
     const bool own = kPat && (M.map_Ka >= 0 || M.map_Kd >= 0 || M.map_Ks >= 0 || M.map_refl >= 0 || M.map_Ns >= 0);
     rec.store(node, nr, own, kPat && M.map_d >= 0);
-    ShadowHead hd;
-    for (int k = 0; k < 3; ++k) hd.over_point[k] = c.over_point[k];
-    hd.key = key;
-    hd.material = c.material;
-    hd.pad = 0;
-#ifdef FRT_EXPERIMENT_HEAD_COLS
-    {
-        uint64_t t[5];
-        __builtin_memcpy(t, &hd, sizeof(hd));
-        uint64_t* w = (uint64_t*)heads;
 #pragma unroll
-        for (int f = 0; f < 5; ++f) w[(int64_t)f * n + node] = t[f];
-    }
-#else
-    heads[node] = hd;
-#endif
+    for (int k = 0; k < 3; ++k) rec.head.op[k * rec.head.cap + node] = c.over_point[k];
+    if (rec.head.key != nullptr) rec.head.key[node] = key;
     PSTAMP(4);
     for (int k = 0; k < 3; ++k) op[k] = c.over_point[k];
     };
@@ -471,7 +458,7 @@
 __global__ void __launch_bounds__(kBlock) __attribute__((amdgpu_waves_per_eu(kPat ? 1 : FRT_PREPARE_WAVES, 8)))
 k_prepare(DevScene S, Batch B, const QueuedRay* __restrict__ q, int64_t n, const HitRec* __restrict__ hits,
           const double* __restrict__ hn12,
-          NodeCols rec, ShadowHead* __restrict__ heads, QueuedRay* __restrict__ next_q, unsigned long long* counters,
+          NodeCols rec, QueuedRay* __restrict__ next_q, unsigned long long* counters,
           unsigned* err, float* __restrict__ tbox, int tile_log2, float* __restrict__ stbox, int sub_log2,
           int32_t* __restrict__ counts, unsigned long long* __restrict__ spawn_masks, int uniform_ok) {
     const int64_t node = (int64_t)blockIdx.x * blockDim.x + threadIdx.x;
@@ -481,7 +468,7 @@
         for (int l = 0; l < S.num_lights; ++l) counts[node * S.num_lights + l] = 0;
     int spawned = 0;
     if (node < n)
-        hit = prepare_node<kPat>(S, B, q, n, hits, hn12, rec, heads, next_q, counters, err, node, op,
+        hit = prepare_node<kPat>(S, B, q, n, hits, hn12, rec, next_q, counters, err, node, op,
                                  spawn_masks != nullptr ? &spawned : nullptr, uniform_ok);
     if (spawn_masks != nullptr) {
         const unsigned long long mr = __ballot(spawned & 1), mt = __ballot((spawned >> 1) & 1);
@@ -500,7 +487,7 @@
 #define FRT_SHADOW_ATTR
 #endif
 template <int kFeat>
-__global__ void __launch_bounds__(kTraceBlock) FRT_SHADOW_ATTR k_shadow(DevScene S, Batch B, const ShadowHead* __restrict__ shead, int64_t n,
+__global__ void __launch_bounds__(kTraceBlock) FRT_SHADOW_ATTR k_shadow(DevScene S, Batch B, const HeadCols shead, int64_t n,
                                                         const int32_t* __restrict__ j_light,
                                                         const int32_t* __restrict__ j_point, int32_t samples_per_node,
                                                         int32_t* __restrict__ counts, unsigned* err) {
@@ -518,7 +505,7 @@
 }
 
 template <int kFeat>
-__global__ void __launch_bounds__(kTraceBlock) k_shadow_redo(DevScene S, Batch B, const ShadowHead* __restrict__ shead, int64_t n,
+__global__ void __launch_bounds__(kTraceBlock) k_shadow_redo(DevScene S, Batch B, const HeadCols shead, int64_t n,
                                                              const int32_t* __restrict__ j_light,
                                                              const int32_t* __restrict__ j_point, int32_t samples_per_node,
                                                              int32_t* __restrict__ counts, unsigned* err,
@@ -993,6 +980,7 @@
     NodeRec nr{};
     if (i < n) {
         nr = rec.load(i, S.materials);
+        if (!kLazy) nr.key = rec.key(S, B, i);
         mine = nr.material >= 0;
         heavy = mine && lit != nullptr && shade_heavy(S, counts, i);
     }
@@ -1059,7 +1047,7 @@
     return __shfl(incl, 63, 64);
 }
 
-__global__ void __launch_bounds__(kBlock) k_lit_rows(DevScene S, Batch B, const ShadowHead* __restrict__ head,
+__global__ void __launch_bounds__(kBlock) k_lit_rows(DevScene S, Batch B, const HeadCols head,
                                                      const uint32_t* __restrict__ lit, const unsigned* __restrict__ lcount,
                                                      uint32_t segcap, int sort_light, uint32_t* __restrict__ rows,
                                                      uint32_t* __restrict__ nodes) {
@@ -1069,7 +1057,7 @@
     const size_t slot = jit::mix_slot(m < total ? m : 0u, lcount, segcap);
     if (m >= total) return;
     const uint32_t i = lit[slot];
-    rows[m] = (uint32_t)light_row(S.lights[sort_light], B.seed, head[i].key, sort_light, 1);
+    rows[m] = (uint32_t)light_row(S.lights[sort_light], B.seed, head_key(S, B, head, i), sort_light, 1);
     nodes[m] = i;
 }
 
@@ -1093,6 +1081,7 @@
     if (m >= total) return;
     const uint32_t i = lit[slot];
     NodeRec nr = rec.load(i, S.materials);
+    nr.key = rec.key(S, B, i);
     if (rec.eye_cam) camera_eyev(S, B, i, nr.eyev);
     LitStage r;
     for (int k = 0; k < 3; ++k) {
@@ -1169,6 +1158,7 @@
             i = (int64_t)lit[slot];
         }
         nr = rec.load(i, S.materials);
+        nr.key = rec.key(S, B, i);
         if (rec.eye_cam) camera_eyev(S, B, i, nr.eyev);
     }
     if (staged) {
@@ -2055,7 +2045,8 @@
     unsigned long long* jit_stats = nullptr;
     struct Level {
         frt::NodeCols rec;
-        frt::ShadowHead* head = nullptr;
+        double* head_op = nullptr;
+        uint64_t* head_key = nullptr;
         frt::QueuedRay* q = nullptr;
         frt::Cols<frt::Tri9> surface;
         frt::Cols<frt::Tri9> child;
@@ -3359,7 +3350,8 @@
     for (void* p : h->owned) hip_ignore(hipFree(p));
     for (auto& L : h->levels) {
         hip_ignore(hipFree(L.rec.core.w));
-        hip_ignore(hipFree(L.head));
+        hip_ignore(hipFree(L.head_op));
+        hip_ignore(hipFree(L.head_key));
         hip_ignore(hipFree(L.q));
         hip_ignore(hipFree(L.surface.w));
         hip_ignore(hipFree(L.child.w));
@@ -3423,13 +3415,36 @@
     return d == 0 && !h->S.cfg.use_gi && eye_cam_env && h->strip_views == 0 ? 1 : 0;
 }
 
+static bool level_keyed(const frt_scene_handle* h, size_t d) {
+    bool multi = false;
+    for (const auto& L : h->host_lights) multi = multi || L.rows > 1;
+    const char* e = std::getenv("FRT_HEAD_KEY0");
+    if (e && std::atoi(e) == 0) multi = false;
+    return d > 0 || h->S.cfg.use_gi || h->strip_views > 0 || multi;
+}
+
+static int set_level_head(frt_scene_handle* h, size_t d) {
+    auto& L = h->levels[d];
+    if (L.cap <= 0) return 0;
+    if (level_keyed(h, d) && L.head_key == nullptr)
+        FRT_HIP(hipMalloc((void**)&L.head_key, (size_t)L.cap * sizeof(uint64_t)));
+    L.rec.head.op = L.head_op;
+    L.rec.head.key = level_keyed(h, d) ? L.head_key : nullptr;
+    L.rec.head.mat = L.rec.core.w;
+    L.rec.head.cap = L.cap;
+    L.rec.head.node0 = 0;
+    return 0;
+}
+
 static int ensure_level(frt_scene_handle* h, size_t d, int64_t need) {
     auto& L = h->levels[d];
     if (need <= L.cap) return 0;
     int64_t nc = std::max<int64_t>(need, L.cap * 2);
     hip_ignore(hipFree(L.rec.core.w));
-    hip_ignore(hipFree(L.head));
-    L.head = nullptr;
+    hip_ignore(hipFree(L.head_op));
+    hip_ignore(hipFree(L.head_key));
+    L.head_op = nullptr;
+    L.head_key = nullptr;
     hip_ignore(hipFree(L.q));
     hip_ignore(hipFree(L.surface.w));
     hip_ignore(hipFree(L.child.w));
@@ -3448,8 +3463,7 @@
         L.rec.root = d == 0 ? 1 : 0;
         L.rec.eye_cam = level_eye_cam(h, d);
     }
-    FRT_HIP(hipMalloc((void**)&L.head, nc * sizeof(frt::ShadowHead)));
-    L.rec.head = L.head;
+    FRT_HIP(hipMalloc((void**)&L.head_op, (size_t)nc * 3 * sizeof(double)));
     FRT_HIP(hipMalloc((void**)&L.q, nc * sizeof(frt::QueuedRay)));
     FRT_HIP(hipMalloc((void**)&L.surface.w, frt::Cols<frt::Tri9>::bytes(nc)));
     L.surface.cap = nc;
@@ -3459,7 +3473,7 @@
     FRT_HIP(hipMalloc((void**)&L.counts, nc * std::max(1, h->S.num_lights) * sizeof(int32_t)));
     if (h->shade_stage) FRT_HIP(hipMalloc((void**)&L.spos, nc * sizeof(uint32_t)));
     L.cap = nc;
-    return 0;
+    return set_level_head(h, d);
 }
 
 static inline unsigned grid_for(int64_t n, int block = frt::kBlock) { return (unsigned)((n + block - 1) / block); }
@@ -3593,14 +3607,14 @@
 }
 
 template <int F>
-static void launch_shadow_f(frt_scene_handle* h, const frt::Batch& B, const frt::ShadowHead* rec, int64_t n, int32_t* counts) {
+static void launch_shadow_f(frt_scene_handle* h, const frt::Batch& B, const frt::HeadCols& rec, int64_t n, int32_t* counts) {
     const int64_t work = n * h->samples_per_node;
     hipLaunchKernelGGL(frt::k_shadow<F>, dim3(grid_for(work, frt::kTraceBlock)), dim3(frt::kTraceBlock), h->lds_bytes,
                        h->stream, h->S, B, rec, n, h->j_light, h->j_point, h->samples_per_node, counts, h->err);
 }
 
 template <int F>
-static void launch_shadow_redo_f(frt_scene_handle* h, const frt::Batch& B, const frt::ShadowHead* rec, int64_t n,
+static void launch_shadow_redo_f(frt_scene_handle* h, const frt::Batch& B, const frt::HeadCols& rec, int64_t n,
                                  int32_t* counts) {
     hipLaunchKernelGGL(frt::k_shadow_redo<F>, dim3(64), dim3(frt::kTraceBlock), h->lds_bytes, h->stream, h->S, B, rec, n,
                        h->j_light, h->j_point, h->samples_per_node, counts, h->err, h->redo, h->redo_count, h->redo_cap);
@@ -3621,7 +3635,7 @@
     return nblk;
 }
 
-static void launch_shadow(frt_scene_handle* h, const frt::Batch& B, const frt::ShadowHead* rec, int64_t n, int32_t* counts,
+static void launch_shadow(frt_scene_handle* h, const frt::Batch& B, const frt::HeadCols& rec, int64_t n, int32_t* counts,
                           int64_t node0 = 0) {
     if (h->jit_shadow) {
         using frt::jit::kMixLine;
@@ -3652,7 +3666,7 @@
             int64_t per = std::max<int64_t>(1, kMaxPairs / NP);
             if (h->tile > 0) per = std::max<int64_t>(h->tile, per / h->tile * h->tile);
             for (int64_t off = 0; off < n; off += per)
-                launch_shadow(h, B, rec + off, std::min(per, n - off), counts + off * h->S.num_lights, node0 + off);
+                launch_shadow(h, B, rec.at(off), std::min(per, n - off), counts + off * h->S.num_lights, node0 + off);
             return;
         }
         const int64_t npairs = n * NP;
@@ -4671,6 +4685,7 @@
     const int32_t nviews = h->strip_views;
     const int64_t npix = nrows * hs * std::max(1, nviews);
     if (!h->levels.empty()) h->levels[0].rec.eye_cam = level_eye_cam(h, 0);
+    if (!h->levels.empty() && set_level_head(h, 0)) return -1;
     const int32_t spp = (int32_t)(h->S.cam.usteps * h->S.cam.vsteps);
     if (spp <= 0) return fail("render: usteps*vsteps must be positive");
     const char* benv = std::getenv("FRT_BATCH_SAMPLES");
@@ -4786,7 +4801,7 @@
                     return -1;
                 hipLaunchKernelGGL(h->S.num_patterns > 0 ? k_prepare<true> : k_prepare<false>, dim3(grid_for(n)),
                                    dim3(kBlock), 0, h->stream, h->S, B, q, n, h->hits, hn12,
-                                   L.rec, L.head, N.q, h->counters, h->err, tiles ? h->tbox : nullptr, tl,
+                                   L.rec, N.q, h->counters, h->err, tiles ? h->tbox : nullptr, tl,
                                    subtiles ? h->stbox : nullptr, stl, L.counts, dense ? h->spawn_masks : nullptr,
                                    h->prepare_uniform);
                 FRT_HIP(hipGetLastError());
@@ -4810,17 +4825,17 @@
             const uint64_t counters_epoch = h->sync_epoch;
             if (h->S.cfg.include_direct && h->samples_per_node > 0) {
                 KTimer t(h, st, 1);
-                launch_shadow(h, B, L.head, n, L.counts);
+                launch_shadow(h, B, L.rec.head, n, L.counts);
                 FRT_HIP(hipGetLastError());
             }
             if (h->jit_stats && h->S.num_lights > 0) {
                 std::vector<int32_t> hc((size_t)n * h->S.num_lights);
-                std::vector<frt::ShadowHead> hh((size_t)n);
+                std::vector<uint64_t> hh((size_t)n);
                 FRT_HIP(hipMemcpyAsync(hc.data(), L.counts, hc.size() * sizeof(int32_t), hipMemcpyDeviceToHost, h->stream));
-                FRT_HIP(hipMemcpyAsync(hh.data(), L.head, hh.size() * sizeof(frt::ShadowHead), hipMemcpyDeviceToHost, h->stream));
+                FRT_HIP(hipMemcpyAsync(hh.data(), L.rec.core.w, hh.size() * sizeof(uint64_t), hipMemcpyDeviceToHost, h->stream));
                 FRT_HIP(hipStreamSynchronize(h->stream));
                 for (int64_t i = 0; i < n; ++i) {
-                    if (hh[(size_t)i].material < 0) continue;
+                    if ((int32_t)(uint32_t)hh[(size_t)i] < 0) continue;
                     for (int l = 0; l < h->S.num_lights; ++l) {
                         const int32_t c = hc[(size_t)(i * h->S.num_lights + l)];
                         h->uniform_stats[c == 0 ? 1 : (c == h->host_lights[(size_t)l].num_samples ? 0 : 2)]++;
@@ -4866,7 +4881,7 @@
                                            L.counts, h->shade_lit, h->shade_lcount, segcap, h->sort_light, keys, vals,
                                            h->lit_stage);
                     else
-                        hipLaunchKernelGGL(k_lit_rows, dim3(grid_for(n)), dim3(kBlock), 0, h->stream, h->S, B, L.head,
+                        hipLaunchKernelGGL(k_lit_rows, dim3(grid_for(n)), dim3(kBlock), 0, h->stream, h->S, B, L.rec.head,
                                            h->shade_lit, h->shade_lcount, segcap, h->sort_light, keys, vals);
                     auto& lc = h->host_lcount;
                     FRT_HIP(hipMemcpyAsync(lc.data(), h->shade_lcount, lc.size() * sizeof(unsigned), hipMemcpyDeviceToHost,
@@ -5019,9 +5034,9 @@
         st->pruned_secondary = pruned;
         st->hits = hits;
         st->shadow_rays = h->S.cfg.include_direct ? hits * (uint64_t)h->samples_per_node : 0;
-        constexpr double kHead = (double)sizeof(frt::ShadowHead);
         bool multi = false;
         for (const auto& L : h->host_lights) multi = multi || L.rows > 1;
+        const double kHead = multi ? 40.0 : 32.0;
         st->shadow_kernel_bytes = !(h->S.cfg.include_direct && h->samples_per_node > 0) ? 0.0
                                   : h->jit_shadow != nullptr ? (double)h->pairs_walked * 8.0 + (double)h->heads_walked * (kHead + 4.0) +
                                                                    (multi ? 24.0 * (double)h->rays_walked : 0.0)
diff --git a/fast_ray_tracer_amd/csrc/frt_jit.hip b/fast_ray_tracer_amd/csrc/frt_jit.hip
--- a/fast_ray_tracer_amd/csrc/frt_jit.hip
+++ b/fast_ray_tracer_amd/csrc/frt_jit.hip
@@ -1255,7 +1255,7 @@
                          : mode == 3 ? "frt_jit_sub" : "frt_jit_subtile";
         const bool boxed = mode == 1 || mode == 3 || mode == 4;
         o << "extern \"C\" __global__ void __launch_bounds__(kTraceBlock)" << waves_attr("FRT_JIT_BEAM_WAVES") << "\n"
-          << name << "(DevScene S, Batch B, const ShadowHead* __restrict__ shead, uint32_t nlanes, uint32_t nnodes,\n"
+          << name << "(DevScene S, Batch B, const HeadCols shead, uint32_t nlanes, uint32_t nnodes,\n"
              "             const float* __restrict__ tbox, const uint32_t* __restrict__ tlist, jit::SegTable seg,\n"
              "             uint32_t b0, uint32_t tsegcap,\n"
              "             const float* __restrict__ laabb, int32_t* __restrict__ counts, uint32_t* __restrict__ mixed,\n"
@@ -1352,11 +1352,12 @@
             else
                 o << "        live = jit::beam_box32(tbox + 6 * (size_t)tile, bx, bx + 3, W);  // (false: no live node in the tile)\n";
         } else {
-            o << "        const ShadowHead* nr = shead + node;\n"
-                 "        live = nr->material >= 0;\n"
-                 "        if (live) {\n";
+            o << "        live = shead.hit(node);\n"
+                 "        if (live) {\n"
+                 "            double OPN[3];\n"
+                 "            shead.over_point(node, OPN);\n";
             if (T.multi_row)
-                o << "            const int row = light_row_n(" << T.rows() << ", B.seed, nr->key, lt, 0);\n";
+                o << "            const int row = light_row_n(" << T.rows() << ", B.seed, head_key(S, B, shead, node), lt, 0);\n";
             else
                 o << "            const int row = 0;\n";
             if (mode == 2 && SQ && T.multi_row) {
@@ -1372,14 +1373,14 @@
                      "                    bh[a] = fmaxf(bh[a], __double2float_ru(rp[3 * js + a]));\n"
                      "                }\n"
                      "            }\n"
-                     "            jit::beam32(nr->over_point, bl, bh, W);\n";
+                     "            jit::beam32(OPN, bl, bh, W);\n";
             } else {
                 if (mode == 2 && SQ)
                     o << "            const float* bx = laabb + 6 * ((size_t)gp * " << SQ << "u + q);\n";
                 else
                     o << "            const float* bx = laabb + 6 * (" << T.boxbase_of() << " + (int64_t)row * " << T.nparts()
                       << " + pp);\n";
-                o << "            jit::beam32(nr->over_point, bx, bx + 3, W);\n";
+                o << "            jit::beam32(OPN, bx, bx + 3, W);\n";
             }
             o << "        }\n";
         }
@@ -1451,7 +1452,7 @@
             o << "    if (live && !amb && result == 0) {  // the part's samples are unshadowed from every node of the tile\n"
                  "        for (uint32_t n = 0; n < " << TS << "u; ++n) {\n"
                  "            const uint32_t nd = (tile << " << TSL << ") + n;\n"
-                 "            if (nd < nnodes && shead[nd].material >= 0) atomicAdd(counts + nd * " << NL << " + (uint32_t)lt, " << cnt << ");\n"
+                 "            if (nd < nnodes && shead.hit(nd)) atomicAdd(counts + nd * " << NL << " + (uint32_t)lt, " << cnt << ");\n"
                  "        }\n"
                  "    }\n"
                  "    jit::mix_append(live && amb, tile * " << NP << " + gp, " << rsv << ", mixed, mcount, segcap, err);\n"
@@ -1465,7 +1466,7 @@
             o << "    if (live && !amb && result == 0) {  // the sub-part's samples are unshadowed from every node of the tile\n"
                  "        for (uint32_t n = 0; n < " << TS << "u; ++n) {\n"
                  "            const uint32_t nd = (tile << " << TSL << ") + n;\n"
-                 "            if (nd < nnodes && shead[nd].material >= 0) atomicAdd(counts + nd * " << NL
+                 "            if (nd < nnodes && shead.hit(nd)) atomicAdd(counts + nd * " << NL
               << " + (uint32_t)lt, SUBN[gp * " << SQ << "u + q]);\n"
                  "        }\n"
                  "    }\n"
@@ -1481,7 +1482,7 @@
             o << "    if (live && !amb && result == 0) {  // the sub-part's samples are unshadowed from every node of the sub-tile\n"
                  "        for (uint32_t n = 0; n < " << ST << "u; ++n) {\n"
                  "            const uint32_t nd = node + n;\n"
-                 "            if (nd < nnodes && shead[nd].material >= 0) atomicAdd(counts + nd * " << NL
+                 "            if (nd < nnodes && shead.hit(nd)) atomicAdd(counts + nd * " << NL
               << " + (uint32_t)lt, SUBN[gp * " << SQ << "u + q]);\n"
                  "        }\n"
                  "    }\n"
@@ -1526,7 +1527,7 @@
     g.u32 = u32_mode >= 2;
 
     o << "extern \"C\" __global__ void __launch_bounds__(kTraceBlock)" << waves_attr("FRT_JIT_WAVES") << "\n"
-         "frt_jit_shadow(DevScene S, Batch B, const ShadowHead* __restrict__ shead, uint32_t total, uint32_t m0,\n"
+         "frt_jit_shadow(DevScene S, Batch B, const HeadCols shead, uint32_t total, uint32_t m0,\n"
          "               const uint32_t* __restrict__ mixed, jit::SegTable seg, uint32_t b0, uint32_t segcap,\n"
          "               uint32_t all_pairs, const int32_t* __restrict__ psamp, uint32_t subq,\n"
          "               const int32_t* __restrict__ psamp2,\n"
@@ -1544,6 +1545,7 @@
          "    L.node = 0;\n"
          "    L.light = 0;\n"
          "    L.lp = L.op = nullptr;\n"
+         "    L.ocap = 0;\n"
          "    double LP[3] = {0.0, 0.0, 0.0}, OP[3] = {0.0, 0.0, 0.0};\n"
          "    uint32_t jall = 0;  // the sample's index among the node's spn samples (k_shadow_redo's lane)\n"
          "    uint32_t j = 0;  // the lane's sample within its part\n"
@@ -1606,19 +1608,22 @@
          "            L.light = lt;\n"
          "            L.valid = jp >= 0 && in_range;\n"
          "            jall = " << T.first() << " + js;\n"
-         "            const ShadowHead* nr = shead + (in_range ? L.node : 0u);\n"
-         "            if (L.valid && nr->material >= 0) {\n"
+         "            // the node's head words, loaded side by side ahead of the test of its hit (they sit in columns of their\n"
+         "            // own: behind the test their misses would queue up after the material word's)\n"
+         "            const uint32_t nd = in_range ? L.node : 0u;\n"
+         "            const bool hit = shead.hit(nd);\n"
+         "            shead.over_point(nd, OP);\n";
+    if (T.multi_row) o << "            const uint64_t key = head_key(S, B, shead, nd);\n";
+    o << "            if (L.valid && hit) {\n"
          "                L.live = true;\n";
     if (T.multi_row)
-        o << "                const int row = light_row_n(" << T.rows() << ", B.seed, nr->key, lt, 0);\n";
+        o << "                const int row = light_row_n(" << T.rows() << ", B.seed, key, lt, 0);\n";
     else
         o << "                const int row = 0;\n";
     o << "                L.lp = S.light_points + " << T.points() << " + 3 * ((int64_t)row * " << T.ns() << " + js);\n"
-         "                L.op = nr->over_point;\n"
-         "                for (int a = 0; a < 3; ++a) {\n"
-         "                    LP[a] = L.lp[a];\n"
-         "                    OP[a] = L.op[a];\n"
-         "                }\n"
+         "                L.op = shead.op;\n"
+         "                L.ocap = shead.cap;\n"
+         "                for (int a = 0; a < 3; ++a) LP[a] = L.lp[a];\n"
          "            }\n"
          "        }\n"
          "    }\n"
@@ -1722,6 +1727,7 @@
              "    jit::Lane32 L;\n"
              "    L.live = L.valid = false;\n"
              "    L.lp = L.op = nullptr;\n"
+             "    L.ocap = 0;\n"
              "    bool have64 = true;\n"
              "    Ray R64 = ray;\n"
              "    double D64 = 0.0;\n"
diff --git a/fast_ray_tracer_amd/csrc/frt_jit_rt.hpp b/fast_ray_tracer_amd/csrc/frt_jit_rt.hpp
--- a/fast_ray_tracer_amd/csrc/frt_jit_rt.hpp
+++ b/fast_ray_tracer_amd/csrc/frt_jit_rt.hpp
@@ -1,6 +1,6 @@
 #pragma once
 
-#include "frt_shadow.hpp"
+#include "frt_camera.hpp"
 
 namespace frt {
 namespace jit {
@@ -130,9 +130,15 @@
     bool valid, live;
     const double* lp;
     const double* op;
-};
-
-__device__ __forceinline__ void lane32(const DevScene& S, const Batch& B, const ShadowHead* __restrict__ shead,
+    int64_t ocap;
+};
+
+__device__ __forceinline__ void lane_op(const Lane32& L, double* o) {
+#pragma unroll
+    for (int a = 0; a < 3; ++a) o[a] = L.op[a * L.ocap + L.node];
+}
+
+__device__ __forceinline__ void lane32(const DevScene& S, const Batch& B, const HeadCols& shead,
                                        uint32_t total, const int32_t* __restrict__ j_light,
                                        const int32_t* __restrict__ j_point, uint32_t spn, uint64_t magic,
                                        uint32_t shift, uint32_t tid, Lane32& L) {
@@ -141,18 +147,19 @@
     L.node = 0;
     L.light = 0;
     L.lp = L.op = nullptr;
+    L.ocap = 0;
     if (L.valid) {
         L.node = (uint32_t)(((uint64_t)tid * magic) >> shift);
         const uint32_t j = tid - L.node * spn;
         L.light = j_light[j];
         const int pt = j_point[j];
-        const ShadowHead* nr = shead + L.node;
-        if (nr->material >= 0) {
+        if (shead.hit(L.node)) {
             L.live = true;
             const frt_light& lt = S.lights[L.light];
-            const int row = light_row(lt, B.seed, nr->key, L.light, 0);
+            const int row = lt.rows <= 1 ? 0 : light_row(lt, B.seed, head_key(S, B, shead, L.node), L.light, 0);
             L.lp = S.light_points + lt.points + 3 * ((int64_t)row * lt.num_samples + pt);
-            L.op = nr->over_point;
+            L.op = shead.op;
+            L.ocap = shead.cap;
         }
     }
 }
@@ -174,7 +181,11 @@
     return n2 >= 0x1p-60f && n2 <= 0x1p100f && w.omax <= 0x1p100f;
 }
 
-__device__ __forceinline__ bool ray32(const Lane32& L, World32& w, Iv& dist) { return ray32v(L.lp, L.op, w, dist); }
+__device__ __forceinline__ bool ray32(const Lane32& L, World32& w, Iv& dist) {
+    double op[3];
+    lane_op(L, op);
+    return ray32v(L.lp, op, w, dist);
+}
 
 __device__ __forceinline__ bool ray32d(const Ray& r, World32& w) {
 #pragma unroll
@@ -193,11 +204,12 @@
         dist = 0.0;
         return;
     }
-    double v[3];
-#pragma unroll
-    for (int a = 0; a < 3; ++a) {
-        v[a] = L.lp[a] - L.op[a];
-        r.o[a] = L.op[a];
+    double v[3], op[3];
+    lane_op(L, op);
+#pragma unroll
+    for (int a = 0; a < 3; ++a) {
+        v[a] = L.lp[a] - op[a];
+        r.o[a] = op[a];
     }
     dist = sqrt(v[0] * v[0] + v[1] * v[1] + v[2] * v[2]);
     normalize3(v, r.d);
@@ -258,7 +270,7 @@
     }
 }
 
-__device__ __forceinline__ void add_run_counts(const ShadowHead* __restrict__ shead, int32_t* counts, uint32_t nl,
+__device__ __forceinline__ void add_run_counts(const HeadCols& shead, int32_t* counts, uint32_t nl,
                                                bool add, uint32_t base, uint32_t len, uint32_t lt, int32_t amount,
                                                uint32_t nnodes) {
     const int lane = threadIdx.x & 63;
@@ -274,7 +286,7 @@
         for (int o = 32; o > 0; o >>= 1) v += __shfl_xor(v, o, 64);
         for (uint32_t n = (uint32_t)lane; n < len; n += 64u) {
             const uint32_t nd = b0 + n;
-            if (nd < nnodes && shead[nd].material >= 0) atomicAdd(counts + nd * nl + l0, v);
+            if (nd < nnodes && shead.hit(nd)) atomicAdd(counts + nd * nl + l0, v);
         }
     }
 }
diff --git a/fast_ray_tracer_amd/csrc/frt_shadow.hpp b/fast_ray_tracer_amd/csrc/frt_shadow.hpp
--- a/fast_ray_tracer_amd/csrc/frt_shadow.hpp
+++ b/fast_ray_tracer_amd/csrc/frt_shadow.hpp
@@ -53,13 +53,33 @@
     return (int64_t)lo * B.qsegcap + (i - B.qprefix[lo]);
 }
 
-struct alignas(8) ShadowHead {
-    double over_point[3];
-    uint64_t key;
-    int32_t material;
-    int32_t pad;
+__device__ __forceinline__ uint64_t camera_key(const DevScene& S, const Batch& B, int64_t s);
+
+struct HeadCols {
+    double* op = nullptr;
+    uint64_t* key = nullptr;
+    const uint64_t* mat = nullptr;
+    int64_t cap = 0;
+    int64_t node0 = 0;
+
+    __host__ __device__ HeadCols at(int64_t off) const {
+        HeadCols v = *this;
+        v.op += off;
+        if (v.key != nullptr) v.key += off;
+        v.mat += off;
+        v.node0 += off;
+        return v;
+    }
+    __device__ __forceinline__ bool hit(int64_t i) const { return (int32_t)(uint32_t)mat[i] >= 0; }
+    __device__ __forceinline__ void over_point(int64_t i, double* o) const {
+#pragma unroll
+        for (int a = 0; a < 3; ++a) o[a] = op[a * cap + i];
+    }
 };
-static_assert(sizeof(ShadowHead) == 40, "ShadowHead layout");
+
+__device__ __forceinline__ uint64_t head_key(const DevScene& S, const Batch& B, const HeadCols& H, int64_t i) {
+    return H.key != nullptr ? H.key[i] : camera_key(S, B, H.node0 + i);
+}
 
 struct ShadowLane {
     Ray r;
@@ -70,7 +90,7 @@
     bool live;
 };
 
-__device__ __forceinline__ void shadow_lane(const DevScene& S, const Batch& B, const ShadowHead* __restrict__ shead,
+__device__ __forceinline__ void shadow_lane(const DevScene& S, const Batch& B, const HeadCols& shead,
                                             int64_t n, const int32_t* __restrict__ j_light,
                                             const int32_t* __restrict__ j_point, int32_t samples_per_node,
                                             int64_t tid, ShadowLane& L) {
@@ -85,17 +105,18 @@
         const int j = (int)(tid % samples_per_node);
         L.light = j_light[j];
         const int pt = j_point[j];
-        const ShadowHead* nr = shead + L.node;
-        if (nr->material >= 0) {
+        if (shead.hit(L.node)) {
             L.live = true;
             const frt_light& lt = S.lights[L.light];
-            const int row = light_row(lt, B.seed, nr->key, L.light, 0);
+            const int row = lt.rows <= 1 ? 0 : light_row(lt, B.seed, head_key(S, B, shead, L.node), L.light, 0);
             const double* lp = S.light_points + lt.points + 3 * ((int64_t)row * lt.num_samples + pt);
-            double v[3] = {lp[0] - nr->over_point[0], lp[1] - nr->over_point[1], lp[2] - nr->over_point[2]};
+            double op[3];
+            shead.over_point(L.node, op);
+            double v[3] = {lp[0] - op[0], lp[1] - op[1], lp[2] - op[2]};
             L.distance = sqrt(v[0] * v[0] + v[1] * v[1] + v[2] * v[2]);
-            L.r.o[0] = nr->over_point[0];
-            L.r.o[1] = nr->over_point[1];
-            L.r.o[2] = nr->over_point[2];
+            L.r.o[0] = op[0];
+            L.r.o[1] = op[1];
+            L.r.o[2] = op[2];
             normalize3(v, L.r.d);
         }
     }
```

Measured after the change: 518,200 (median of 6 runs). +2.1%, better.
